# ruotianluo/ImageCaptioning.pytorch

Hardware: NVIDIA H100
Metric: captions/sec at beam=5 seq_len=20 (higher is better)
Workload: dtype f32 (fp32-grade: split-fp16 x3 tensor-core passes, fp32 accumulate)

## Files before the change

imagecaptioning.pytorch_b200/csrc/beam.cu:

```cuda
#include "../../include/capb200.h"
#include "common.cuh"
#include "kernels.cuh"
#include "vocab_row.cuh"

namespace capb200 {

namespace {

constexpr int MAXB = 16;

__device__ __forceinline__ double apply_penalty(int kind, float alpha, int length, double p) {
    if (kind == 1) return p / (pow(5.0 + length, (double)alpha) / pow(6.0, (double)alpha));
    if (kind == 2) return p / (double)length;
    return p;
}

template <int U = 8>
__device__ __forceinline__ void select_step(const BeamState& s, int img, int t, int live, int kl, int row0, int hist0, const float* top_val,
                                            const int* top_idx, const int* pen, int n_pen, float lambda, int penalty_kind,
                                            float penalty_alpha, double* __restrict__ done_p) {
    const int lane = threadIdx.x;
    const int b = s.beam, T = s.T;
    const int ncand = live * kl;
    float cv[U];
// ... 33 lines not shown
#pragma unroll
        for (int o = 16; o > 0; o >>= 1) {
            const float ov = __shfl_xor_sync(0xffffffffu, wv, o);
            const int of = __shfl_xor_sync(0xffffffffu, wf, o);
            if (ov > wv || (ov == wv && of < wf)) { wv = ov; wf = of; }
        }
        if (bu >= 0 && bf == wf && bv == wv) {
#pragma unroll
            for (int u = 0; u < U; ++u) if (u == bu) { cv[u] = -INFINITY; cf[u] = 0x7fffffff; }
        }
        if (lane == j) { my_v = wv; my_f = wf; }
    }
    __shared__ int sh_parent[MAXB], sh_word[MAXB], sh_slot[MAXB];
    const bool has = lane < b;
    const int parent = has ? my_f / s.V1 : 0;
    const int word = has ? my_f % s.V1 : 0;
    const bool ended = has && ((word == 0) || (t == T - 1));
    const unsigned em = __ballot_sync(0xffffffffu, ended);
    const int cnt0 = s.done_cnt[img];
    const int slot = cnt0 + __popc(em & ((1u << lane) - 1u));
    if (has) { sh_parent[lane] = parent; sh_word[lane] = word; sh_slot[lane] = ended ? slot : -1; }
    __syncwarp();
#pragma unroll 1
    for (int idx = lane; idx < b * t; idx += 32) {
        const int j = idx / t, q = idx - j * t;
        const long dst = ((long)img * b + j) * T, src = ((long)img * b + sh_parent[j]) * T;
        seq_new[dst + q] = seq_old[src + q];
        hist_new[dst + q] = hist_old[src + q];
    }
    if (em != 0u) {
#pragma unroll 1
        for (int idx = lane; idx < b * (t + 1); idx += 32) {
            const int j = idx / (t + 1), q = idx - j * (t + 1);
            if (sh_slot[j] < 0) continue;
            const long rec = ((long)img * b * T + sh_slot[j]) * T, src = ((long)img * b + sh_parent[j]) * T;
            s.done_seq[rec + q] = (q < t) ? seq_old[src + q] : sh_word[j];
            s.done_hist[rec + q] = (q < t) ? hist_old[src + q] : hist0 + sh_parent[j];
        }
    }
    if (has) {
        const long dst = ((long)img * b + lane) * T;
        seq_new[dst + t] = word;
        hist_new[dst + t] = hist0 + parent;
        float new_sum = my_v;
        if (ended) {
            const long rec = (long)img * b * T + slot;
            s.done_len[rec] = t + 1;
            s.done_raw[rec] = new_sum;
            done_p[rec] = apply_penalty(penalty_kind, penalty_alpha, t + 1, (double)new_sum);
            new_sum -= 1000.0f;
        }
        s.sums[(long)img * b + lane] = new_sum;
        s.tokens[(long)img * b + lane] = word;
        s.src_row[(long)img * b + lane] = row0 + parent;
    }
    if (lane == 0 && em != 0u) s.done_cnt[img] = cnt0 + __popc(em);
}

__global__ void __launch_bounds__(32) beam_step_kernel(BeamState s, int t, int live, const float* __restrict__ top_val,
                                                       const int* __restrict__ top_idx, int penalty_kind, float penalty_alpha,
                                                       double* __restrict__ done_p) {
    const int img = blockIdx.x;
    const long row0 = (long)img * live;
    select_step(s, img, t, live, s.beam, (int)row0, (int)row0, top_val + row0 * s.beam, top_idx + row0 * s.beam, nullptr, 0, 0.f, penalty_kind,
                penalty_alpha, done_p);
}

constexpr int kStepGroups = 8;
template <int U>
__global__ void __maxnreg__(U <= 2 ? 48 : 64) beam_search_step_kernel(BeamState s, const VocabStepArgs a, int t, int live, int penalty_kind, float penalty_alpha,
                                                        double* __restrict__ done_p, NextStateGather next) {
    __shared__ float s_red[kStepGroups][VT2 / 32];
    __shared__ int s_ridx[kStepGroups][VT2 / 32];
    __shared__ float s_val[MAXB * MAXB];
    __shared__ int s_idx[MAXB * MAXB];
    const int img = blockIdx.x, g = threadIdx.x / VT2, ng = blockDim.x / VT2;
    const int b = s.beam, row0 = img * live;
    for (int j = g; j < live; j += ng)
        stats_online128_row(a, row0 + j, threadIdx.x % VT2, GroupBarrier{1 + g}, s_red[g], s_ridx[g], s_val + j * b, s_idx + j * b);
    __syncthreads();
    if (threadIdx.x < 32) select_step<U>(s, img, t, live, b, row0, row0, s_val, s_idx, nullptr, 0, 0.f, penalty_kind, penalty_alpha, done_p);
    if (t == s.T - 1) return;
    __syncthreads();
    const int n4 = next.H >> 2;
    for (int i = threadIdx.x; i < b * n4; i += blockDim.x) {
        const int j = i / n4, c4 = i - j * n4;
        const long r = (long)img * b + j;
        copy_states4(r, s.src_row[r], c4, 2, next.s0, next.s1);
    }
}

__global__ void __launch_bounds__(32) diverse_beam_step_kernel(BeamState s, int G, int t, int k, const float* __restrict__ top_val,
                                                               const int* __restrict__ top_idx, float lambda, int rows_total, int penalty_kind,
                                                               float penalty_alpha, double* __restrict__ done_p) {
    const int i = blockIdx.x, lane = threadIdx.x;
    const int b = s.beam, T = s.T;
    __shared__ int sh_pen[MAXB];
    for (int g = 0; g < G && g <= t; ++g) {
        const int lt = t - g;
        if (lt >= T) continue;
        const int n_pen = g * b;
        __syncwarp();
        if (lane < n_pen) {
            const int pg = lane / b, j = lane - pg * b;
            const int last = min(t - pg, T - 1);
            const int* seq_pg = (last & 1) ? s.seq_a : s.seq_b;
            sh_pen[lane] = seq_pg[((long)(i * G + pg) * b + j) * T + lt];
        }
        __syncwarp();
        const int vimg = i * G + g;
        select_step(s, vimg, lt, lt == 0 ? 1 : b, k, vimg * b, g * rows_total + vimg * b, top_val + (long)vimg * b * k, top_idx + (long)vimg * b * k,
                    sh_pen, n_pen, lambda, penalty_kind, penalty_alpha, done_p);
    }
}

__global__ void __launch_bounds__(32) beam_finalize_kernel(BeamState s, int keep, const double* __restrict__ done_p, long long* __restrict__ out_seq,
                                                           int* __restrict__ out_len, float* __restrict__ out_p, float* __restrict__ out_raw,
                                                           int* __restrict__ out_hist) {
    const int img = blockIdx.x, lane = threadIdx.x;
    const int b = s.beam, T = s.T;
    const int cnt = s.done_cnt[img];
    const long base = (long)img * b * T;
    extern __shared__ unsigned char taken[];
    for (int i = lane; i < cnt; i += 32) taken[i] = 0;
    __syncwarp();
    for (int k = 0; k < keep; ++k) {
        double bv = -INFINITY;
        int bi = 0x7fffffff;
        for (int i = lane; i < cnt; i += 32) {
            if (!taken[i]) {
                const double v = done_p[base + i];
                if (v > bv || (v == bv && i < bi)) { bv = v; bi = i; }
            }
        }
#pragma unroll
        for (int o = 16; o > 0; o >>= 1) {
            const double ov = __shfl_xor_sync(0xffffffffu, bv, o);
            const int oi = __shfl_xor_sync(0xffffffffu, bi, o);
            if (ov > bv || (ov == bv && oi < bi)) { bv = ov; bi = oi; }
        }
        const long o = (long)img * keep + k;
        if (bi == 0x7fffffff) {
            if (lane == 0) { out_len[o] = 0; out_p[o] = -INFINITY; out_raw[o] = -INFINITY; }
            for (int q = lane; q < T; q += 32) { out_seq[o * T + q] = 0; out_hist[o * T + q] = -1; }
            continue;
        }
        if (lane == 0) {
            taken[bi] = 1;
            out_len[o] = s.done_len[base + bi];
            out_p[o] = (float)bv;
            out_raw[o] = s.done_raw[base + bi];
        }
        const int len = s.done_len[base + bi];
        for (int q = lane; q < T; q += 32) {
            out_seq[o * T + q] = (q < len) ? (long long)s.done_seq[(base + bi) * T + q] : 0;
            out_hist[o * T + q] = (q < len) ? s.done_hist[(base + bi) * T + q] : -1;
        }
        __syncwarp();
    }
}

__global__ void beam_edit_kernel(int rows, int k_in, int beam, int t, DecodeEdits ed, const int* __restrict__ prev_tokens,
                                 const float* __restrict__ val_in, const int* __restrict__ idx_in, float* __restrict__ val_out, int* __restrict__ idx_out,
                                 int first_beam, int first_group_rows, int first_group) {
    const int r = blockIdx.x * blockDim.x + threadIdx.x;
    if (r >= rows) return;
    if (first_beam > 0 && (r % first_beam) / first_group_rows == first_group) t = 0;
    float v[MAXB];
    int ix[MAXB];
    const int prev = (t > 0 && prev_tokens != nullptr) ? prev_tokens[r] : -1;
    bool prev_bad = false;
// ... 40 lines not shown
        return;
    }
    auto apply_edits = [&]() {
        if (seqs == nullptr || !ed.any()) return;
        __syncthreads();
        if (threadIdx.x == 0) {
            const int prev = sidx > 0 ? (int)seqs[item - 1] : -1;
            if (ed.unk_col >= 0 && ed.unk_col < V1) d[ed.unk_col] -= 1000.0f;
            if (ed.constraint && prev >= 0 && prev < V1) d[prev] = -INFINITY;
            bool prev_bad = false;
            for (int i = 0; i < ed.n_bad; ++i) prev_bad |= (sidx > 0 && ed.bad[i] == prev);
            if (prev_bad) d[0] = -INFINITY;
        }
    };
    const float* src = slab + (long)sidx * step_stride + (long)row * ld_slab;
    if (stats != nullptr) {
        const float2 st = stats[(long)sidx * stats_stride + row];
        const float mx = st.x, lsum = st.y;
        const float m2 = (mx - mx) - lsum, l2 = lsum;
        const bool twice = sidx > 0;
        const bool vec4 = ((V1 & 3) == 0) && ((ld_slab & 3) == 0) && ((step_stride & 3) == 0) && ((reinterpret_cast<uintptr_t>(slab) & 15) == 0) &&
                          ((reinterpret_cast<uintptr_t>(dst) & 15) == 0);
        if (vec4) {
            const float4* s4 = reinterpret_cast<const float4*>(src);
            float4* d4 = reinterpret_cast<float4*>(d);
            for (int v = threadIdx.x; v < V1 / 4; v += blockDim.x) {
                const float4 x = __ldg(s4 + v);
                float4 o;
                o.x = (x.x - mx) - lsum; o.y = (x.y - mx) - lsum; o.z = (x.z - mx) - lsum; o.w = (x.w - mx) - lsum;
                if (twice) { o.x = (o.x - m2) - l2; o.y = (o.y - m2) - l2; o.z = (o.z - m2) - l2; o.w = (o.w - m2) - l2; }
                d4[v] = o;
            }
        } else {
            for (int v = threadIdx.x; v < V1; v += blockDim.x) {
                const float lp = (src[v] - mx) - lsum;
                d[v] = twice ? (lp - m2) - l2 : lp;
            }
        }
        apply_edits();
        return;
    }
    const bool vec = ((V1 & 3) == 0) && ((ld_slab & 3) == 0) && ((step_stride & 3) == 0) && ((reinterpret_cast<uintptr_t>(slab) & 15) == 0) &&
                     ((reinterpret_cast<uintptr_t>(dst) & 15) == 0);
    if (vec) {
        const float4* s4 = reinterpret_cast<const float4*>(src);
        float4* d4 = reinterpret_cast<float4*>(d);
        for (int v = threadIdx.x; v < V1 / 4; v += blockDim.x) d4[v] = __ldg(s4 + v);
    } else {
        for (int v = threadIdx.x; v < V1; v += blockDim.x) d[v] = src[v];
    }
    apply_edits();
}

}

int beam_edit_launch(int rows, int k_in, int beam, int t, const DecodeEdits& ed, const int* prev_tokens, const float* val_in, const int* idx_in,
                     float* val_out, int* idx_out, cudaStream_t stream, int first_beam, int first_group_rows, int first_group) {
    CAPB_REQUIRE(k_in >= beam && k_in <= MAXB, "beam_size + number of active decode edits must be <= 16");
    if (rows <= 0) return 0;
    beam_edit_kernel<<<cdiv(rows, 128), 128, 0, stream>>>(rows, k_in, beam, t, ed, prev_tokens, val_in, idx_in, val_out, idx_out, first_beam,
                                                          first_group_rows, first_group);
    CAPB_CHECK_CUDA(cudaGetLastError());
    return 0;
}

int scale_rows_launch(float* x, long ld, int rows, int cols, float factor, cudaStream_t stream, int skip_beam, int skip_group_rows, int skip_group) {
    if (rows <= 0 || cols <= 0) return 0;
    long blocks = ((long)rows * cols + 255) / 256;
    if (blocks > sm_count() * 16) blocks = sm_count() * 16;
    scale_rows_kernel<<<(int)blocks, 256, 0, stream>>>(x, ld, rows, cols, factor, skip_beam, skip_group_rows, skip_group);
    CAPB_CHECK_CUDA(cudaGetLastError());
    return 0;
}

int beam_step_launch(const BeamState& s, int t, int live, const float* top_val, const int* top_idx, int penalty_kind, float penalty_alpha,
                     cudaStream_t stream) {
    CAPB_REQUIRE(s.beam >= 1 && s.beam <= MAXB, "beam size 1..16");
    CAPB_REQUIRE(s.beam * s.T <= MAXB * CAPB200_MAX_SEQ_LENGTH, "beam*T record capacity (16 x CAPB200_MAX_SEQ_LENGTH)");
    beam_step_kernel<<<s.B, 32, 0, stream>>>(s, t, live, top_val, top_idx, penalty_kind, penalty_alpha, s.done_p);
    CAPB_CHECK_CUDA(cudaGetLastError());
    return 0;
}

bool beam_search_step_applies(const VocabStepArgs& a, const NextStateGather& next) {
    auto al16 = [](const void* p) { return (reinterpret_cast<uintptr_t>(p) & 15) == 0; };
    auto al8 = [](const void* p) { return (reinterpret_cast<uintptr_t>(p) & 7) == 0; };
    auto state_ok = [&](const StateCopy& c) {
        return c.src != nullptr && c.dst.f != nullptr && (c.ld_src & 3) == 0 && (c.dst.ld & 3) == 0 && al16(c.src) && al16(c.dst.f) &&
               ((c.dst.hi == nullptr) == (c.dst.lo == nullptr)) && (c.dst.hi == nullptr || (al8(c.dst.hi) && al8(c.dst.lo)));
    };
    return (a.V1 & 3) == 0 && (a.ld & 3) == 0 && al16(a.logits) && next.H > 0 && (next.H & 3) == 0 && state_ok(next.s0) && state_ok(next.s1);
}

int beam_search_step_launch(const BeamState& s, const VocabStepArgs& a, int t, int live, int penalty_kind, float penalty_alpha,
                            const NextStateGather& next, cudaStream_t stream) {
    CAPB_REQUIRE(s.beam >= 1 && s.beam <= MAXB, "beam size 1..16");
    CAPB_REQUIRE(s.beam * s.T <= MAXB * CAPB200_MAX_SEQ_LENGTH, "beam*T record capacity (16 x CAPB200_MAX_SEQ_LENGTH)");
    CAPB_REQUIRE(a.topk == s.beam && a.stats != nullptr && a.rows == s.B * live && live >= 1 && live <= s.beam, "fused beam step arguments");
    CAPB_REQUIRE(beam_search_step_applies(a, next), "the fused beam step needs 16-byte aligned logit and state rows (V + 1 and H multiples of 4)");
    const int threads = min(live, kStepGroups) * VT2;
    if (s.beam <= 8) beam_search_step_kernel<2><<<s.B, threads, 0, stream>>>(s, a, t, live, penalty_kind, penalty_alpha, s.done_p, next);
    else beam_search_step_kernel<8><<<s.B, threads, 0, stream>>>(s, a, t, live, penalty_kind, penalty_alpha, s.done_p, next);
    CAPB_CHECK_CUDA(cudaGetLastError());
    return 0;
}

int diverse_beam_step_launch(const BeamState& s, int G, int t, int k, const float* top_val, const int* top_idx, float lambda, int rows_total,
                             int penalty_kind, float penalty_alpha, cudaStream_t stream) {
    CAPB_REQUIRE(G >= 2 && s.beam >= 1 && G * s.beam <= MAXB, "group_size * beams per group must be in 2..16");
    CAPB_REQUIRE(k >= s.beam && k <= MAXB && s.beam * k <= 256, "candidate list width");
    CAPB_REQUIRE(s.beam * s.T <= MAXB * CAPB200_MAX_SEQ_LENGTH, "beam*T record capacity (16 x CAPB200_MAX_SEQ_LENGTH)");
    CAPB_REQUIRE(lambda >= 0.f, "diversity_lambda must be >= 0 (the candidate lists rely on the penalty only lowering values)");
    diverse_beam_step_kernel<<<s.B / G, 32, 0, stream>>>(s, G, t, k, top_val, top_idx, lambda, rows_total, penalty_kind, penalty_alpha, s.done_p);
    CAPB_CHECK_CUDA(cudaGetLastError());
    return 0;
}

int beam_finalize_launch(const BeamState& s, int keep, long long* out_seq, int* out_len, float* out_p, float* out_raw, int* out_hist,
                         cudaStream_t stream) {
    CAPB_REQUIRE(keep >= 1 && keep <= s.beam, "keep must be in 1..beam");
    beam_finalize_kernel<<<s.B, 32, (size_t)s.beam * s.T, stream>>>(s, keep, s.done_p, out_seq, out_len, out_p, out_raw, out_hist);
    CAPB_CHECK_CUDA(cudaGetLastError());
    return 0;
}

int gather_logprob_rows_launch(const float* slab, long step_stride, long ld_slab, const int* hist, int nseq, int T, int V1, float* dst,
                               const float2* stats, long stats_stride, cudaStream_t stream, const long long* seqs, const DecodeEdits* ed) {
    if (nseq <= 0) return 0;
    gather_rows_kernel<<<nseq * T, 256, 0, stream>>>(slab, step_stride, ld_slab, hist, T, V1, dst, stats, stats_stride, seqs, ed ? *ed : DecodeEdits());
    CAPB_CHECK_CUDA(cudaGetLastError());
    return 0;
}

}
```

imagecaptioning.pytorch_b200/csrc/common.cuh:

```cuda
#pragma once
#include <atomic>
#include <cstdint>
#include <cstdio>
#include <cstring>
#include <string>
#include <cuda.h>
#include <cuda_fp16.h>
#include <cuda_runtime.h>

namespace capb200 {

void set_error(const std::string& msg);
#define CAPB_CHECK_CUDA(expr)                                                                          \
    do {                                                                                               \
        cudaError_t _e = (expr);                                                                       \
        if (_e != cudaSuccess) {                                                                       \
            capb200::set_error(std::string(#expr) + " failed: " + cudaGetErrorString(_e) + " at " +    \
                               __FILE__ + ":" + std::to_string(__LINE__));                            \
            return 1;                                                                                  \
        }                                                                                              \
    } while (0)
#define CAPB_REQUIRE(cond, msg)                                                                        \
    do {                                                                                               \
        if (!(cond)) {                                                                                 \
            capb200::set_error(std::string("requirement failed: ") + #cond + " -- " + (msg));          \
            return 1;                                                                                  \
        }                                                                                              \
    } while (0)

inline int cdiv(int a, int b) { return (a + b - 1) / b; }
inline long round_up(long a, long b) { return (a + b - 1) / b * b; }

inline bool first_use_on_device(std::atomic<unsigned long long>& mask) {
    int dev = 0;
    if (cudaGetDevice(&dev) != cudaSuccess || dev < 0 || dev > 63) return true;
    const unsigned long long bit = 1ull << dev;
    return (mask.fetch_or(bit) & bit) == 0;
}

inline int sm_count() {
    static std::atomic<int> cache[64];
    int dev = 0;
    if (cudaGetDevice(&dev) != cudaSuccess || dev < 0 || dev > 63) dev = 0;
    int n = cache[dev].load();
    if (n == 0) {
        if (cudaDeviceGetAttribute(&n, cudaDevAttrMultiProcessorCount, dev) != cudaSuccess || n < 1) n = 132;
        cache[dev].store(n);
    }
    return n;
}

__device__ __forceinline__ void split_f32(float x, __half& hi, __half& lo) {
    hi = __float2half_rn(x);
    lo = __float2half_rn(x - __half2float(hi));
}

constexpr int kMaxSeg = 3;
struct GemmSeg {
    const float* A = nullptr;
    long lda = 0;
    const float* W = nullptr;
    long ldw = 0;
    const __half* A_hi = nullptr;
    const __half* A_lo = nullptr;
    long lda_h = 0;
    const __half* W_hi = nullptr;
    const __half* W_lo = nullptr;
    long ldw_h = 0;
    int K = 0;
};
struct GemmEpilogue {
    const float* bias = nullptr;
    const float* row_bias = nullptr;
    long ld_row_bias = 0;
    int rows_per_group = 1;
    const float* residual = nullptr;
    long ld_res = 0;
    int relu = 0;
    float* C = nullptr;
    long ldc = 0;
    __half* C_hi = nullptr;
    __half* C_lo = nullptr;
    long ldcs = 0;
    int lstm = 0;
    int H = 0;
    const float* c_prev = nullptr;
    long ld_cprev = 0;
    const int* src_row = nullptr;
    float* c_out = nullptr;
    long ld_cout = 0;
    const float* gather_bias = nullptr;
    long ld_gb = 0;
    const int* gather_idx = nullptr;
    float* h_f = nullptr;
    __half* h_hi = nullptr;
    __half* h_lo = nullptr;
    long ld_h = 0;
    unsigned long long* trace = nullptr;
};

__device__ __forceinline__ float fast_sigmoid(float x) { return __fdividef(1.0f, 1.0f + __expf(-x)); }
__device__ __forceinline__ float fast_tanh(float x) {
    const float e = __expf(2.0f * x);
    return 1.0f - __fdividef(2.0f, 1.0f + e);
}
__device__ __forceinline__ void fast_tanh4(const float (&x)[4], float (&t)[4]) {
    float y[4];
#pragma unroll
    for (int i = 0; i < 4; ++i) y[i] = 1.0f + __expf(fminf(2.0f * x[i], 20.0f));
    const float p01 = y[0] * y[1], p23 = y[2] * y[3];
    const float r = __fdividef(1.0f, p01 * p23);
    const float r01 = r * p23, r23 = r * p01;
    t[0] = fmaf(-2.0f, r01 * y[1], 1.0f);
    t[1] = fmaf(-2.0f, r01 * y[0], 1.0f);
    t[2] = fmaf(-2.0f, r23 * y[3], 1.0f);
    t[3] = fmaf(-2.0f, r23 * y[2], 1.0f);
}
struct GemmProblem {
    int M = 0, N = 0, nseg = 0;
    GemmSeg seg[kMaxSeg];
    GemmEpilogue epi;
};

enum NumericMode : int {
    kModeSimtFp32 = 0,
    kModeTcF16x3 = 1,
    kModeTcF16x1 = 2,
};

int gemm_simt_launch(const GemmProblem& p, cudaStream_t stream);

struct GemmTcPlan;
GemmTcPlan* gemm_tc_plan_create(const GemmProblem& p, int passes);
int gemm_tc_tile_n(int M, int N);
int gemm_tc_tile_m(int M, int N, int bn);
void gemm_tc_plan_destroy(GemmTcPlan* plan);
int gemm_tc_plan_launch(GemmTcPlan* plan, const GemmEpilogue* epi_override, int M_override, cudaStream_t stream);
bool gemm_tc_supported(const GemmProblem& p, std::string* why);

int split_planes_launch(const float* x, long ldx, int rows, int cols, __half* hi, __half* lo, long ldh, cudaStream_t stream);
int* range_flag_ptr();
int range_flag_read(int reset);
#define CAPB_CHECK_RANGE()                                                                                              \
    do {                                                                                                                \
        if (capb200::range_flag_read(0)) {                                                                              \
            capb200::set_error("a value with |x| >= 65504 (or inf/nan) reached a split-fp16 conversion in an earlier call: results of the "   \
                               "tensor-core modes are invalid for such inputs/weights (DESIGN.md section 3); capb200_range_status(1) clears the flag"); \
            return 1;                                                                                                   \
        }                                                                                                               \
    } while (0)
int split_planes_interleave_launch(const float* x, long ldx, int H, int cols, __half* hi, __half* lo, long ldh, cudaStream_t stream);

}
```

imagecaptioning.pytorch_b200/csrc/engine.cu:

```cuda
#include <map>
#include <mutex>
#include <vector>

#include "../../include/capb200.h"
#include "common.cuh"
#include "kernels.cuh"
#include "engine_common.cuh"
#include "train_common.cuh"

namespace capb200 {

static thread_local std::string g_last_error;
void set_error(const std::string& msg) { g_last_error = msg; }
const char* last_error_cstr() { return g_last_error.c_str(); }

__global__ void capb_fill_int_kernel(int* p, int n, int v) {
    const int i = blockIdx.x * blockDim.x + threadIdx.x;
    if (i < n) p[i] = v;
}
__global__ void capb_load_token_column_kernel(const long long* src, long ld, int col, int n, int* dst) {
    const int i = blockIdx.x * blockDim.x + threadIdx.x;
    if (i < n) dst[i] = (int)src[(long)i * ld + col];
}
__global__ void capb_store_token_column_kernel(const int* src, int n, long long* dst, long ld, int col) {
    const int i = blockIdx.x * blockDim.x + threadIdx.x;
    if (i < n) dst[(long)i * ld + col] = src[i];
}
int store_token_column_launch(const int* src, int n, long long* dst, long ld, int col, cudaStream_t st) {
    if (n <= 0) return 0;
    capb_store_token_column_kernel<<<cdiv(n, 256), 256, 0, st>>>(src, n, dst, ld, col);
    CAPB_CHECK_CUDA(cudaGetLastError());
    return 0;
}
int fill_int_launch(int* p, int n, int v, cudaStream_t st) {
    if (n <= 0) return 0;
    capb_fill_int_kernel<<<cdiv(n, 256), 256, 0, st>>>(p, n, v);
    CAPB_CHECK_CUDA(cudaGetLastError());
    return 0;
}
int load_token_column_launch(const long long* src, long ld, int col, int n, int* dst, cudaStream_t st) {
    if (n <= 0) return 0;
    capb_load_token_column_kernel<<<cdiv(n, 256), 256, 0, st>>>(src, ld, col, n, dst);
    CAPB_CHECK_CUDA(cudaGetLastError());
    return 0;
}

namespace {

__global__ void add_vec_kernel(const float* a, const float* b, float* o, int n) {
    const int i = blockIdx.x * blockDim.x + threadIdx.x;
    if (i < n) o[i] = a[i] + b[i];
}
__global__ void interleave_gates_kernel(const float* src, float* dst, int H) {
    const int i = blockIdx.x * blockDim.x + threadIdx.x;
    if (i < 4 * H) dst[i] = src[(i & 3) * H + (i >> 2)];
}

__global__ void iota_div_kernel(int* p, int n, int div) {
    const int i = blockIdx.x * blockDim.x + threadIdx.x;
    if (i < n) p[i] = i / div;
}


enum GemmId { G_FC = 0, G_ATT, G_CTX, G_GFC, G_LSTM1, G_H2ATT, G_LSTM2, G_LOGIT, G_CORE, G_A2C, G_COUNT };
constexpr int G_REPORTED = 9;

}
}

using namespace capb200;


struct capb200_engine : EngineBase {
    capb200_model_cfg cfg{};
    capb200_weights w{};
    int E = 0, H = 0, A = 0;

    float *bsum_att = nullptr, *bsum_lang = nullptr, *bsum_core = nullptr;
    float *bsum_att_il = nullptr, *bsum_lang_il = nullptr;
    float* xgate = nullptr;
    long ld_xgate = 0;
    bool use_xgate = true;
    Planes p_fc, p_attw, p_ctx, p_logit, p_a_ih_h, p_a_ih_fc, p_a_ih_x, p_a_hh, p_l_ih_a, p_l_ih_h, p_l_hh, p_h2att, p_i2h, p_h2h, p_a2c;

    Planes in_fc, in_att;
    Act fc_e, att_e, p_att, g_fc, xt, h0_in, h1_in, h0_out, h1_out, att_res, att_h, gates;
    float *c0[2] = {nullptr, nullptr}, *c1[2] = {nullptr, nullptr};
    long ld_c = 0;
    int* img_of_row = nullptr;
    float* att_score = nullptr;
    int core_cur = 0;

    bool profiling = false;
    std::vector<cudaEvent_t> ev_pool;
    std::vector<int> ev_ids;
    std::vector<double> ev_flops;
    size_t ev_used = 0;
    double prof_ms[G_COUNT] = {0};
    double prof_flops[G_COUNT] = {0};
    long prof_calls[G_COUNT] = {0};

    ~capb200_engine() override { for (cudaEvent_t ev : ev_pool) cudaEventDestroy(ev); }
    int decode_workspace(int B, int rows, int R, int beam, int rows_per_image, cudaStream_t st) override;
    int decode_prepare(const float* fc, const float* att, const DecodeCtx& c, cudaStream_t st) override;
    int decode_core(int rows, int rpi, const int* tokens, const int* src_row, int t, float* logits, long ld, const DecodeCtx& c, cudaStream_t st) override;
    bool next_state(NextStateGather* next) override;
    bool loop_graph_ok() const override { return !profiling; }
};

namespace {

void layout_weights(capb200_engine* e, Arena& a) {
    const int H = e->H, E = e->E, A = e->A, V1 = e->V1;
    const bool updown = e->cfg.family == CAPB200_FAMILY_UPDOWN;
    e->bsum_att = a.take<float>(4 * H);
    e->bsum_lang = a.take<float>(4 * H);
    e->bsum_core = a.take<float>(5 * H);
    e->bsum_att_il = a.take<float>(4 * H);
    e->bsum_lang_il = a.take<float>(4 * H);
    if (updown) { e->ld_xgate = round_up(4 * H, 8); e->xgate = a.take<float>((long)V1 * e->ld_xgate); }
    if (!e->tc) return;
    e->p_logit = carve_planes(a, V1, H);
    if (updown) {
        e->p_fc = carve_planes(a, H, e->cfg.fc_feat_size);
        e->p_attw = carve_planes(a, H, e->cfg.att_feat_size);
        e->p_ctx = carve_planes(a, A, H);
        e->p_a_ih_h = carve_planes(a, 4 * H, H);
        e->p_a_ih_fc = carve_planes(a, 4 * H, H);
        e->p_a_ih_x = carve_planes(a, 4 * H, E);
        e->p_a_hh = carve_planes(a, 4 * H, H);
        e->p_l_ih_a = carve_planes(a, 4 * H, H);
        e->p_l_ih_h = carve_planes(a, 4 * H, H);
        e->p_l_hh = carve_planes(a, 4 * H, H);
        e->p_h2att = carve_planes(a, A, H);
    } else if (e->cfg.family == CAPB200_FAMILY_ATT2IN2) {
        e->p_attw = carve_planes(a, H, e->cfg.att_feat_size);
        e->p_ctx = carve_planes(a, A, H);
        e->p_h2att = carve_planes(a, A, H);
        e->p_i2h = carve_planes(a, 5 * H, E);
        e->p_h2h = carve_planes(a, 5 * H, H);
        e->p_a2c = carve_planes(a, 2 * H, H);
    } else {
        e->p_fc = carve_planes(a, E, e->cfg.fc_feat_size);
        e->p_i2h = carve_planes(a, 5 * H, E);
        e->p_h2h = carve_planes(a, 5 * H, H);
    }
}

void layout_workspace(capb200_engine* e, Arena& a, int B, int rows, int R, int beam) {
    const int H = e->H, E = e->E, A = e->A, T = e->T;
    const bool updown = e->cfg.family == CAPB200_FAMILY_UPDOWN;
    const bool attn = e->reads_att;
    const bool tc = e->tc;
    if (tc) {
        e->in_fc = carve_planes(a, B, e->cfg.fc_feat_size);
        if (attn) e->in_att = carve_planes(a, (long)B * R, e->cfg.att_feat_size);
    }
    e->fc_e.carve(a, B, updown ? H : E, tc);
    if (attn) {
        e->att_e.carve(a, (long)B * R, H, tc);
        e->p_att.carve(a, (long)B * R, A, false);
        e->att_res.carve(a, rows, H, tc);
        e->att_h.carve(a, rows, A, false);
    }
    if (updown) {
        e->g_fc.carve(a, B, 4 * H, false);
        e->h1_in.carve(a, rows, H, tc);
        e->h1_out.carve(a, rows, H, tc);
    }
    e->xt.carve(a, rows, E, tc);
    e->h0_in.carve(a, rows, H, tc);
    e->h0_out.carve(a, rows, H, tc);
    e->gates.carve(a, rows, 5 * H, false);
    e->ld_c = round_up(H, 8);
    for (int i = 0; i < 2; ++i) {
        e->c0[i] = a.take<float>((long)rows * e->ld_c);
        e->c1[i] = a.take<float>((long)rows * e->ld_c);
    }
    e->carve_head(a, rows);
    e->img_of_row = a.take<int>(rows);
    e->att_score = a.take<float>((long)rows * (R > 0 ? R : 1));
    e->d.carve(a, B, rows, beam, T);
}

int ensure_workspace(capb200_engine* e, int B, int rows, int R, int beam, cudaStream_t st) {
    return e->grow(B, rows, R, beam, st, [&](Arena& a, int nB, int nRows, int nR, int nBeam) { layout_workspace(e, a, nB, nRows, nR, nBeam); });
}

int run_gemm(capb200_engine* e, int id, GemmProblem& g, int plan_rows, cudaStream_t st) {
    if (!e->profiling) return e->gemm(id, g, plan_rows, st);
    if (e->ev_used + 2 > e->ev_pool.size()) {
        for (int i = 0; i < 64; ++i) {
            cudaEvent_t ev;
            CAPB_CHECK_CUDA(cudaEventCreate(&ev));
            e->ev_pool.push_back(ev);
        }
    }
    double k_total = 0;
    for (int s = 0; s < g.nseg; ++s) k_total += g.seg[s].K;
    CAPB_CHECK_CUDA(cudaEventRecord(e->ev_pool[e->ev_used], st));
    const int rc = e->gemm(id, g, plan_rows, st);
    CAPB_CHECK_CUDA(cudaEventRecord(e->ev_pool[e->ev_used + 1], st));
    e->ev_used += 2;
    e->ev_ids.push_back(id);
    e->ev_flops.push_back(2.0 * g.M * g.N * k_total);
    return rc;
}

int prepare(capb200_engine* e, const float* fc, const float* att, const float* mask, int B, int R, cudaStream_t st) {
    CAPB_NVTX("capb200 prepare_feature (fc_embed, att_embed, ctx2att)");
    const int H = e->H, E = e->E, A = e->A;
    const bool updown = e->cfg.family == CAPB200_FAMILY_UPDOWN;
    const capb200_weights& w = e->w;
    ActView fc_in;  fc_in.f = const_cast<float*>(fc);  fc_in.ld = e->cfg.fc_feat_size;
    if (e->tc && e->cfg.family != CAPB200_FAMILY_ATT2IN2) {
        e->launches++;
        if (split_planes_launch(fc, e->cfg.fc_feat_size, B, e->cfg.fc_feat_size, e->in_fc.hi, e->in_fc.lo, e->in_fc.ld, st)) return 1;
    }
    if (e->cfg.family != CAPB200_FAMILY_ATT2IN2) {
        GemmProblem g;
        g.M = B; g.N = updown ? H : E; g.nseg = 1;
        g.seg[0] = seg_of(fc_in, w.fc_embed_w, e->cfg.fc_feat_size, e->p_fc, e->cfg.fc_feat_size);
        g.seg[0].A_hi = e->in_fc.hi; g.seg[0].A_lo = e->in_fc.lo; g.seg[0].lda_h = e->in_fc.ld;
        g.epi.bias = w.fc_embed_b; g.epi.relu = updown ? 1 : 0;
        g.epi.C = e->fc_e.v.f; g.epi.ldc = e->fc_e.v.ld; g.epi.C_hi = e->fc_e.v.hi; g.epi.C_lo = e->fc_e.v.lo; g.epi.ldcs = e->fc_e.v.ld;
        if (run_gemm(e, G_FC, g, e->capB, st)) return 1;
    }
    if (!e->reads_att) return 0;
    ActView att_in; att_in.f = const_cast<float*>(att); att_in.ld = e->cfg.att_feat_size;
    if (e->tc) {
        e->launches++;
        if (split_planes_launch(att, e->cfg.att_feat_size, B * R, e->cfg.att_feat_size, e->in_att.hi, e->in_att.lo, e->in_att.ld, st)) return 1;
    }
    {
        GemmProblem g;
        g.M = B * R; g.N = H; g.nseg = 1;
        g.seg[0] = seg_of(att_in, w.att_embed_w, e->cfg.att_feat_size, e->p_attw, e->cfg.att_feat_size);
        g.seg[0].A_hi = e->in_att.hi; g.seg[0].A_lo = e->in_att.lo; g.seg[0].lda_h = e->in_att.ld;
        g.epi.bias = w.att_embed_b; g.epi.relu = 1;
        g.epi.C = e->att_e.v.f; g.epi.ldc = e->att_e.v.ld; g.epi.C_hi = e->att_e.v.hi; g.epi.C_lo = e->att_e.v.lo; g.epi.ldcs = e->att_e.v.ld;
        if (run_gemm(e, G_ATT, g, e->capB * e->capR, st)) return 1;
    }
    if (mask != nullptr) {
        e->launches++;
        if (mask_rows_launch(e->att_e.v, B, R, H, mask, R, st)) return 1;
    }
    {
        GemmProblem g;
        g.M = B * R; g.N = A; g.nseg = 1;
        g.seg[0] = seg_of(e->att_e.v, w.ctx2att_w, H, e->p_ctx, H);
        g.epi.bias = w.ctx2att_b;
        g.epi.C = e->p_att.v.f; g.epi.ldc = e->p_att.v.ld;
        if (run_gemm(e, G_CTX, g, e->capB * e->capR, st)) return 1;
    }
    if (!updown) return 0;
    {
        GemmProblem g;
        g.M = B; g.N = 4 * H; g.nseg = 1;
        g.seg[0] = seg_of(e->fc_e.v, w.att_lstm_w_ih + H, E + 2 * H, e->p_a_ih_fc, H);
        g.epi.bias = e->tc ? e->bsum_att_il : e->bsum_att;
        g.epi.C = e->g_fc.v.f; g.epi.ldc = e->g_fc.v.ld;
        if (run_gemm(e, G_GFC, g, e->capB, st)) return 1;
    }
    return 0;
}

int logit_gemm(capb200_engine* e, const ActView& h, int rows, float* logits, long ld_logits, cudaStream_t st) {
    ActView x;
    if (e->run_logit_head(h, rows, &x, st)) return 1;
    GemmProblem g;
    g.M = rows; g.N = e->V1; g.nseg = 1;
    g.seg[0] = seg_of(x, e->w.logit_w, e->H, e->p_logit, e->H);
    g.epi.bias = e->w.logit_b;
    g.epi.C = logits; g.epi.ldc = ld_logits;
    return run_gemm(e, G_LOGIT, g, e->capRows, st);
}

int core_step(capb200_engine* e, int rows, int rpi, const int* tokens, const int* src_row, float* logits, long ld_logits, int n_images, int R,
              const float* mask, cudaStream_t st, bool states_gathered = false) {
    const int H = e->H, E = e->E, A = e->A;
    const capb200_weights& w = e->w;
    if (e->cfg.family == CAPB200_FAMILY_UPDOWN) {
        StateCopy s0, s1;
        s0.src = e->h0_out.v.f; s0.ld_src = e->h0_out.v.ld; s0.dst = e->h0_in.v;
        s1.src = e->h1_out.v.f; s1.ld_src = e->h1_out.v.ld; s1.dst = e->h1_in.v;
        const bool xg = e->use_xgate;
        CAPB_REQUIRE(!states_gathered || xg, "the fused beam step gathers the states only; the word embedding needs the separate gather");
        if (!states_gathered) {
            e->launches++;
            if (state_gather_embed_launch(rows, tokens, src_row, w.embed, E, xg ? 0 : E, 1, e->xt.v, H, 2, s0, s1, st)) return 1;
        }
        const int cur = e->core_cur, nxt = cur ^ 1;
        {
            GemmProblem g;
            g.M = rows; g.N = 4 * H;
            g.seg[0] = seg_of(e->h1_in.v, w.att_lstm_w_ih, E + 2 * H, e->p_a_ih_h, H);
            g.seg[1] = seg_of(e->h0_in.v, w.att_lstm_w_hh, H, e->p_a_hh, H);
            g.nseg = 2;
            if (!xg) { g.seg[2] = seg_of(e->xt.v, w.att_lstm_w_ih + 2 * H, E + 2 * H, e->p_a_ih_x, E); g.nseg = 3; }
            g.epi.row_bias = e->g_fc.v.f; g.epi.ld_row_bias = e->g_fc.v.ld; g.epi.rows_per_group = rpi;
            if (e->tc) {
                g.epi.lstm = 1; g.epi.H = H;
                g.epi.c_prev = e->c0[cur]; g.epi.ld_cprev = e->ld_c; g.epi.src_row = src_row;
                g.epi.c_out = e->c0[nxt]; g.epi.ld_cout = e->ld_c;
                g.epi.gather_bias = xg ? e->xgate : nullptr; g.epi.ld_gb = e->ld_xgate; g.epi.gather_idx = tokens;
                g.epi.h_f = e->h0_out.v.f; g.epi.h_hi = e->h0_out.v.hi; g.epi.h_lo = e->h0_out.v.lo; g.epi.ld_h = e->h0_out.v.ld;
            } else {
                g.epi.C = e->gates.v.f; g.epi.ldc = e->gates.v.ld;
            }
            if (run_gemm(e, G_LSTM1, g, e->capRows, st)) return 1;
        }
        if (!e->tc) {
            e->launches++;
            if (lstm_pointwise_launch(rows, H, e->gates.v.f, e->gates.v.ld, src_row, e->c0[cur], e->ld_c, e->c0[nxt], e->ld_c, e->h0_out.v,
                                      xg ? e->xgate : nullptr, e->ld_xgate, tokens, st)) return 1;
        }
        {
            GemmProblem g;
            g.M = rows; g.N = A; g.nseg = 1;
            g.seg[0] = seg_of(e->h0_out.v, w.h2att_w, H, e->p_h2att, H);
            g.epi.bias = w.h2att_b;
            g.epi.C = e->att_h.v.f; g.epi.ldc = e->att_h.v.ld;
            if (run_gemm(e, G_H2ATT, g, e->capRows, st)) return 1;
        }
        e->launches += 2;
        if (additive_attention_launch(n_images, rpi, R, A, H, e->att_h.v.f, e->att_h.v.ld, e->p_att.v.f, e->p_att.v.ld, e->att_e.v.f, e->att_e.v.ld,
                                      mask, R, w.alpha_w, w.alpha_b, e->att_score, e->att_res.v, st)) return 1;
        {
            GemmProblem g;
            g.M = rows; g.N = 4 * H; g.nseg = 3;
            g.seg[0] = seg_of(e->att_res.v, w.lang_lstm_w_ih, 2 * H, e->p_l_ih_a, H);
            g.seg[1] = seg_of(e->h0_out.v, w.lang_lstm_w_ih + H, 2 * H, e->p_l_ih_h, H);
            g.seg[2] = seg_of(e->h1_in.v, w.lang_lstm_w_hh, H, e->p_l_hh, H);
            if (e->tc) {
                g.epi.bias = e->bsum_lang_il;
                g.epi.lstm = 1; g.epi.H = H;
                g.epi.c_prev = e->c1[cur]; g.epi.ld_cprev = e->ld_c; g.epi.src_row = src_row;
                g.epi.c_out = e->c1[nxt]; g.epi.ld_cout = e->ld_c;
                g.epi.h_f = e->h1_out.v.f; g.epi.h_hi = e->h1_out.v.hi; g.epi.h_lo = e->h1_out.v.lo; g.epi.ld_h = e->h1_out.v.ld;
            } else {
                g.epi.bias = e->bsum_lang;
                g.epi.C = e->gates.v.f; g.epi.ldc = e->gates.v.ld;
            }
            if (run_gemm(e, G_LSTM2, g, e->capRows, st)) return 1;
        }
        if (!e->tc) {
            e->launches++;
            if (lstm_pointwise_launch(rows, H, e->gates.v.f, e->gates.v.ld, src_row, e->c1[cur], e->ld_c, e->c1[nxt], e->ld_c, e->h1_out.v,
                                      nullptr, 0, nullptr, st)) return 1;
        }
        e->core_cur = nxt;
        return logit_gemm(e, e->h1_out.v, rows, logits, ld_logits, st);
    }
    if (e->cfg.family == CAPB200_FAMILY_ATT2IN2) {
        StateCopy s0, s1;
        s0.src = e->h0_out.v.f; s0.ld_src = e->h0_out.v.ld; s0.dst = e->h0_in.v;
        e->launches++;
        if (state_gather_embed_launch(rows, tokens, src_row, w.embed, E, E, 1, e->xt.v, H, 1, s0, s1, st)) return 1;
        const int cur = e->core_cur, nxt = cur ^ 1;
        {
            GemmProblem g;
            g.M = rows; g.N = A; g.nseg = 1;
            g.seg[0] = seg_of(e->h0_in.v, w.h2att_w, H, e->p_h2att, H);
            g.epi.bias = w.h2att_b;
            g.epi.C = e->att_h.v.f; g.epi.ldc = e->att_h.v.ld;
            if (run_gemm(e, G_H2ATT, g, e->capRows, st)) return 1;
        }
        e->launches += 2;
        if (additive_attention_launch(n_images, rpi, R, A, H, e->att_h.v.f, e->att_h.v.ld, e->p_att.v.f, e->p_att.v.ld, e->att_e.v.f, e->att_e.v.ld,
                                      mask, R, w.alpha_w, w.alpha_b, e->att_score, e->att_res.v, st)) return 1;
        {
            GemmProblem g;
            g.M = rows; g.N = 5 * H; g.nseg = 2;
            g.seg[0] = seg_of(e->xt.v, w.i2h_w, E, e->p_i2h, E);
            g.seg[1] = seg_of(e->h0_in.v, w.h2h_w, H, e->p_h2h, H);
            g.epi.bias = e->bsum_core;
            g.epi.C = e->gates.v.f; g.epi.ldc = e->gates.v.ld;
            if (run_gemm(e, G_CORE, g, e->capRows, st)) return 1;
        }
        {
            GemmProblem g;
            g.M = rows; g.N = 2 * H; g.nseg = 1;
            g.seg[0] = seg_of(e->att_res.v, w.a2c_w, H, e->p_a2c, H);
            g.epi.residual = e->gates.v.f + 3 * H; g.epi.ld_res = e->gates.v.ld;
            g.epi.C = e->gates.v.f + 3 * H; g.epi.ldc = e->gates.v.ld;
            if (run_gemm(e, G_A2C, g, e->capRows, st)) return 1;
        }
        e->launches++;
        if (maxout_pointwise_launch(rows, H, e->gates.v.f, e->gates.v.ld, src_row, e->c0[cur], e->ld_c, e->c0[nxt], e->ld_c, e->h0_out.v, st)) return 1;
        e->core_cur = nxt;
        return logit_gemm(e, e->h0_out.v, rows, logits, ld_logits, st);
    }
    const bool fresh = (src_row == e->d.neg1);
    for (int pass = fresh ? 0 : 1; pass < 2; ++pass) {
        StateCopy s0, s1;
        s0.src = e->h0_out.v.f; s0.ld_src = e->h0_out.v.ld; s0.dst = e->h0_in.v;
        const int* srcs = (pass == 0) ? e->d.neg1 : (fresh ? nullptr : src_row);
        e->launches++;
        if (pass == 0) {
            if (state_gather_embed_launch(rows, e->img_of_row, srcs, e->fc_e.v.f, e->fc_e.v.ld, E, 0, e->xt.v, H, 1, s0, s1, st)) return 1;
        } else {
            if (state_gather_embed_launch(rows, tokens, srcs, w.embed, E, E, 0, e->xt.v, H, 1, s0, s1, st)) return 1;
        }
        const int cur = e->core_cur, nxt = cur ^ 1;
        GemmProblem g;
        g.M = rows; g.N = 5 * H; g.nseg = 2;
        g.seg[0] = seg_of(e->xt.v, w.i2h_w, E, e->p_i2h, E);
        g.seg[1] = seg_of(e->h0_in.v, w.h2h_w, H, e->p_h2h, H);
        g.epi.bias = e->bsum_core;
        g.epi.C = e->gates.v.f; g.epi.ldc = e->gates.v.ld;
        if (run_gemm(e, G_CORE, g, e->capRows, st)) return 1;
        e->launches++;
        if (maxout_pointwise_launch(rows, H, e->gates.v.f, e->gates.v.ld, srcs, e->c0[cur], e->ld_c, e->c0[nxt], e->ld_c, e->h0_out.v, st)) return 1;
        e->core_cur = nxt;
    }
    return logit_gemm(e, e->h0_out.v, rows, logits, ld_logits, st);
}

}

namespace capb200 {

int add_vec_launch(const float* a, const float* b, float* o, int n, cudaStream_t st) {
    add_vec_kernel<<<cdiv(n, 256), 256, 0, st>>>(a, b, o, n);
    CAPB_CHECK_CUDA(cudaGetLastError());
    return 0;
}

int interleave_gates_launch(const float* src, float* dst, int H, cudaStream_t st) {
    interleave_gates_kernel<<<cdiv(4 * H, 256), 256, 0, st>>>(src, dst, H);
    CAPB_CHECK_CUDA(cudaGetLastError());
    return 0;
}

int build_gate_table(EngineBase& e, const float* embed, int E, int H, const float* w_x, long ld_w, const Planes& p_x, float* xgate, long ld_xgate,
                     cudaStream_t st) {
    const int V1 = e.V1;
    const long ldE = round_up(E, 8);
    char* tmp = nullptr;
    const size_t tmp_bytes = (size_t)V1 * ldE * (sizeof(float) + (e.tc ? 2 * sizeof(__half) : 0)) + 1024;
    CAPB_CHECK_CUDA(cudaMallocAsync(&tmp, tmp_bytes, st));
    CAPB_CHECK_CUDA(cudaMemsetAsync(tmp, 0, tmp_bytes, st));
    ActView ev;
    ev.ld = ldE;
    ev.f = reinterpret_cast<float*>(tmp);
    if (e.tc) {
        ev.hi = reinterpret_cast<__half*>(tmp + (size_t)V1 * ldE * sizeof(float));
        ev.lo = ev.hi + (size_t)V1 * ldE;
    }
    int rc = 0;
    if (ldE == E) {
        rc = relu_copy_launch(embed, (long)V1 * E, ev, st);
    } else {
        for (int v = 0; v < V1 && !rc; ++v) {
            ActView rv = ev;
            rv.f += (long)v * ldE; if (rv.hi) { rv.hi += (long)v * ldE; rv.lo += (long)v * ldE; }
            rc = relu_copy_launch(embed + (long)v * E, E, rv, st);
        }
    }
    GemmProblem g;
    g.M = V1; g.N = 4 * H; g.nseg = 1;
    g.seg[0] = seg_of(ev, w_x, ld_w, p_x, E);
    g.epi.C = xgate; g.epi.ldc = ld_xgate;
    if (!rc) {
        if (!e.tc) {
            rc = gemm_simt_launch(g, st);
        } else {
            GemmTcPlan* plan = gemm_tc_plan_create(g, e.mode == CAPB200_MODE_TC_F16X3 ? 3 : 1);
            rc = plan ? gemm_tc_plan_launch(plan, nullptr, 0, st) : 1;
            if (plan) gemm_tc_plan_destroy(plan);
        }
    }
    e.launches += 2;
    cudaFreeAsync(tmp, st);
    return rc;
}

EngineBase* engine_base(capb200_engine* e) { return e; }

}

int capb200_engine::decode_workspace(int B, int rows, int R, int beam, int rows_per_image, cudaStream_t st) {
    if (ensure_workspace(this, B, rows, R, beam, st)) return 1;
    if (!reads_att) { iota_div_kernel<<<cdiv(rows, 256), 256, 0, st>>>(img_of_row, rows, rows_per_image); launches++; }
    return 0;
}

int capb200_engine::decode_prepare(const float* fc, const float* att, const DecodeCtx& c, cudaStream_t st) {
    if (prepare(this, fc, att, c.mask, c.B, c.R, st)) return 1;
    core_cur = 0;
    return 0;
}

int capb200_engine::decode_core(int rows, int rpi, const int* tokens, const int* src_row, int , float* logits, long ld, const DecodeCtx& c,
                                cudaStream_t st) {
    return core_step(this, rows, rpi, tokens, src_row, logits, ld, c.B, c.R, c.mask, st, d.states_gathered);
}

bool capb200_engine::next_state(NextStateGather* next) {
    if (cfg.family != CAPB200_FAMILY_UPDOWN || !use_xgate) return false;
    next->s0.src = h0_out.v.f; next->s0.ld_src = h0_out.v.ld; next->s0.dst = h0_in.v;
    next->s1.src = h1_out.v.f; next->s1.ld_src = h1_out.v.ld; next->s1.dst = h1_in.v;
    next->H = H;
    return true;
}

extern "C" {

const char* capb200_last_error(void) { return g_last_error.c_str(); }
int capb200_abi_version(void) { return CAPB200_ABI_VERSION; }
int capb200_range_status(int reset) { return range_flag_read(reset); }

capb200_engine* capb200_engine_create(const capb200_model_cfg* cfg) {
    if (cfg == nullptr) { set_error("null cfg"); return nullptr; }
    if (cfg->family != CAPB200_FAMILY_UPDOWN && cfg->family != CAPB200_FAMILY_NEWFC && cfg->family != CAPB200_FAMILY_ATT2IN2) {
        set_error("unknown model family");
        return nullptr;
    }
    capb200_engine* e = create_engine<capb200_engine>(cfg->vocab_size, cfg->seq_length, cfg->numeric_mode, G_COUNT);
    if (e == nullptr) return nullptr;
    e->cfg = *cfg;
    e->E = cfg->input_encoding_size;
    e->H = cfg->rnn_size;
    e->A = cfg->att_hid_size;
    e->bind_name = "capb200_engine_bind_weights";
    e->family = e->graph_family = cfg->family;
    e->reads_fc = cfg->family != CAPB200_FAMILY_ATT2IN2;
    e->reads_att = cfg->family != CAPB200_FAMILY_NEWFC;
    return e;
}

void capb200_engine_destroy(capb200_engine* e) { delete e; }

long capb200_engine_launch_count(const capb200_engine* e) { return e ? e->launches : 0; }

int capb200_engine_set_profiling(capb200_engine* e, int enable) {
    CAPB_REQUIRE(e != nullptr, "null engine");
    e->profiling = enable != 0;
    return 0;
}

int capb200_engine_read_profile(capb200_engine* e, int reset, double* ms, double* flops, long* calls, int n) {
    CAPB_REQUIRE(e != nullptr && n >= G_REPORTED, "need room for 9 GEMM ids");
    CAPB_CHECK_CUDA(cudaDeviceSynchronize());
    for (size_t i = 0; i < e->ev_ids.size(); ++i) {
        float t = 0.f;
        CAPB_CHECK_CUDA(cudaEventElapsedTime(&t, e->ev_pool[2 * i], e->ev_pool[2 * i + 1]));
        e->prof_ms[e->ev_ids[i]] += t;
        e->prof_flops[e->ev_ids[i]] += e->ev_flops[i];
        e->prof_calls[e->ev_ids[i]] += 1;
    }
    e->ev_ids.clear();
    e->ev_flops.clear();
    e->ev_used = 0;
    e->prof_ms[G_CORE] += e->prof_ms[G_A2C]; e->prof_flops[G_CORE] += e->prof_flops[G_A2C]; e->prof_calls[G_CORE] += e->prof_calls[G_A2C];
    e->prof_ms[G_A2C] = 0; e->prof_flops[G_A2C] = 0; e->prof_calls[G_A2C] = 0;
    for (int i = 0; i < G_REPORTED; ++i) {
        if (ms) ms[i] = e->prof_ms[i];
        if (flops) flops[i] = e->prof_flops[i];
        if (calls) calls[i] = e->prof_calls[i];
        if (reset) { e->prof_ms[i] = 0; e->prof_flops[i] = 0; e->prof_calls[i] = 0; }
    }
    return 0;
}

int capb200_engine_bind_weights(capb200_engine* e, const capb200_weights* w, void* stream) {
    CAPB_REQUIRE(e != nullptr && w != nullptr, "null argument");
    cudaStream_t st = static_cast<cudaStream_t>(stream);
    const bool updown = e->cfg.family == CAPB200_FAMILY_UPDOWN;
    const bool att2in2 = e->cfg.family == CAPB200_FAMILY_ATT2IN2;
    CAPB_REQUIRE(w->embed && (att2in2 || (w->fc_embed_w && w->fc_embed_b)) && w->logit_w && w->logit_b, "missing shared weights");
    if (att2in2) {
        CAPB_REQUIRE(w->att_embed_w && w->att_embed_b && w->ctx2att_w && w->ctx2att_b && w->h2att_w && w->h2att_b && w->alpha_w && w->alpha_b &&
                         w->i2h_w && w->i2h_b && w->h2h_w && w->h2h_b && w->a2c_w && w->a2c_b, "missing Att2in2 weights");
    } else if (updown) {
        CAPB_REQUIRE(w->att_embed_w && w->att_embed_b && w->ctx2att_w && w->ctx2att_b && w->att_lstm_w_ih && w->att_lstm_w_hh && w->att_lstm_b_ih &&
                         w->att_lstm_b_hh && w->lang_lstm_w_ih && w->lang_lstm_w_hh && w->lang_lstm_b_ih && w->lang_lstm_b_hh && w->h2att_w &&
                         w->h2att_b && w->alpha_w && w->alpha_b, "missing UpDown weights");
    } else {
        CAPB_REQUIRE(w->i2h_w && w->i2h_b && w->h2h_w && w->h2h_b, "missing NewFC weights");
    }
    e->w = *w;
    const int H = e->H, E = e->E, A = e->A, V1 = e->V1;
    if (e->alloc_wblock(st, [&](Arena& a) { layout_weights(e, a); })) return 1;
    int rc = 0;
    if (updown) {
        rc |= add_vec_launch(w->att_lstm_b_ih, w->att_lstm_b_hh, e->bsum_att, 4 * H, st);
        rc |= add_vec_launch(w->lang_lstm_b_ih, w->lang_lstm_b_hh, e->bsum_lang, 4 * H, st);
        rc |= interleave_gates_launch(e->bsum_att, e->bsum_att_il, H, st);
        rc |= interleave_gates_launch(e->bsum_lang, e->bsum_lang_il, H, st);
        e->launches += 4;
    } else {
        rc |= add_vec_launch(w->i2h_b, w->h2h_b, e->bsum_core, 5 * H, st);
        e->launches += 1;
        if (att2in2) {
            rc |= add_vec_launch(e->bsum_core + 3 * H, w->a2c_b, e->bsum_core + 3 * H, 2 * H, st);
            e->launches += 1;
        }
    }
    if (rc) return 1;
    if (e->tc) {
        rc = e->pack(w->logit_w, H, V1, H, e->p_logit, st);
        if (updown) {
            rc |= e->pack(w->fc_embed_w, e->cfg.fc_feat_size, H, e->cfg.fc_feat_size, e->p_fc, st);
            rc |= e->pack(w->att_embed_w, e->cfg.att_feat_size, H, e->cfg.att_feat_size, e->p_attw, st);
            rc |= e->pack(w->ctx2att_w, H, A, H, e->p_ctx, st);
            rc |= e->pack_gates(w->att_lstm_w_ih, E + 2 * H, H, H, e->p_a_ih_h, st);
            rc |= e->pack_gates(w->att_lstm_w_ih + H, E + 2 * H, H, H, e->p_a_ih_fc, st);
            rc |= e->pack_gates(w->att_lstm_w_ih + 2 * H, E + 2 * H, H, E, e->p_a_ih_x, st);
            rc |= e->pack_gates(w->att_lstm_w_hh, H, H, H, e->p_a_hh, st);
            rc |= e->pack_gates(w->lang_lstm_w_ih, 2 * H, H, H, e->p_l_ih_a, st);
            rc |= e->pack_gates(w->lang_lstm_w_ih + H, 2 * H, H, H, e->p_l_ih_h, st);
            rc |= e->pack_gates(w->lang_lstm_w_hh, H, H, H, e->p_l_hh, st);
            rc |= e->pack(w->h2att_w, H, A, H, e->p_h2att, st);
        } else if (att2in2) {
            rc |= e->pack(w->att_embed_w, e->cfg.att_feat_size, H, e->cfg.att_feat_size, e->p_attw, st);
            rc |= e->pack(w->ctx2att_w, H, A, H, e->p_ctx, st);
            rc |= e->pack(w->h2att_w, H, A, H, e->p_h2att, st);
            rc |= e->pack(w->i2h_w, E, 5 * H, E, e->p_i2h, st);
            rc |= e->pack(w->h2h_w, H, 5 * H, H, e->p_h2h, st);
            rc |= e->pack(w->a2c_w, H, 2 * H, H, e->p_a2c, st);
        } else {
            rc |= e->pack(w->fc_embed_w, e->cfg.fc_feat_size, E, e->cfg.fc_feat_size, e->p_fc, st);
            rc |= e->pack(w->i2h_w, E, 5 * H, E, e->p_i2h, st);
            rc |= e->pack(w->h2h_w, H, 5 * H, H, e->p_h2h, st);
        }
// ... 1025 lines not shown
```

imagecaptioning.pytorch_b200/csrc/engine_common.cuh:

```cuda
#pragma once
#include <cstdio>
#include <cstdlib>
#include <cstring>
#include <string>
#include <vector>

#include "../../include/capb200.h"
#include "common.cuh"
#include "kernels.cuh"
#include "nvtx.cuh"

struct capb200_cider_table {
    capb200::CiderTable* t = nullptr;
};

namespace capb200 {

struct Planes {
    __half* hi = nullptr;
    __half* lo = nullptr;
    long ld = 0;
};

struct Arena {
// ... 10 lines not shown

struct Act {
    ActView v;
    void carve(Arena& a, long rows, long cols, bool planes) {
        v.ld = round_up(cols, 64);
        v.f = a.take<float>(rows * v.ld);
        if (planes) {
            v.hi = a.take<__half>(rows * v.ld);
            v.lo = a.take<__half>(rows * v.ld);
        } else {
            v.hi = v.lo = nullptr;
        }
    }
};

inline DecodeEdits to_edits(const capb200_decode_edits& c) {
    DecodeEdits e;
    e.constraint = c.decoding_constraint;
    e.unk_col = c.unk_col;
    e.n_bad = (c.bad_endings != nullptr && c.n_bad_endings > 0) ? c.n_bad_endings : 0;
    e.bad = c.bad_endings;
    e.trigrams = c.block_trigrams;
    e.trigram_rows = c.trigram_rows;
    return e;
}

inline Planes carve_planes(Arena& a, long rows, long cols) {
    Planes p;
    p.ld = round_up(cols, 64);
    p.hi = a.take<__half>(rows * p.ld);
    p.lo = a.take<__half>(rows * p.ld);
    return p;
}


inline GemmSeg seg_of(const ActView& a, const float* w, long ldw, const Planes& wp, int K) {
    GemmSeg s;
    s.A = a.f; s.lda = a.ld; s.W = w; s.ldw = ldw;
    s.A_hi = a.hi; s.A_lo = a.lo; s.lda_h = a.ld;
    s.W_hi = wp.hi; s.W_lo = wp.lo; s.ldw_h = wp.ld;
    s.K = K;
    return s;
}


inline int run_gemm_mode(int mode, GemmTcPlan** plan, GemmProblem& g, int plan_rows, cudaStream_t st) {
    if (mode == 0) return gemm_simt_launch(g, st);
    if (*plan == nullptr) {
        GemmProblem planned = g;
        planned.M = plan_rows;
        *plan = gemm_tc_plan_create(planned, mode == 1 ? 3 : 1);
        if (*plan == nullptr) return 1;
    }
    return gemm_tc_plan_launch(*plan, &g.epi, g.M, st);
}


struct DecodeBuffers {
    int *tokens = nullptr, *src_row = nullptr, *neg1 = nullptr, *unfinished = nullptr, *forced = nullptr;
    float* top_val = nullptr;
    int* top_idx = nullptr;
    float* top_val_e = nullptr;
    int* top_idx_e = nullptr;
    float2* slab_stats = nullptr;
    BeamState bs;
    long long* rec_seq = nullptr;
    int *rec_len = nullptr, *rec_hist = nullptr, *out_hist = nullptr, *tmp_len = nullptr;
    float *rec_p = nullptr, *rec_raw = nullptr, *tmp_p = nullptr, *tmp_raw = nullptr;
    float* slab = nullptr;
    size_t slab_bytes = 0;
    float2* dbs_stats = nullptr;
    size_t dbs_stats_bytes = 0;
    int* dbs_done_cnt = nullptr;
    size_t dbs_done_bytes = 0;
    const float2* last_stats = nullptr;
    long slab_step_stride = 0;
    int last_B = 0, last_beam = 0;
    DecodeEdits last_edits;
    cudaGraphExec_t loop_exec = nullptr;
    unsigned long long loop_key[8] = {0, 0, 0, 0, 0, 0, 0, 0}, seen_key[8] = {0, 0, 0, 0, 0, 0, 0, 0};
    long loop_launches = 0;
    bool graph_broken = false;
    bool states_gathered = false;

    void release() {
        if (loop_exec) cudaGraphExecDestroy(loop_exec);
        loop_exec = nullptr;
        cudaFree(slab);
        cudaFree(dbs_stats);
        cudaFree(dbs_done_cnt);
        slab = nullptr; dbs_stats = nullptr; dbs_done_cnt = nullptr;
    }

    void carve(Arena& a, int B, int rows, int beam, int T) {
        tokens = a.take<int>(rows);
        src_row = a.take<int>(rows);
        neg1 = a.take<int>(rows);
        unfinished = a.take<int>(rows);
        forced = a.take<int>(rows);
        top_val = a.take<float>((long)rows * 16);
        top_idx = a.take<int>((long)rows * 16);
        top_val_e = a.take<float>((long)rows * 16);
        top_idx_e = a.take<int>((long)rows * 16);
        slab_stats = a.take<float2>((long)rows * T);
        const long rec = (long)B * beam * T;
        bs.sums = a.take<float>((long)B * beam);
        bs.seq_a = a.take<int>(rec);
        bs.seq_b = a.take<int>(rec);
        bs.hist_a = a.take<int>(rec);
        bs.hist_b = a.take<int>(rec);
        bs.done_cnt = a.take<int>(B);
        bs.done_seq = a.take<int>(rec * T);
        bs.done_hist = a.take<int>(rec * T);
        bs.done_len = a.take<int>(rec);
        bs.done_p = a.take<double>(rec);
        bs.done_raw = a.take<float>(rec);
        bs.tokens = tokens;
        bs.src_row = src_row;
        rec_seq = a.take<long long>(rec);
        rec_hist = a.take<int>(rec);
        out_hist = a.take<int>(rec);
        rec_len = a.take<int>((long)B * beam);
        rec_p = a.take<float>((long)B * beam);
        rec_raw = a.take<float>((long)B * beam);
        tmp_len = a.take<int>((long)B * beam);
        tmp_p = a.take<float>((long)B * beam);
        tmp_raw = a.take<float>((long)B * beam);
    }
};

__global__ void capb_fill_int_kernel(int* p, int n, int v);
__global__ void capb_load_token_column_kernel(const long long* src, long ld, int col, int n, int* dst);
int fill_int_launch(int* p, int n, int v, cudaStream_t st);
int load_token_column_launch(const long long* src, long ld, int col, int n, int* dst, cudaStream_t st);
int store_token_column_launch(const int* src, int n, long long* dst, long ld, int col, cudaStream_t st);

inline const int* beam_ancestors(const BeamState& s, int t) { return ((t - 1) & 1) ? s.hist_a : s.hist_b; }

inline unsigned long long loop_graph_key(const void* ws, const void* wblock, const void* mask, int R, int family) {
    unsigned long long h = 1469598103934665603ull;
    auto mix = [&](unsigned long long v) { h ^= v; h *= 1099511628211ull; };
    mix(reinterpret_cast<uintptr_t>(ws)); mix(reinterpret_cast<uintptr_t>(wblock)); mix(reinterpret_cast<uintptr_t>(mask));
    mix((unsigned long long)R); mix((unsigned long long)family + 17);
    return h | 1ull;
}

inline int grow_buffer(void** p, size_t* bytes, size_t need, cudaStream_t st) {
    if (need <= *bytes) return 0;
    CAPB_CHECK_CUDA(cudaStreamSynchronize(st));
    if (*p) CAPB_CHECK_CUDA(cudaFree(*p));
    *p = nullptr;
    *bytes = 0;
    const cudaError_t e = cudaMalloc(p, need);
    if (e != cudaSuccess) {
        (void)cudaGetLastError();
        *p = nullptr;
        set_error("cannot allocate " + std::to_string(need >> 20) + " MB of device workspace (" + cudaGetErrorString(e) +
                  "); its size grows with batch, length and V + 1: DESIGN.md, 'Vocabularies above 51 199 words'");
        return 1;
    }
    *bytes = need;
    return 0;
}

template <class Loop>
int run_beam_loop(DecodeBuffers& d, const unsigned long long (&key)[8], bool use_graph, long* launches, cudaStream_t st, Loop run_loop) {
    static const bool graphs_off = getenv("CAPB200_NO_GRAPH") != nullptr;
    const bool debug = getenv("CAPB200_GRAPH_DEBUG") != nullptr;
    const bool try_graph = use_graph && !graphs_off && !d.graph_broken;
    if (try_graph && d.loop_exec != nullptr && memcmp(key, d.loop_key, sizeof(key)) == 0) {
        CAPB_CHECK_CUDA(cudaGraphLaunch(d.loop_exec, st));
        *launches += d.loop_launches;
        if (debug) fprintf(stderr, "capb200: beam loop replayed from its CUDA graph\n");
    } else if (try_graph && memcmp(key, d.seen_key, sizeof(key)) == 0) {
        if (d.loop_exec != nullptr) { cudaGraphExecDestroy(d.loop_exec); d.loop_exec = nullptr; }
        const long l0 = *launches;
        cudaGraph_t graph = nullptr;
        bool ok = cudaStreamBeginCapture(st, cudaStreamCaptureModeThreadLocal) == cudaSuccess;
        const int rc = ok ? run_loop() : 1;
        if (ok) ok = cudaStreamEndCapture(st, &graph) == cudaSuccess && graph != nullptr && rc == 0;
        if (ok) ok = cudaGraphInstantiate(&d.loop_exec, graph, 0) == cudaSuccess;
        if (graph != nullptr) cudaGraphDestroy(graph);
        if (!ok) {
            (void)cudaGetLastError();
            d.loop_exec = nullptr;
            d.graph_broken = true;
            *launches = l0;
            if (run_loop()) return 1;
        } else {
            d.loop_launches = *launches - l0;
            memcpy(d.loop_key, key, sizeof(key));
            CAPB_CHECK_CUDA(cudaGraphLaunch(d.loop_exec, st));
            if (debug) fprintf(stderr, "capb200: beam loop captured into a CUDA graph (%ld launches)\n", d.loop_launches);
        }
    } else {
        memcpy(d.seen_key, key, sizeof(key));
        if (run_loop()) return 1;
    }
    return 0;
}

template <class CoreFn>
int beam_decode_driver(DecodeBuffers& d, int V1, int T, int B, int beam, int keep, int penalty_kind, float penalty_alpha, long long* seq,
                       float* seq_logprobs, long long* done_seq, int* done_len, float* done_p, float* done_raw, CoreFn core, long* launches,
                       cudaStream_t st, unsigned long long graph_key = 0, const DecodeEdits& ed = DecodeEdits(), float temperature = 1.0f,
                       const NextStateGather* next = nullptr, int form = 0) {
    const int rows = B * beam;
    const bool edits = ed.any();
    const int k_in = beam + ed.kinds();
    CAPB_REQUIRE(!ed.trigrams, "block_trigrams applies to _sample only (AttModel.py:306)");
    CAPB_REQUIRE(k_in <= 16, "beam_size + number of active decode edits (decoding_constraint, remove_bad_endings, UNK suppression) must be <= 16");
    CAPB_REQUIRE(form >= 0 && form <= 2, "beam step form must be 0 (automatic), 1 (separate kernels) or 2 (fused)");
    if (temperature == 0.f) temperature = 1.0f;
    CAPB_REQUIRE(temperature > 0.f, "temperature must be positive");
    if (grow_buffer(reinterpret_cast<void**>(&d.slab), &d.slab_bytes, (size_t)T * rows * V1 * sizeof(float), st)) return 1;
    d.slab_step_stride = (long)rows * V1;
    d.last_B = B;
    d.last_beam = beam;
    BeamState s = d.bs;
    s.B = B; s.beam = beam; s.T = T; s.V1 = V1;
    bool fused = false;
    if (form != 1 && next != nullptr && !edits && temperature == 1.0f) {
        VocabStepArgs probe;
        probe.V1 = V1; probe.ld = V1; probe.logits = d.slab;
        fused = beam_search_step_applies(probe, *next);
    }
    CAPB_REQUIRE(form != 2 || fused, "the fused beam step needs the engine's state descriptor, no decode edits, temperature 1 and 16-byte aligned "
                                     "logit and state rows (V + 1 and H multiples of 4)");
    auto run_loop = [&]() -> int {
        CAPB_NVTX("capb200 beam loop (T steps: core, vocab stats, beam step)");
        CAPB_CHECK_CUDA(cudaMemsetAsync(s.sums, 0, sizeof(float) * B * beam, st));
        CAPB_CHECK_CUDA(cudaMemsetAsync(s.done_cnt, 0, sizeof(int) * B, st));
        CAPB_CHECK_CUDA(cudaMemsetAsync(d.tokens, 0, sizeof(int) * rows, st));
        for (int t = 0; t < T; ++t) {
            const int live = (t == 0) ? 1 : beam;
            const int nrows = B * live;
            float* logits = d.slab + (long)t * d.slab_step_stride;
            d.states_gathered = fused && t > 0;
            const int rc = core(nrows, live, d.tokens, t == 0 ? d.neg1 : d.src_row, t, logits, (long)V1);
            d.states_gathered = false;
            if (rc) return 1;
            if (t > 0 && temperature != 1.0f) {
                if (scale_rows_launch(logits, V1, nrows, V1, 1.0f / temperature, st)) return 1;
                *launches += 1;
            }
            VocabStepArgs va;
            va.rows = nrows; va.V1 = V1; va.logits = logits; va.ld = V1;
            va.twice = (t > 0) ? 1 : 0;
            va.topk = edits ? k_in : beam; va.top_val = d.top_val; va.top_idx = d.top_idx;
            va.stats = d.slab_stats + (long)t * rows;
            if (fused) {
                if (beam_search_step_launch(s, va, t, live, penalty_kind, penalty_alpha, *next, st)) return 1;
                *launches += 1;
                continue;
            }
            if (vocab_step_launch(va, st)) return 1;
            const float* tv = d.top_val;
            const int* ti = d.top_idx;
            if (edits) {
                if (beam_edit_launch(nrows, k_in, beam, t, ed, d.tokens, d.top_val, d.top_idx, d.top_val_e, d.top_idx_e, st)) return 1;
                tv = d.top_val_e; ti = d.top_idx_e;
                *launches += 1;
            }
            if (beam_step_launch(s, t, live, tv, ti, penalty_kind, penalty_alpha, st)) return 1;
            *launches += 2;
        }
        return 0;
    };
    unsigned long long key[8] = {graph_key, (unsigned long long)B, (unsigned long long)beam, (unsigned long long)T, (unsigned long long)V1,
                                 (unsigned long long)penalty_kind, 0ull, (unsigned long long)reinterpret_cast<uintptr_t>(d.slab)};
    memcpy(&key[6], &penalty_alpha, sizeof(float));
    memcpy(reinterpret_cast<char*>(&key[6]) + 4, &temperature, sizeof(float));
    key[5] ^= ((unsigned long long)(ed.constraint & 1) << 8) ^ ((unsigned long long)(unsigned)(ed.unk_col + 1) << 16) ^ ((unsigned long long)ed.n_bad << 48);
    key[5] ^= (unsigned long long)fused << 9;
    key[0] ^= (unsigned long long)reinterpret_cast<uintptr_t>(ed.bad) * 0x9E3779B97F4A7C15ull;
    d.last_edits = ed;
    d.last_stats = d.slab_stats;
    if (run_beam_loop(d, key, graph_key != 0, launches, st, run_loop)) return 1;
    CAPB_NVTX("capb200 beam finalize + log-prob rows");
    if (beam_finalize_launch(s, beam, d.rec_seq, d.rec_len, d.rec_p, d.rec_raw, d.rec_hist, st)) return 1;
    *launches += 1;
    if (keep == beam) {
        CAPB_CHECK_CUDA(cudaMemcpyAsync(seq, d.rec_seq, sizeof(long long) * B * beam * T, cudaMemcpyDeviceToDevice, st));
        if (seq_logprobs) {
            *launches += 1;
            if (gather_logprob_rows_launch(d.slab, d.slab_step_stride, V1, d.rec_hist, B * beam, T, V1, seq_logprobs, d.slab_stats, rows, st, d.rec_seq, &ed)) return 1;
        }
    } else {
        *launches += 1;
        if (beam_finalize_launch(s, 1, seq, d.tmp_len, d.tmp_p, d.tmp_raw, d.out_hist, st)) return 1;
        if (seq_logprobs) {
            *launches += 1;
            if (gather_logprob_rows_launch(d.slab, d.slab_step_stride, V1, d.out_hist, B, T, V1, seq_logprobs, d.slab_stats, rows, st, seq, &ed)) return 1;
        }
    }
    if (done_seq) CAPB_CHECK_CUDA(cudaMemcpyAsync(done_seq, d.rec_seq, sizeof(long long) * B * beam * T, cudaMemcpyDeviceToDevice, st));
    if (done_len) CAPB_CHECK_CUDA(cudaMemcpyAsync(done_len, d.rec_len, sizeof(int) * B * beam, cudaMemcpyDeviceToDevice, st));
    if (done_p) CAPB_CHECK_CUDA(cudaMemcpyAsync(done_p, d.rec_p, sizeof(float) * B * beam, cudaMemcpyDeviceToDevice, st));
    if (done_raw) CAPB_CHECK_CUDA(cudaMemcpyAsync(done_raw, d.rec_raw, sizeof(float) * B * beam, cudaMemcpyDeviceToDevice, st));
    return 0;
}

template <class CoreFn>
int diverse_beam_decode_driver(DecodeBuffers& d, int V1, int T, int B, int beam, int G, float lambda, int keep, int penalty_kind, float penalty_alpha,
                               long long* seq, float* seq_logprobs, long long* done_seq, int* done_len, float* done_p, float* done_raw, CoreFn core,
                               long* launches, cudaStream_t st, unsigned long long graph_key, const DecodeEdits& ed, float temperature) {
    CAPB_REQUIRE(G >= 2 && beam % G == 0, "diverse beam search needs group_size >= 2 dividing beam_size");
    CAPB_REQUIRE(lambda >= 0.f, "diversity_lambda must be >= 0");
    const int bdash = beam / G, rows = B * beam, steps = T + G - 1;
    CAPB_REQUIRE(keep == 1 || keep == bdash, "sample_n must be 1 or beam_size / group_size (AttModel.py:223)");
    const bool edits = ed.any();
    const int k_in = beam + ed.kinds();
    CAPB_REQUIRE(!ed.trigrams, "block_trigrams applies to _sample only (AttModel.py:306)");
    CAPB_REQUIRE(k_in <= 16, "beam_size + number of active decode edits (decoding_constraint, remove_bad_endings, UNK suppression) must be <= 16");
    if (temperature == 0.f) temperature = 1.0f;
    CAPB_REQUIRE(temperature > 0.f, "temperature must be positive");
    if (grow_buffer(reinterpret_cast<void**>(&d.slab), &d.slab_bytes, (size_t)steps * rows * V1 * sizeof(float), st)) return 1;
    if (grow_buffer(reinterpret_cast<void**>(&d.dbs_stats), &d.dbs_stats_bytes, (size_t)steps * rows * sizeof(float2), st)) return 1;
    if (grow_buffer(reinterpret_cast<void**>(&d.dbs_done_cnt), &d.dbs_done_bytes, (size_t)B * G * sizeof(int), st)) return 1;
    d.slab_step_stride = (long)rows * V1;
    d.last_B = B;
    d.last_beam = beam;
    d.last_edits = ed;
    d.last_stats = d.dbs_stats;
    BeamState s = d.bs;
    s.B = B * G; s.beam = bdash; s.T = T; s.V1 = V1;
    s.done_cnt = d.dbs_done_cnt;
    auto run_loop = [&]() -> int {
        CAPB_NVTX("capb200 diverse beam loop (T+G-1 steps: core, vocab stats, group steps)");
        CAPB_CHECK_CUDA(cudaMemsetAsync(s.sums, 0, sizeof(float) * rows, st));
        CAPB_CHECK_CUDA(cudaMemsetAsync(s.done_cnt, 0, sizeof(int) * B * G, st));
        CAPB_CHECK_CUDA(cudaMemsetAsync(d.tokens, 0, sizeof(int) * rows, st));
        CAPB_CHECK_CUDA(cudaMemsetAsync(d.src_row, 0xff, sizeof(int) * rows, st));
        for (int t = 0; t < steps; ++t) {
            float* logits = d.slab + (long)t * d.slab_step_stride;
            if (core(rows, beam, d.tokens, d.src_row, t, logits, (long)V1)) return 1;
            if (t > 0 && temperature != 1.0f) {
                if (scale_rows_launch(logits, V1, rows, V1, 1.0f / temperature, st, beam, bdash, t)) return 1;
                *launches += 1;
            }
            VocabStepArgs va;
            va.rows = rows; va.V1 = V1; va.logits = logits; va.ld = V1;
            va.twice = (t > 0) ? 1 : 0;
            va.first_beam = beam; va.first_group_rows = bdash; va.first_group = t;
            va.topk = edits ? k_in : beam; va.top_val = d.top_val; va.top_idx = d.top_idx;
            va.stats = d.dbs_stats + (long)t * rows;
            if (vocab_step_launch(va, st)) return 1;
            const float* tv = d.top_val;
            const int* ti = d.top_idx;
            if (edits) {
                if (beam_edit_launch(rows, k_in, beam, t, ed, d.tokens, d.top_val, d.top_idx, d.top_val_e, d.top_idx_e, st, beam, bdash, t)) return 1;
                tv = d.top_val_e; ti = d.top_idx_e;
                *launches += 1;
            }
            if (diverse_beam_step_launch(s, G, t, beam, tv, ti, lambda, rows, penalty_kind, penalty_alpha, st)) return 1;
            *launches += 2;
        }
// ... 573 lines not shown
```

imagecaptioning.pytorch_b200/csrc/gemm_tc.cu:

```cuda
#include <cstdlib>
#include <cstring>

#include "common.cuh"
#include "ptx.cuh"

namespace capb200 {

namespace {

constexpr int BM = 128;
constexpr int BK = 64;
constexpr int kConsumers = 2;
constexpr int kThreads = 128 * (1 + kConsumers);

struct TcParams {
    CUtensorMap a_hi[kMaxSeg];
    CUtensorMap a_lo[kMaxSeg];
    CUtensorMap w_hi[kMaxSeg];
    CUtensorMap w_lo[kMaxSeg];
    int kblocks[kMaxSeg];
    int nseg;
    int M, N;
    float* C;
    long ldc;
    __half* C_hi;
    __half* C_lo;
    long ldcs;
    const float* bias;
    const float* row_bias;
    long ld_row_bias;
    int rows_per_group;
    int relu;
    const float* residual;
    long ld_res;
    int tiles_m, tiles_n;
    int lstm, H;
    const float* c_prev;
    long ld_cprev;
    const int* src_row;
    float* c_out;
    long ld_cout;
    const float* gather_bias;
    long ld_gb;
    const int* gather_idx;
    float* h_f;
    __half* h_hi;
    __half* h_lo;
    long ld_h;
    unsigned long long* trace;
};

__device__ __forceinline__ unsigned long long gtimer() {
    unsigned long long t;
    asm volatile("mov.u64 %0, %%globaltimer;" : "=l"(t));
    return t;
}
#define CAPB_TRACE(slot) do { if (TRACE && p.trace != nullptr) p.trace[(long)blockIdx.x * 16 + (slot)] = gtimer(); } while (0)

template <int BN, int PASSES, int TM = BM>
struct TcCfg {
    static constexpr int kTileM = TM;
    static constexpr int kPasses = PASSES;
    static constexpr int kPlanes = (PASSES == 3) ? 2 : 1;
    static constexpr uint32_t kABytes = TM * BK * 2;
    static constexpr uint32_t kWBytes = BN * BK * 2;
    static constexpr uint32_t kStageBytes = kPlanes * (kABytes + kWBytes);
    static constexpr uint32_t kRingBudget = 227 * 1024 - 1024  - 256 ;
    static constexpr int kStages = kRingBudget / kStageBytes >= 8 ? 8 : kRingBudget / kStageBytes;
    static constexpr uint32_t kSmemBytes = kStages * kStageBytes + 1024  + 256 ;
    static_assert(BN == 64 || BN == 128 || BN == 160, "wgmma wrappers exist for N = 64, 128 and 160");
    static_assert(TM == BM || TM == 2 * BM, "one or two 128-row A boxes per plane");
    static_assert(kWBytes % 1024 == 0, "operand tiles must keep the 1024-byte swizzle-atom alignment");
    static_assert(kStages >= 2, "need at least a double buffer");
    static_assert(kSmemBytes <= 227 * 1024, "shared memory of one H100 block");
};

template <int BN>
__device__ __forceinline__ void wgmma_f16(float* acc, uint64_t da, uint64_t db, int scale_d) {
    if (BN == 160) ptx::wgmma_f16_n160(acc, da, db, scale_d);
    else if (BN == 128) ptx::wgmma_f16_n128(acc, da, db, scale_d);
    else ptx::wgmma_f16_n64(acc, da, db, scale_d);
}

enum EpiKind : int {
    kEpiStore = 0,
    kEpiPlanes = 1,
    kEpiLstm = 2,
};

template <int BN>
__device__ __forceinline__ void epi_adds(const TcParams& p, float* acc, int r0, int c0) {
    const int ncol = p.N - c0;
    const int lim[2] = {r0 < p.M ? ncol : 0, r0 + 8 < p.M ? ncol : 0};
    if (p.bias != nullptr) {
        const float* b = p.bias + c0;
#pragma unroll
        for (int j = 0; j < BN / 8; ++j) {
#pragma unroll
            for (int e = 0; e < 2; ++e) {
                if (8 * j + e < ncol) {
                    const float x = __ldg(b + 8 * j + e);
                    acc[4 * j + e] += x;
                    acc[4 * j + 2 + e] += x;
                }
            }
        }
    }
    const float* tab[3][2];
#pragma unroll
    for (int h = 0; h < 2; ++h) {
        const int row = lim[h] > 0 ? r0 + 8 * h : 0;
        tab[0][h] = p.row_bias != nullptr ? p.row_bias + (long)(row / p.rows_per_group) * p.ld_row_bias + c0 : nullptr;
        tab[1][h] = p.gather_bias != nullptr ? p.gather_bias + (long)(lim[h] > 0 ? p.gather_idx[row] : 0) * p.ld_gb + c0 : nullptr;
        tab[2][h] = p.residual != nullptr ? p.residual + (long)row * p.ld_res + c0 : nullptr;
    }
#pragma unroll 1
    for (int t = 0; t < 3; ++t) {
        const float* const t0 = t == 0 ? tab[0][0] : t == 1 ? tab[1][0] : tab[2][0];
        const float* const t1 = t == 0 ? tab[0][1] : t == 1 ? tab[1][1] : tab[2][1];
        if (t0 == nullptr) continue;
#pragma unroll
        for (int j = 0; j < BN / 8; ++j) {
#pragma unroll
            for (int e = 0; e < 4; ++e) {
                const int k = 8 * j + (e & 1);
                if (k < lim[e >> 1]) acc[4 * j + e] += (e >> 1 ? t1 : t0)[k];
            }
        }
    }
    if (p.relu) {
#pragma unroll
        for (int i = 0; i < BN / 2; ++i) acc[i] = fmaxf(acc[i], 0.0f);
    }
}

template <int BN, bool TRACE>
__device__ __forceinline__ void epi_lstm(const TcParams& p, float* acc, int r0, int c0, int lane, int slot) {
    constexpr int kRuns = BN / 32;
    const bool odd = lane & 1;
    const bool upper = lane & 2;
    const int row = r0 + (odd ? 8 : 0);
    const int u0 = ((c0 - 2 * (lane & 3)) >> 2) + (upper ? 4 : 0);
    const bool row_ok = row < p.M;
    const bool full = u0 + 8 * (kRuns - 1) + 4 <= p.H;
    int src = row;
    if (p.src_row != nullptr && row_ok) src = p.src_row[row];
    const float* cprev = (row_ok && src >= 0 && p.c_prev != nullptr) ? p.c_prev + (long)src * p.ld_cprev + u0 : nullptr;
    float cp[BN / 8];
    if (cprev != nullptr && full && (reinterpret_cast<uintptr_t>(cprev) & 15) == 0) {
#pragma unroll
        for (int k = 0; k < kRuns; ++k) {
            const float4 v = *reinterpret_cast<const float4*>(cprev + 8 * k);
            cp[4 * k] = v.x; cp[4 * k + 1] = v.y; cp[4 * k + 2] = v.z; cp[4 * k + 3] = v.w;
        }
    } else {
#pragma unroll
        for (int i = 0; i < BN / 8; ++i) {
            const int du = 8 * (i / 4) + i % 4;
            cp[i] = (cprev != nullptr && u0 + du < p.H) ? cprev[du] : 0.0f;
        }
    }
    if (TRACE && slot >= 0) {
        float s = 0.0f;
#pragma unroll
        for (int i = 0; i < BN / 8; ++i) s += cp[i];
        asm volatile("" ::"f"(s));
        CAPB_TRACE(slot);
    }
    __syncwarp();
#pragma unroll
    for (int j = 0; j < BN / 8; ++j) {
        float* v = acc + 4 * j;
        const float s0 = __shfl_xor_sync(0xffffffffu, odd ? v[0] : v[2], 1);
        const float s1 = __shfl_xor_sync(0xffffffffu, odd ? v[1] : v[3], 1);
        const float gi = odd ? s0 : v[0], gf = odd ? s1 : v[1], gg = odd ? v[2] : s0, go = odd ? v[3] : s1;
        v[0] = gi; v[1] = gf; v[2] = gg; v[3] = go;
    }
#pragma unroll
    for (int k = 0; k < kRuns; ++k) {
#pragma unroll
        for (int t = 0; t < 2; ++t) {
            float* x = acc + 4 * (4 * k + t);
            float* y = acc + 4 * (4 * k + 2 + t);
#pragma unroll
            for (int g = 0; g < 4; ++g) {
                const float keep = upper ? y[g] : x[g];
                const float recv = __shfl_xor_sync(0xffffffffu, upper ? x[g] : y[g], 2);
                x[g] = upper ? recv : keep;
                y[g] = upper ? keep : recv;
            }
        }
    }
    float cn[BN / 8], hn[BN / 8];
#pragma unroll
    for (int i = 0; i < BN / 8; ++i) {
        const int k = i / 4, o = i % 4;
        const float* g = acc + 4 * (4 * k + (o >> 1) + 2 * (o & 1));
        cn[i] = fast_sigmoid(g[1]) * cp[i] + fast_sigmoid(g[0]) * fast_tanh(g[2]);
        hn[i] = fast_sigmoid(g[3]) * fast_tanh(cn[i]);
    }
    if (TRACE && slot >= 0) {
        float s = 0.0f;
#pragma unroll
        for (int i = 0; i < BN / 8; ++i) s += hn[i];
        asm volatile("" ::"f"(s));
        CAPB_TRACE(slot + 1);
    }
    if (row_ok) {
        float* const c_out = p.c_out + (long)row * p.ld_cout + u0;
        float* const h_f = p.h_f + (long)row * p.ld_h + u0;
        __half* const h_hi = p.h_hi + (long)row * p.ld_h + u0;
        __half* const h_lo = p.h_lo + (long)row * p.ld_h + u0;
        const bool planes = p.h_hi != nullptr;
        const uintptr_t a16 = reinterpret_cast<uintptr_t>(c_out) | reinterpret_cast<uintptr_t>(h_f);
        const uintptr_t a8 = planes ? reinterpret_cast<uintptr_t>(h_hi) | reinterpret_cast<uintptr_t>(h_lo) : 0;
        if (full && (a16 & 15) == 0 && (a8 & 7) == 0) {
#pragma unroll
            for (int k = 0; k < kRuns; ++k) {
                const float* c = cn + 4 * k;
                const float* h = hn + 4 * k;
                *reinterpret_cast<float4*>(c_out + 8 * k) = make_float4(c[0], c[1], c[2], c[3]);
                *reinterpret_cast<float4*>(h_f + 8 * k) = make_float4(h[0], h[1], h[2], h[3]);
                if (planes) {
                    __half hh[4], hl[4];
#pragma unroll
                    for (int o = 0; o < 4; ++o) split_f32(h[o], hh[o], hl[o]);
                    const __half2 hi01 = __halves2half2(hh[0], hh[1]), hi23 = __halves2half2(hh[2], hh[3]);
                    const __half2 lo01 = __halves2half2(hl[0], hl[1]), lo23 = __halves2half2(hl[2], hl[3]);
                    *reinterpret_cast<uint2*>(h_hi + 8 * k) = make_uint2(*reinterpret_cast<const uint32_t*>(&hi01), *reinterpret_cast<const uint32_t*>(&hi23));
                    *reinterpret_cast<uint2*>(h_lo + 8 * k) = make_uint2(*reinterpret_cast<const uint32_t*>(&lo01), *reinterpret_cast<const uint32_t*>(&lo23));
                }
            }
        } else {
#pragma unroll
            for (int i = 0; i < BN / 8; ++i) {
                const int du = 8 * (i / 4) + i % 4;
                if (u0 + du < p.H) {
                    c_out[du] = cn[i];
                    h_f[du] = hn[i];
                    if (planes) {
                        __half hh, hl;
                        split_f32(hn[i], hh, hl);
                        h_hi[du] = hh;
                        h_lo[du] = hl;
                    }
                }
            }
        }
    }
    if (TRACE && slot >= 0) CAPB_TRACE(slot + 2);
}

template <int BN, bool PLANES>
__device__ __forceinline__ void epi_store(const TcParams& p, const float* acc, int r0, int c0) {
    const int ncol = p.N - c0;
#pragma unroll
    for (int h = 0; h < 2; ++h) {
        const int row = r0 + 8 * h;
        if (row >= p.M) continue;
        if (p.C != nullptr) {
            float* const dst = p.C + (long)row * p.ldc + c0;
            if (ncol >= BN && (reinterpret_cast<uintptr_t>(dst) & 7) == 0) {
#pragma unroll
                for (int j = 0; j < BN / 8; ++j) *reinterpret_cast<float2*>(dst + 8 * j) = make_float2(acc[4 * j + 2 * h], acc[4 * j + 2 * h + 1]);
            } else {
#pragma unroll
                for (int j = 0; j < BN / 8; ++j) {
                    if (8 * j < ncol) dst[8 * j] = acc[4 * j + 2 * h];
                    if (8 * j + 1 < ncol) dst[8 * j + 1] = acc[4 * j + 2 * h + 1];
                }
            }
        }
        if (PLANES) {
            __half* const dh = p.C_hi + (long)row * p.ldcs + c0;
            __half* const dl = p.C_lo + (long)row * p.ldcs + c0;
            if (ncol >= BN && ((reinterpret_cast<uintptr_t>(dh) | reinterpret_cast<uintptr_t>(dl)) & 3) == 0) {
#pragma unroll
                for (int j = 0; j < BN / 8; ++j) {
                    __half h0, l0, h1, l1;
                    split_f32(acc[4 * j + 2 * h], h0, l0);
                    split_f32(acc[4 * j + 2 * h + 1], h1, l1);
                    *reinterpret_cast<__half2*>(dh + 8 * j) = __halves2half2(h0, h1);
                    *reinterpret_cast<__half2*>(dl + 8 * j) = __halves2half2(l0, l1);
                }
            } else {
#pragma unroll
                for (int j = 0; j < BN / 8; ++j) {
#pragma unroll
                    for (int e = 0; e < 2; ++e) {
                        __half hi, lo;
                        split_f32(acc[4 * j + 2 * h + e], hi, lo);
                        if (8 * j + e < ncol) { dh[8 * j + e] = hi; dl[8 * j + e] = lo; }
                    }
                }
            }
        }
    }
}

template <int BN, int EPI, bool TRACE>
__device__ __forceinline__ void epilogue_tile(const TcParams& p, float* acc, int m0, int n0, int tid, int slot) {
    const int warp = tid >> 5, lane = tid & 31;
    const int r0 = m0 + warp * 16 + (lane >> 2);
    const int c0 = n0 + 2 * (lane & 3);
    epi_adds<BN>(p, acc, r0, c0);
    if (EPI == kEpiLstm) epi_lstm<BN, TRACE>(p, acc, r0, c0, lane, slot);
    else epi_store<BN, EPI == kEpiPlanes>(p, acc, r0, c0);
}

template <int BN, int EPI, bool TRACE>
__device__ __forceinline__ void epilogue_rows128(const TcParams& p, float* acc0, const float* acc1, int m0, int n0, int tid, int slot) {
#pragma unroll 1
    for (int h = 0; h < 2; ++h) {
        epilogue_tile<BN, EPI, TRACE>(p, acc0, m0 + 64 * h, n0, tid, h == 0 ? slot : -1);
#pragma unroll
        for (int i = 0; i < BN / 2; ++i) acc0[i] = acc1[i];
    }
}

template <int PASSES>
__device__ __forceinline__ void init_ring(const TcParams& p, uint64_t* full_bar, uint64_t* empty_bar, int stages, int readers) {
    for (int s = 0; s < p.nseg; ++s) {
        ptx::prefetch_tmap(&p.a_hi[s]);
        ptx::prefetch_tmap(&p.w_hi[s]);
        if (PASSES == 3) {
            ptx::prefetch_tmap(&p.a_lo[s]);
            ptx::prefetch_tmap(&p.w_lo[s]);
        }
    }
    for (int i = 0; i < stages; ++i) {
        ptx::mbar_init(&full_bar[i], 1);
        ptx::mbar_init(&empty_bar[i], readers);
    }
}

template <typename Cfg>
__device__ __forceinline__ void fill_stage(const TcParams& p, uint8_t* st, uint64_t* bar, int s, int kb, int m0, int n0) {
    uint8_t* a_hi = st;
    uint8_t* a_lo = st + Cfg::kABytes;
    uint8_t* w_hi = st + Cfg::kABytes * Cfg::kPlanes;
    uint8_t* w_lo = w_hi + Cfg::kWBytes;
    ptx::mbar_arrive_expect_tx(bar, Cfg::kStageBytes);
#pragma unroll
    for (int r = 0; r < Cfg::kTileM; r += BM) ptx::tma_load_2d(a_hi + r * BK * 2, &p.a_hi[s], bar, kb * BK, m0 + r);
    ptx::tma_load_2d(w_hi, &p.w_hi[s], bar, kb * BK, n0);
    if (Cfg::kPasses == 3) {
#pragma unroll
        for (int r = 0; r < Cfg::kTileM; r += BM) ptx::tma_load_2d(a_lo + r * BK * 2, &p.a_lo[s], bar, kb * BK, m0 + r);
        ptx::tma_load_2d(w_lo, &p.w_lo[s], bar, kb * BK, n0);
    }
}

template <int BN, int PASSES>
__device__ __forceinline__ void mma_kblock(float* acc0, float* acc1, uint32_t a_hi, uint32_t a_lo, uint32_t w_hi, uint32_t w_lo) {
    constexpr uint32_t kHalf = 64 * 128;
#pragma unroll
    for (int i = 0; i < BN / 2; ++i) { ptx::reg_fence(acc0[i]); ptx::reg_fence(acc1[i]); }
    ptx::wgmma_fence();
#pragma unroll
    for (int k = 0; k < BK / 16; ++k) {
        const uint32_t koff = k * 32;
        const uint64_t dwh = ptx::make_smem_desc_sw128(w_hi + koff);
        if (PASSES == 3) {
            const uint64_t dwl = ptx::make_smem_desc_sw128(w_lo + koff);
            wgmma_f16<BN>(acc0, ptx::make_smem_desc_sw128(a_hi + koff), dwl, 1);
            wgmma_f16<BN>(acc1, ptx::make_smem_desc_sw128(a_hi + kHalf + koff), dwl, 1);
            wgmma_f16<BN>(acc0, ptx::make_smem_desc_sw128(a_lo + koff), dwh, 1);
            wgmma_f16<BN>(acc1, ptx::make_smem_desc_sw128(a_lo + kHalf + koff), dwh, 1);
            wgmma_f16<BN>(acc0, ptx::make_smem_desc_sw128(a_hi + koff), dwh, 1);
            wgmma_f16<BN>(acc1, ptx::make_smem_desc_sw128(a_hi + kHalf + koff), dwh, 1);
        } else {
            wgmma_f16<BN>(acc0, ptx::make_smem_desc_sw128(a_hi + koff), dwh, 1);
            wgmma_f16<BN>(acc1, ptx::make_smem_desc_sw128(a_hi + kHalf + koff), dwh, 1);
        }
    }
    ptx::wgmma_commit();
    ptx::wgmma_wait<0>();
#pragma unroll
    for (int i = 0; i < BN / 2; ++i) { ptx::reg_fence(acc0[i]); ptx::reg_fence(acc1[i]); }
}

template <int BN, int PASSES, int EPI, bool TRACE = false>
__global__ void __launch_bounds__(kThreads, 1) gemm_tc_kernel(const __grid_constant__ TcParams p) {
    using Cfg = TcCfg<BN, PASSES>;
    extern __shared__ uint8_t smem_raw[];
    uint8_t* smem = reinterpret_cast<uint8_t*>((reinterpret_cast<uintptr_t>(smem_raw) + 1023) & ~uintptr_t(1023));
    uint64_t* full_bar = reinterpret_cast<uint64_t*>(smem + Cfg::kStages * Cfg::kStageBytes);
    uint64_t* empty_bar = full_bar + Cfg::kStages;
    uint64_t* turn_bar = empty_bar + Cfg::kStages;

    const int wg = threadIdx.x >> 7;
    const int n_tiles = p.tiles_m * p.tiles_n;

    if (threadIdx.x == 0) {
        init_ring<PASSES>(p, full_bar, empty_bar, Cfg::kStages, 1);
        for (int c = 0; c < kConsumers; ++c) ptx::mbar_init(&turn_bar[c], 1);
        ptx::fence_mbar_init();
    }
    __syncthreads();
    if (threadIdx.x == 0) CAPB_TRACE(0);

    if (wg == 0) {
        ptx::setmaxnreg_dec<40>();
        if (threadIdx.x == 0) {
            int stage = 0;
            uint32_t phase = 0;
            for (int t = blockIdx.x; t < n_tiles; t += gridDim.x) {
                const int m0 = (t % p.tiles_m) * BM;
                const int n0 = (t / p.tiles_m) * BN;
                for (int s = 0; s < p.nseg; ++s) {
                    for (int kb = 0; kb < p.kblocks[s]; ++kb) {
                        ptx::mbar_wait(&empty_bar[stage], phase ^ 1);
                        fill_stage<Cfg>(p, smem + stage * Cfg::kStageBytes, &full_bar[stage], s, kb, m0, n0);
                        if (++stage == Cfg::kStages) { stage = 0; phase ^= 1; }
                    }
                }
            }
        }
    } else {
        ptx::setmaxnreg_inc<232>();
        const int cw = wg - 1;
        const int tid = threadIdx.x & 127;
        int kb_tile = 0;
        for (int s = 0; s < p.nseg; ++s) kb_tile += p.kblocks[s];
        int mine = 0;
        for (int it = cw, t = blockIdx.x + cw * gridDim.x; t < n_tiles; it += 2, t += 2 * gridDim.x, ++mine) {
            const int m0 = (t % p.tiles_m) * BM;
            const int n0 = (t / p.tiles_m) * BN;
            if (it > 0) ptx::mbar_wait(&turn_bar[cw], (cw == 1 ? mine : mine - 1) & 1);
            if (TRACE && it == 1 && tid == 0) CAPB_TRACE(4);
            const long g0 = (long)it * kb_tile;
            int stage = (int)(g0 % Cfg::kStages);
            uint32_t phase = (uint32_t)(g0 / Cfg::kStages) & 1;
            float acc0[BN / 2], acc1[BN / 2];
#pragma unroll
            for (int i = 0; i < BN / 2; ++i) { acc0[i] = 0.0f; acc1[i] = 0.0f; }
            for (int s = 0; s < p.nseg; ++s) {
                for (int kb = 0; kb < p.kblocks[s]; ++kb) {
                    ptx::mbar_wait(&full_bar[stage], phase);
                    if (TRACE && it == 0 && s == 0 && kb == 0 && tid == 0) CAPB_TRACE(1);
                    const uint32_t st = ptx::smem_u32(smem + stage * Cfg::kStageBytes);
                    const uint32_t w_hi = st + Cfg::kABytes * Cfg::kPlanes;
                    mma_kblock<BN, PASSES>(acc0, acc1, st, st + Cfg::kABytes, w_hi, w_hi + Cfg::kWBytes);
                    if (tid == 0) ptx::mbar_arrive(&empty_bar[stage]);
                    if (++stage == Cfg::kStages) { stage = 0; phase ^= 1; }
                }
            }
            if (tid == 0) ptx::mbar_arrive(&turn_bar[cw ^ 1]);
            if (TRACE && it < 2 && tid == 0) CAPB_TRACE(2 + it);
            epilogue_rows128<BN, EPI, TRACE>(p, acc0, acc1, m0, n0, tid, (TRACE && it < 2 && tid == 0) ? 9 + 3 * it : -1);
            if (TRACE && it < 2 && tid == 0) CAPB_TRACE(6 + it);
        }
    }
    __syncthreads();
    if (threadIdx.x == 0) CAPB_TRACE(8);
}

template <int BN, int PASSES, int EPI, bool TRACE = false>
__global__ void __launch_bounds__(kThreads, 1) gemm_tc256_kernel(const __grid_constant__ TcParams p) {
    using Cfg = TcCfg<BN, PASSES, 2 * BM>;
    extern __shared__ uint8_t smem_raw[];
    uint8_t* smem = reinterpret_cast<uint8_t*>((reinterpret_cast<uintptr_t>(smem_raw) + 1023) & ~uintptr_t(1023));
    uint64_t* full_bar = reinterpret_cast<uint64_t*>(smem + Cfg::kStages * Cfg::kStageBytes);
    uint64_t* empty_bar = full_bar + Cfg::kStages;

    const int wg = threadIdx.x >> 7;
    const int n_tiles = p.tiles_m * p.tiles_n;

    if (threadIdx.x == 0) {
        init_ring<PASSES>(p, full_bar, empty_bar, Cfg::kStages, kConsumers);
        ptx::fence_mbar_init();
    }
    __syncthreads();
    if (threadIdx.x == 0) CAPB_TRACE(0);

    if (wg == 0) {
        ptx::setmaxnreg_dec<40>();
        if (threadIdx.x == 0) {
            int stage = 0;
            uint32_t phase = 0;
            for (int t = blockIdx.x; t < n_tiles; t += gridDim.x) {
                const int m0 = (t % p.tiles_m) * Cfg::kTileM;
                const int n0 = (t / p.tiles_m) * BN;
                for (int s = 0; s < p.nseg; ++s) {
                    for (int kb = 0; kb < p.kblocks[s]; ++kb) {
                        ptx::mbar_wait(&empty_bar[stage], phase ^ 1);
                        fill_stage<Cfg>(p, smem + stage * Cfg::kStageBytes, &full_bar[stage], s, kb, m0, n0);
                        if (++stage == Cfg::kStages) { stage = 0; phase ^= 1; }
                    }
                }
                if (TRACE && t == (int)blockIdx.x) CAPB_TRACE(5);
            }
        }
    } else {
        ptx::setmaxnreg_inc<232>();
        const int cw = wg - 1;
        const int tid = threadIdx.x & 127;
        const uint32_t a_rows = cw * BM * BK * 2;
        int stage = 0;
        uint32_t phase = 0;
        for (int it = 0, t = blockIdx.x; t < n_tiles; ++it, t += gridDim.x) {
            const int m0 = (t % p.tiles_m) * Cfg::kTileM + BM * cw;
            const int n0 = (t / p.tiles_m) * BN;
            float acc0[BN / 2], acc1[BN / 2];
#pragma unroll
            for (int i = 0; i < BN / 2; ++i) { acc0[i] = 0.0f; acc1[i] = 0.0f; }
            for (int s = 0; s < p.nseg; ++s) {
                for (int kb = 0; kb < p.kblocks[s]; ++kb) {
                    ptx::mbar_wait(&full_bar[stage], phase);
                    if (TRACE && it == 0 && s == 0 && kb == 0 && cw == 0 && tid == 0) CAPB_TRACE(1);
                    const uint32_t st = ptx::smem_u32(smem + stage * Cfg::kStageBytes);
                    const uint32_t w_hi = st + Cfg::kABytes * Cfg::kPlanes;
                    mma_kblock<BN, PASSES>(acc0, acc1, st + a_rows, st + Cfg::kABytes + a_rows, w_hi, w_hi + Cfg::kWBytes);
                    if (tid == 0) ptx::mbar_arrive(&empty_bar[stage]);
                    if (++stage == Cfg::kStages) { stage = 0; phase ^= 1; }
                }
            }
            if (TRACE && it == 0 && tid == 0) CAPB_TRACE(2 + cw);
            epilogue_rows128<BN, EPI, TRACE>(p, acc0, acc1, m0, n0, tid, (TRACE && it == 0 && tid == 0) ? 9 + 3 * cw : -1);
            if (TRACE && it == 0 && tid == 0) CAPB_TRACE(6 + cw);
        }
    }
    __syncthreads();
    if (threadIdx.x == 0) CAPB_TRACE(8);
}

typedef CUresult (*EncodeTiledFn)(CUtensorMap*, CUtensorMapDataType, cuuint32_t, void*, const cuuint64_t*, const cuuint64_t*,
                                  const cuuint32_t*, const cuuint32_t*, CUtensorMapInterleave, CUtensorMapSwizzle,
                                  CUtensorMapL2promotion, CUtensorMapFloatOOBfill);

EncodeTiledFn get_encode_fn() {
    static EncodeTiledFn fn = nullptr;
    if (fn == nullptr) {
        void* sym = nullptr;
        cudaDriverEntryPointQueryResult qres;
        if (cudaGetDriverEntryPoint("cuTensorMapEncodeTiled", &sym, cudaEnableDefault, &qres) != cudaSuccess || sym == nullptr) {
            return nullptr;
        }
        fn = reinterpret_cast<EncodeTiledFn>(sym);
    }
    return fn;
}

bool encode_plane(CUtensorMap* map, const __half* base, long rows, long K, long pitch, int box_rows, std::string* err) {
    EncodeTiledFn fn = get_encode_fn();
    if (fn == nullptr) { *err = "cuTensorMapEncodeTiled entry point not available"; return false; }
    cuuint64_t gdim[2] = {static_cast<cuuint64_t>(K), static_cast<cuuint64_t>(rows)};
    cuuint64_t gstride[1] = {static_cast<cuuint64_t>(pitch) * 2};
    cuuint32_t box[2] = {static_cast<cuuint32_t>(BK), static_cast<cuuint32_t>(box_rows)};
    cuuint32_t estr[2] = {1, 1};
    CUresult r = fn(map, CU_TENSOR_MAP_DATA_TYPE_FLOAT16, 2, const_cast<__half*>(base), gdim, gstride, box, estr,
                    CU_TENSOR_MAP_INTERLEAVE_NONE, CU_TENSOR_MAP_SWIZZLE_128B, CU_TENSOR_MAP_L2_PROMOTION_L2_256B,
                    CU_TENSOR_MAP_FLOAT_OOB_FILL_NONE);
    if (r != CUDA_SUCCESS) { *err = "cuTensorMapEncodeTiled failed with CUresult " + std::to_string((int)r); return false; }
    return true;
}

template <int BN, int PASSES, int EPI, bool TRACE, int TM>
int launch_cfg(const TcParams& prm, cudaStream_t stream) {
    using Cfg = TcCfg<BN, PASSES, TM>;
    void (*kernel)(TcParams);
    if constexpr (TM == BM) kernel = gemm_tc_kernel<BN, PASSES, EPI, TRACE>;
    else kernel = gemm_tc256_kernel<BN, PASSES, EPI, TRACE>;
    static std::atomic<unsigned long long> attr_set{0};
    if (first_use_on_device(attr_set)) {
        CAPB_CHECK_CUDA(cudaFuncSetAttribute(kernel, cudaFuncAttributeMaxDynamicSharedMemorySize, Cfg::kSmemBytes));
    }
    TcParams prm2 = prm;
    prm2.tiles_n = cdiv(prm.N, BN);
    prm2.tiles_m = cdiv(prm.M, TM);
    const int n_tiles = prm2.tiles_n * prm2.tiles_m;
    const int sms = sm_count();
    kernel<<<n_tiles < sms ? n_tiles : sms, kThreads, Cfg::kSmemBytes, stream>>>(prm2);
    CAPB_CHECK_CUDA(cudaGetLastError());
    return 0;
}

template <int EPI, int TM>
int launch_width(int bn, int passes, const TcParams& prm, cudaStream_t stream) {
    if (prm.trace != nullptr) {
        if (bn == 160) return launch_cfg<160, 3, EPI, true, TM>(prm, stream);
        if constexpr (TM == BM) if (bn == 64) return launch_cfg<64, 3, EPI, true, TM>(prm, stream);
        return launch_cfg<128, 3, EPI, true, TM>(prm, stream);
    }
    if (bn == 160) return passes == 3 ? launch_cfg<160, 3, EPI, false, TM>(prm, stream) : launch_cfg<160, 1, EPI, false, TM>(prm, stream);
    if constexpr (TM == BM) {
        if (bn == 64) return passes == 3 ? launch_cfg<64, 3, EPI, false, TM>(prm, stream) : launch_cfg<64, 1, EPI, false, TM>(prm, stream);
    }
    return passes == 3 ? launch_cfg<128, 3, EPI, false, TM>(prm, stream) : launch_cfg<128, 1, EPI, false, TM>(prm, stream);
}

template <int EPI>
int launch_kind(int bm, int bn, int passes, const TcParams& prm, cudaStream_t stream) {
    return bm == 2 * BM ? launch_width<EPI, 2 * BM>(bn, passes, prm, stream) : launch_width<EPI, BM>(bn, passes, prm, stream);
}

}

struct GemmTcPlan {
    TcParams prm;
    int passes;
    int bn;
};

static void fill_epilogue(TcParams& t, const GemmEpilogue& e) {
    t.C = e.C; t.ldc = e.ldc;
    t.C_hi = e.C_hi; t.C_lo = e.C_lo; t.ldcs = e.ldcs;
    t.bias = e.bias; t.row_bias = e.row_bias; t.ld_row_bias = e.ld_row_bias;
    t.rows_per_group = e.rows_per_group < 1 ? 1 : e.rows_per_group;
    t.relu = e.relu;
    t.residual = e.residual; t.ld_res = e.ld_res;
    t.lstm = e.lstm; t.H = e.H;
    t.c_prev = e.c_prev; t.ld_cprev = e.ld_cprev; t.src_row = e.src_row;
    t.c_out = e.c_out; t.ld_cout = e.ld_cout;
    t.gather_bias = e.gather_bias; t.ld_gb = e.ld_gb; t.gather_idx = e.gather_idx;
    t.h_f = e.h_f; t.h_hi = e.h_hi; t.h_lo = e.h_lo; t.ld_h = e.ld_h;
    t.trace = e.trace;
}

bool gemm_tc_supported(const GemmProblem& p, std::string* why) {
    auto bad = [&](const char* m) { if (why) *why = m; return false; };
    if (p.nseg < 1 || p.nseg > kMaxSeg) return bad("1..3 K-segments");
    for (int s = 0; s < p.nseg; ++s) {
        const GemmSeg& g = p.seg[s];
        if (g.A_hi == nullptr || g.W_hi == nullptr) return bad("split planes missing");
        if ((g.lda_h & 7) || (g.ldw_h & 7)) return bad("plane pitch must be a multiple of 8 elements (16 bytes)");
        if ((reinterpret_cast<uintptr_t>(g.A_hi) & 15) || (reinterpret_cast<uintptr_t>(g.W_hi) & 15)) return bad("plane base must be 16-byte aligned");
        if (g.K < 1) return bad("empty K-segment");
    }
    return true;
}

int gemm_tc_tile_n(int M, int N) {
    const int sms = sm_count();
    const int tiles_m = cdiv(M, BM);
    if (tiles_m * cdiv(N, 128) < sms / 2 && N > 64) return 64;
    const long cost128 = (long)cdiv(tiles_m * cdiv(N, 128), sms) * 128;
    const long cost160 = (long)cdiv(tiles_m * cdiv(N, 160), sms) * 160;
    return cost160 < cost128 ? 160 : 128;
}

int gemm_tc_tile_m(int M, int N, int bn) {
    if (bn == 64) return BM;
    const char* force = getenv("CAPB200_GEMM_BM");
    if (force != nullptr && strcmp(force, "128") == 0) return BM;
    if (force != nullptr && strcmp(force, "256") == 0) return 2 * BM;
    const int sms = sm_count();
    const int tiles_n = cdiv(N, bn);
    return cdiv(M, 2 * BM) * tiles_n <= sms && cdiv(M, BM) * tiles_n > sms ? 2 * BM : BM;
}

GemmTcPlan* gemm_tc_plan_create(const GemmProblem& p, int passes) {
    std::string why;
    if (!gemm_tc_supported(p, &why)) { set_error("gemm_tc: unsupported problem: " + why); return nullptr; }
    if (passes != 1 && passes != 3) { set_error("gemm_tc: passes must be 1 or 3"); return nullptr; }
    GemmTcPlan* plan = new GemmTcPlan();
    memset(&plan->prm, 0, sizeof(TcParams));
    plan->passes = passes;
    plan->bn = gemm_tc_tile_n(p.M, p.N);
    TcParams& t = plan->prm;
    t.nseg = p.nseg;
    t.M = p.M;
    t.N = p.N;
    std::string err;
    for (int s = 0; s < p.nseg; ++s) {
        const GemmSeg& g = p.seg[s];
        t.kblocks[s] = cdiv(g.K, BK);
        bool ok = encode_plane(&t.a_hi[s], g.A_hi, p.M, g.K, g.lda_h, BM, &err) &&
                  encode_plane(&t.w_hi[s], g.W_hi, p.N, g.K, g.ldw_h, plan->bn, &err);
        if (ok && passes == 3) {
            if (g.A_lo == nullptr || g.W_lo == nullptr) { err = "lo planes missing for 3-pass mode"; ok = false; }
            ok = ok && encode_plane(&t.a_lo[s], g.A_lo, p.M, g.K, g.lda_h, BM, &err) &&
                 encode_plane(&t.w_lo[s], g.W_lo, p.N, g.K, g.ldw_h, plan->bn, &err);
        }
        if (!ok) { set_error("gemm_tc: " + err); delete plan; return nullptr; }
    }
    fill_epilogue(t, p.epi);
    return plan;
}

void gemm_tc_plan_destroy(GemmTcPlan* plan) { delete plan; }

int gemm_tc_plan_launch(GemmTcPlan* plan, const GemmEpilogue* epi_override, int M_override, cudaStream_t stream) {
    if (M_override > plan->prm.M) { set_error("gemm_tc: M override exceeds the planned row count"); return 1; }
    const int M = M_override > 0 ? M_override : plan->prm.M;
    TcParams prm = plan->prm;
    if (epi_override != nullptr) fill_epilogue(prm, *epi_override);
    prm.M = M;
    if (prm.lstm && (prm.N != 4 * prm.H || prm.c_out == nullptr || prm.h_f == nullptr)) {
        set_error("gemm_tc: fused LSTM epilogue needs N == 4H, c_out and h_f");
        return 1;
    }
    if (prm.M <= 0 || prm.N <= 0) return 0;
    const int kind = prm.lstm ? kEpiLstm : prm.C_hi != nullptr ? kEpiPlanes : kEpiStore;
    if (prm.trace != nullptr && plan->passes != 3) { set_error("gemm_tc: the traced kernel is the 3-pass one"); return 1; }
    const int bm = gemm_tc_tile_m(prm.M, prm.N, plan->bn);
    if (kind == kEpiLstm) return launch_kind<kEpiLstm>(bm, plan->bn, plan->passes, prm, stream);
    if (kind == kEpiPlanes) return launch_kind<kEpiPlanes>(bm, plan->bn, plan->passes, prm, stream);
    return launch_kind<kEpiStore>(bm, plan->bn, plan->passes, prm, stream);
}

}
```

imagecaptioning.pytorch_b200/csrc/kernels.cuh:

```cuda
#pragma once
#include "common.cuh"

namespace capb200 {

struct ActView {
    float* f = nullptr;
    __half* hi = nullptr;
    __half* lo = nullptr;
    long ld = 0;
};

struct StateCopy {
    const float* src = nullptr;
    long ld_src = 0;
    ActView dst;
};

__device__ __forceinline__ void copy_states4(long r, int src, int c4, int nstate, const StateCopy& sc0, const StateCopy& sc1) {
    float4 v0 = make_float4(0.f, 0.f, 0.f, 0.f), v1 = v0;
    if (src >= 0) {
        v0 = *reinterpret_cast<const float4*>(sc0.src + (long)src * sc0.ld_src + 4 * c4);
        if (nstate > 1) v1 = *reinterpret_cast<const float4*>(sc1.src + (long)src * sc1.ld_src + 4 * c4);
    }
    for (int s = 0; s < nstate; ++s) {
// ... 13 lines not shown
int state_gather_embed_launch(int rows, const int* tokens, const int* src_row, const float* emb, long ld_emb, int E, int relu,
                              ActView xt, int H, int nstate, StateCopy sc0, StateCopy sc1, cudaStream_t stream);
int lstm_pointwise_launch(int rows, int H, const float* gates, long ld_g, const int* src_row, const float* c_prev, long ld_cp,
                          float* c_out, long ld_co, ActView h_out, const float* gather_bias, long ld_gb, const int* gather_idx,
                          cudaStream_t stream);
int relu_copy_launch(const float* x, long n, ActView out_flat, cudaStream_t stream);
int lstm_ln_launch(int rows, int H, const float* gates, long ld_g, const float* c_prev, long ld_cp, float* c_out, long ld_co, float* h_out, long ld_h,
                   const float* ln_a, const float* ln_b, float eps, float* ln_out, long ld_ln, cudaStream_t stream);
int maxout_pointwise_launch(int rows, int H, const float* sums, long ld_s, const int* src_row, const float* c_prev, long ld_cp,
                            float* c_out, long ld_co, ActView h_out, cudaStream_t stream);
int additive_attention_launch(int n_images, int rpi, int R, int A, int H, const float* att_h, long ld_ah, const float* p_att, long ld_pa,
                              const float* att, long ld_at, const float* mask, long ld_mask, const float* alpha_w, const float* alpha_b,
                              float* score_scratch , ActView out, cudaStream_t stream, float* alpha_out = nullptr );
int mask_rows_launch(ActView x, int n_images, int R, int cols, const float* mask, long ld_mask, cudaStream_t stream);
int ss_select_launch(int rows, int V1, const float* prev_logp, long ld, const long long* labels, long ld_labels, int col, unsigned long long seed, float prob,
                     int* tok_out, cudaStream_t stream);

struct DecodeEdits {
    int constraint = 0;
    int unk_col = -1;
    int n_bad = 0;
    const int* bad = nullptr;
    int trigrams = 0;
    int trigram_rows = 0;
    __host__ __device__ bool any() const { return constraint != 0 || unk_col >= 0 || n_bad > 0 || trigrams != 0; }
    __host__ __device__ int kinds() const { return (constraint ? 1 : 0) + (unk_col >= 0 ? 1 : 0) + (n_bad > 0 ? 1 : 0); }
};

struct VocabStepArgs {
    int rows = 0;
    int V1 = 0;
    float* logits = nullptr;
    long ld = 0;
    int twice = 0;
    float2* stats = nullptr;
    int topk = 0;
    float* top_val = nullptr;
    int* top_idx = nullptr;
    int select = 0;
    float top = 0.f;
    DecodeEdits edits;
    const int* prev_tokens = nullptr;
    float temperature = 1.0f;
    unsigned long long seed = 0;
    unsigned long long step = 0;
    const int* forced = nullptr;
    int* unfinished = nullptr;
    int first_step = 0;
    int* tokens_out = nullptr;
    long long* seq_out = nullptr;
    long ld_seq = 0;
    int t = 0;
    float* picked_lp = nullptr;
    long ld_picked = 1;
    int first_beam = 0, first_group_rows = 1, first_group = -1;
    __host__ __device__ int row_twice(int r) const {
        return twice && !(first_beam > 0 && (r % first_beam) / first_group_rows == first_group);
    }
};
int vocab_step_launch(const VocabStepArgs& a, cudaStream_t stream);
int beam_edit_launch(int rows, int k_in, int beam, int t, const DecodeEdits& ed, const int* prev_tokens, const float* val_in, const int* idx_in,
                     float* val_out, int* idx_out, cudaStream_t stream, int first_beam = 0, int first_group_rows = 1, int first_group = -1);
int scale_rows_launch(float* x, long ld, int rows, int cols, float factor, cudaStream_t stream, int skip_beam = 0, int skip_group_rows = 1,
                      int skip_group = -1);

struct BeamState {
    int B = 0, beam = 0, T = 0, V1 = 0;
    float* sums = nullptr;
    int* seq_a = nullptr;
    int* seq_b = nullptr;
    int* hist_a = nullptr;
    int* hist_b = nullptr;
    int* done_cnt = nullptr;
    int* done_seq = nullptr;
    int* done_hist = nullptr;
    int* done_len = nullptr;
    double* done_p = nullptr;
    float* done_raw = nullptr;
    int* tokens = nullptr;
    int* src_row = nullptr;
};
int beam_step_launch(const BeamState& s, int t, int live, const float* top_val, const int* top_idx, int penalty_kind, float penalty_alpha,
                     cudaStream_t stream);
struct NextStateGather {
    StateCopy s0, s1;
    int H = 0;
};
bool beam_search_step_applies(const VocabStepArgs& a, const NextStateGather& next);
int beam_search_step_launch(const BeamState& s, const VocabStepArgs& a, int t, int live, int penalty_kind, float penalty_alpha,
                            const NextStateGather& next, cudaStream_t stream);
int diverse_beam_step_launch(const BeamState& s, int G, int t, int k, const float* top_val, const int* top_idx, float lambda, int rows_total,
                             int penalty_kind, float penalty_alpha, cudaStream_t stream);
int beam_finalize_launch(const BeamState& s, int keep, long long* out_seq, int* out_len, float* out_p, float* out_raw, int* out_hist,
                         cudaStream_t stream);
int gather_logprob_rows_launch(const float* slab, long step_stride, long ld_slab, const int* hist, int nseq, int T, int V1, float* dst,
                               const float2* stats, long stats_stride, cudaStream_t stream, const long long* seqs = nullptr,
                               const DecodeEdits* ed = nullptr);

int layer_norm_launch(int rows, int D, const float* x, long ld_x, const float* a, const float* b, float eps, ActView out, cudaStream_t st);
int embed_pe_launch(int rows, int D, const int* tokens, const float* lut, const float* pe_row, float scale, ActView out, cudaStream_t st);
int enc_self_attention_launch(int B, int R, int heads, int dk, const float* q, const float* k, const float* v, long ld, const float* mask,
                              long ld_mask, ActView out, cudaStream_t st, int form = 0);
int dec_self_attention_launch(int rows, int heads, int dk, int t, const float* qkv, long ld_qkv, float* kcache, float* vcache, long step_stride,
                              long ld_c, const int* anc, long ld_anc, const long long* labels, long ld_lab, ActView out, cudaStream_t st, int form = 0);
int cross_attention_launch(int rows, int rpi, int heads, int dk, int R, const float* q, long ld_q, const float* kk, const float* vv, long ld_kv,
                           const float* mask, long ld_mask, ActView out, cudaStream_t st);

int glu_launch(int rows, int H, const float* t, long ld_t, const float* residual, long ld_res, ActView out, cudaStream_t st);
int masked_mean_launch(int B, int R, int H, const float* x, long ld_x, const float* mask, long ld_mask, ActView out, cudaStream_t st);

int gemm_generic_launch(int ta, int tb, int M, int N, int K, const float* A, long lda, const float* B, long ldb, float* C, long ldc, int accumulate,
                        const float* bias, cudaStream_t st);
int gemm_skinny_launch(int M, int N, int nseg, const float* const* A, const long* lda, const float* const* B, const long* ldb, const int* K, const int* tb,
                       float* C, long ldc, const float* bias, const float* row_bias, long ld_rb, int rpg, int accumulate, float* scratch,
                       size_t scratch_floats, int mode, cudaStream_t st);
int gemm_wgrad_launch(int M, int N, int K, const float* dY, long ld_dy, const float* X, long ld_x, float* G, long ld_g, int accumulate, int mode,
                      cudaStream_t st);
int colsum_launch(int rows, int cols, const float* x, long ld, float* out, int accumulate, cudaStream_t st);
struct Tf32Context;
Tf32Context* tf32_context_create();
void tf32_context_destroy(Tf32Context* c);
void tf32_context_new_step(Tf32Context* c);
long tf32_context_launches(const Tf32Context* c);
bool gemm_tf32_supported(int nseg, const float* const* X, const long* ldx, const float* const* W, const long* ldw, const int* K);
int gemm_tf32_launch(Tf32Context* ctx, int M, int N, int nseg, const float* const* X, const long* ldx, const float* const* W, const long* ldw, const int* K,
                     float* C, long ldc, const float* bias, const float* row_bias, long ld_rb, int rpg, int accumulate, cudaStream_t st);
const float* tf32_transposed(Tf32Context* ctx, const float* src, long ld_src, int rows, int cols, bool per_step, long* ld_dst, cudaStream_t st);
int dropout_apply_launch(float* x, int rows, int cols, long ld, unsigned long long seed, unsigned site, unsigned step, float p, cudaStream_t st);
int relu_dropout_apply_launch(float* x, int rows, int cols, long ld, unsigned long long seed, unsigned site, unsigned step, float p, cudaStream_t st);
int dropout_mask_launch(float* m, long n, unsigned long long seed, unsigned site, unsigned step, float p, cudaStream_t st);
int dropout_copy_launch(const float* x, long ld_x, float* y, long ld_y, int rows, int cols, unsigned long long seed, unsigned site, unsigned step, float p,
                        cudaStream_t st);
int embed_relu_dropout_launch(int rows, int E, const int* tokens, const float* emb, float* xt, unsigned long long seed, unsigned step, float p,
                              cudaStream_t st);
int scst_dlogits_launch(const float* logp, long ld_row, const long long* seq, const float* reward, const float* mask_sum, float upstream, int N, int T, int V1,
                        float* dl, cudaStream_t st, const float* row_coef = nullptr);
int scst_drop_worst_launch(const long long* seq, const float* row_loss, int N, int T, int keep, float upstream, float* row_msum, float* row_coef, float* loss,
                           cudaStream_t st);
int xe_loss_backward_launch(const float* logp, long ld_row, const long long* labels, long ld_l, const float* masks, long ld_m, int N, int steps, int Ls, int V1,
                            float smoothing, float upstream, float* mask_sum, float* item_loss, float* dl, float* loss, cudaStream_t st, int keep = 0,
                            float* row_loss = nullptr, float* row_msum = nullptr, float* row_coef = nullptr);
struct PpoScratch {
    float* terms;
    float* row_msum;
    float* row_coef;
    float* mask_sum;
};
int ppo_shift_launch(const long long* seq, int N, int T, long long* tokens_in, cudaStream_t st);
int ppo_loss_backward_launch(const float* lp, long ld_lp, const float* lo, const long long* seq, const float* adv, const double* scores, int N, int T, int V1,
                             float cliprange, float kl_coef, float upstream, int keep, const PpoScratch& s, float* dl, float* scores_out, float* loss,
                             float* row_loss, float* pg_loss, float* kl_loss, float* clipfrac, cudaStream_t st);
int logsoftmax_vjp_launch(const float* logp, const float* g, long ld_row, const long long* seq, int N, int T, int V1, float* dl, cudaStream_t st);
int lstm_cell_backward_launch(int rows, int H, const float* gates, const float* c_prev, const float* c_new, const float* dh, const float* dh_extra,
                              long ld_extra, unsigned drop_site, unsigned drop_step, unsigned long long seed, float p, float* dc_carry, float* dgates,
                              cudaStream_t st);
int maxout_cell_backward_launch(int rows, int H, const float* sums, const float* c_prev, const float* c_new, const float* dh, const float* dh_extra,
                                long ld_extra, unsigned drop_site, unsigned drop_step, unsigned long long seed, float p, float* dc_carry, float* dsums,
                                cudaStream_t st);
int attention_backward_launch(int n_images, int rpi, int R, int A, int H, const float* d_out, const float* alpha, const float* att_h, const float* p_att,
                              const float* att, const float* w, float* d_att_h, float* d_att, float* d_p_att, float* d_w, float* d_b, float* d_alpha_scratch,
                              cudaStream_t st);
int relu_dropout_backward_launch(long n, const float* x, const float* dy, float* dx, float scale, cudaStream_t st);
int embed_backward_launch(int rows, int E, const int* tokens, const float* xt, const float* dxt, long ld_dxt, float scale, float* d_emb, cudaStream_t st);
int embed_scatter_launch(int rows, int E, const int* tokens, const float* dxt, long ld_dxt, float* d_emb, cudaStream_t st);
int per_image_sum_launch(int steps, int rows, int rpi, int cols, const float* x, float* out, cudaStream_t st);
int add_strided_launch(float* a, const float* b, long ld_b, int rows, int cols, cudaStream_t st);

int ln_backward_launch(int rows, int D, const float* x, long ld_x, const float* a, const float* dy, long ld_dy, float eps, float* dx, long ld_dx, int accumulate,
                       float* stats, float* da, float* db, int accumulate_params, cudaStream_t st, const float* add1 = nullptr, long ld_a1 = 0,
// ... 84 lines not shown
```

imagecaptioning.pytorch_b200/csrc/pointwise.cu:

```cuda
#include "common.cuh"
#include "kernels.cuh"

namespace capb200 {

static int pw_blocks(long total) {
    long b = (total + 255) / 256;
    return (int)(b > sm_count() * 8 ? sm_count() * 8 : b);
}

namespace {

__device__ __forceinline__ float sigmoidf_(float x) { return fast_sigmoid(x); }

__device__ __forceinline__ void store_act(const ActView& o, long row, int col, float v) {
    o.f[row * o.ld + col] = v;
    if (o.hi != nullptr) {
        __half h, l;
        split_f32(v, h, l);
        o.hi[row * o.ld + col] = h;
        o.lo[row * o.ld + col] = l;
    }
}

__global__ void state_gather_embed_kernel(int rows, const int* __restrict__ tokens, const int* __restrict__ src_row,
                                          const float* __restrict__ emb, long ld_emb, int E, int relu, ActView xt,
                                          int H, int nstate, StateCopy sc0, StateCopy sc1) {
    const int r = blockIdx.x;
    if (r >= rows) return;
    const int tok = tokens[r];
    const float* e = emb + (long)tok * ld_emb;
    for (int c = threadIdx.x; c < E; c += blockDim.x) {
        float v = __ldg(e + c);
        if (relu) v = fmaxf(v, 0.f);
        store_act(xt, r, c, v);
    }
    const int src = src_row ? src_row[r] : r;
    const bool vec = (H & 3) == 0 && (sc0.ld_src & 3) == 0 && (sc0.dst.ld & 3) == 0 && (nstate < 2 || ((sc1.ld_src & 3) == 0 && (sc1.dst.ld & 3) == 0));
    if (vec) {
        for (int c4 = threadIdx.x; c4 < (H >> 2); c4 += blockDim.x) copy_states4(r, src, c4, nstate, sc0, sc1);
        return;
    }
    for (int s = 0; s < nstate; ++s) {
        const StateCopy& sc = (s == 0) ? sc0 : sc1;
        for (int c = threadIdx.x; c < H; c += blockDim.x) {
            const float v = (src < 0) ? 0.f : sc.src[(long)src * sc.ld_src + c];
            store_act(sc.dst, r, c, v);
        }
    }
}

__global__ void lstm_pointwise_kernel(int rows, int H, const float* __restrict__ gates, long ld_g, const int* __restrict__ src_row,
                                      const float* __restrict__ c_prev, long ld_cp, float* __restrict__ c_out, long ld_co, ActView h_out,
                                      const float* __restrict__ gather_bias, long ld_gb, const int* __restrict__ gather_idx) {
    const long total = (long)rows * H;
    for (long i = blockIdx.x * (long)blockDim.x + threadIdx.x; i < total; i += (long)gridDim.x * blockDim.x) {
        const int r = (int)(i / H), c = (int)(i % H);
        const float* g = gates + (long)r * ld_g;
        float gi = g[c], gf = g[H + c], gg = g[2 * H + c], go = g[3 * H + c];
        if (gather_bias != nullptr) {
            const float* gb = gather_bias + (long)gather_idx[r] * ld_gb;
            gi += __ldg(gb + c); gf += __ldg(gb + H + c); gg += __ldg(gb + 2 * H + c); go += __ldg(gb + 3 * H + c);
        }
        const int src = src_row ? src_row[r] : r;
        const float cp = (src < 0 || c_prev == nullptr) ? 0.f : c_prev[(long)src * ld_cp + c];
        const float cn = sigmoidf_(gf) * cp + sigmoidf_(gi) * fast_tanh(gg);
        const float hn = sigmoidf_(go) * fast_tanh(cn);
        c_out[(long)r * ld_co + c] = cn;
        store_act(h_out, r, c, hn);
    }
}

__global__ void __launch_bounds__(256) lstm_ln_kernel(int H, const float* __restrict__ gates, long ld_g, const float* __restrict__ c_prev, long ld_cp,
                                                      float* __restrict__ c_out, long ld_co, float* __restrict__ h_out, long ld_h, const float* __restrict__ ln_a,
                                                      const float* __restrict__ ln_b, float eps, float* __restrict__ ln_out, long ld_ln) {
    __shared__ float sh[8];
    const int r = blockIdx.x;
    const float* g = gates + (long)r * ld_g;
    float hv[8];
    float s = 0.f;
#pragma unroll
    for (int u = 0; u < 8; ++u) {
        const int c = threadIdx.x + 256 * u;
        hv[u] = 0.f;
        if (c < H) {
            const float gi = g[c], gf = g[H + c], gg = g[2 * H + c], go = g[3 * H + c];
            const float cp = c_prev == nullptr ? 0.f : c_prev[(long)r * ld_cp + c];
            const float cn = sigmoidf_(gf) * cp + sigmoidf_(gi) * fast_tanh(gg);
            const float hn = sigmoidf_(go) * fast_tanh(cn);
            c_out[(long)r * ld_co + c] = cn;
            h_out[(long)r * ld_h + c] = hn;
            hv[u] = hn;
            s += hn;
        }
    }
    auto bsum = [&](float v) {
#pragma unroll
        for (int o = 16; o > 0; o >>= 1) v += __shfl_xor_sync(0xffffffffu, v, o);
        __syncthreads();
        if ((threadIdx.x & 31) == 0) sh[threadIdx.x >> 5] = v;
        __syncthreads();
        return ((sh[0] + sh[1]) + (sh[2] + sh[3])) + ((sh[4] + sh[5]) + (sh[6] + sh[7]));
    };
    const float mean = bsum(s) / (float)H;
    float q = 0.f;
// ... 108 lines not shown
}

constexpr int ATT_CT = 256;
__global__ void __launch_bounds__(ATT_CT) att_combine_kernel(int rpi, int R, int H, const float* __restrict__ score, const float* __restrict__ att,
                                                             long ld_at, const float* __restrict__ mask, long ld_mask, ActView out,
                                                             float* __restrict__ alpha_out) {
    extern __shared__ float s_w[];
    const int img = blockIdx.x;
    const int c = blockIdx.y * ATT_CT + threadIdx.x;
    const int warp = threadIdx.x >> 5, lane = threadIdx.x & 31;
    for (int j0 = 0; j0 < rpi; j0 += ATT_JB) {
        const int nj = min(ATT_JB, rpi - j0);
        __syncthreads();
        if (warp < nj) {
            const float* sc = score + ((long)img * rpi + j0 + warp) * R;
            float* w = s_w + warp * R;
            float mx = -INFINITY;
            for (int r = lane; r < R; r += 32) mx = fmaxf(mx, sc[r]);
#pragma unroll
            for (int o = 16; o > 0; o >>= 1) mx = fmaxf(mx, __shfl_xor_sync(0xffffffffu, mx, o));
            float sum = 0.f;
            for (int r = lane; r < R; r += 32) { const float e = expf(sc[r] - mx); w[r] = e; sum += e; }
#pragma unroll
            for (int o = 16; o > 0; o >>= 1) sum += __shfl_xor_sync(0xffffffffu, sum, o);
            const float inv = 1.0f / sum;
            float msum = 0.f;
            for (int r = lane; r < R; r += 32) {
                float v = w[r] * inv;
                if (mask != nullptr) { v *= mask[(long)img * ld_mask + r]; msum += v; }
                w[r] = v;
            }
            if (mask != nullptr) {
#pragma unroll
                for (int o = 16; o > 0; o >>= 1) msum += __shfl_xor_sync(0xffffffffu, msum, o);
                for (int r = lane; r < R; r += 32) w[r] = w[r] / msum;
            }
        }
        __syncthreads();
        if (alpha_out != nullptr && blockIdx.y == 0) {
            for (int i = threadIdx.x; i < nj * R; i += ATT_CT) alpha_out[((long)img * rpi + j0) * R + i] = s_w[i];
        }
        if (c < H) {
            float acc[ATT_JB];
#pragma unroll
            for (int j = 0; j < ATT_JB; ++j) acc[j] = 0.f;
            const float* ap = att + (long)img * R * ld_at + c;
            for (int r = 0; r < R; ++r) {
                const float v = __ldg(ap + (long)r * ld_at);
#pragma unroll
                for (int j = 0; j < ATT_JB; ++j)
                    if (j < nj) acc[j] = fmaf(s_w[j * R + r], v, acc[j]);
            }
#pragma unroll
            for (int j = 0; j < ATT_JB; ++j)
                if (j < nj) store_act(out, (long)img * rpi + j0 + j, c, acc[j]);
        }
    }
}

__global__ void relu_copy_kernel(const float* __restrict__ x, long n, ActView out_flat) {
    for (long i = blockIdx.x * (long)blockDim.x + threadIdx.x; i < n; i += (long)gridDim.x * blockDim.x) {
        const float v = fmaxf(__ldg(x + i), 0.f);
        out_flat.f[i] = v;
        if (out_flat.hi) { __half h, l; split_f32(v, h, l); out_flat.hi[i] = h; out_flat.lo[i] = l; }
    }
}

}

int relu_copy_launch(const float* x, long n, ActView out_flat, cudaStream_t stream) {
    relu_copy_kernel<<<pw_blocks(n), 256, 0, stream>>>(x, n, out_flat);
    CAPB_CHECK_CUDA(cudaGetLastError());
    return 0;
}

int state_gather_embed_launch(int rows, const int* tokens, const int* src_row, const float* emb, long ld_emb, int E, int relu,
                              ActView xt, int H, int nstate, StateCopy sc0, StateCopy sc1, cudaStream_t stream) {
    if (rows <= 0) return 0;
    state_gather_embed_kernel<<<rows, 256, 0, stream>>>(rows, tokens, src_row, emb, ld_emb, E, relu, xt, H, nstate, sc0, sc1);
    CAPB_CHECK_CUDA(cudaGetLastError());
    return 0;
}


int lstm_pointwise_launch(int rows, int H, const float* gates, long ld_g, const int* src_row, const float* c_prev, long ld_cp,
                          float* c_out, long ld_co, ActView h_out, const float* gather_bias, long ld_gb, const int* gather_idx,
                          cudaStream_t stream) {
    if (rows <= 0) return 0;
    lstm_pointwise_kernel<<<pw_blocks((long)rows * H), 256, 0, stream>>>(rows, H, gates, ld_g, src_row, c_prev, ld_cp, c_out, ld_co, h_out,
                                                                          gather_bias, ld_gb, gather_idx);
    CAPB_CHECK_CUDA(cudaGetLastError());
    return 0;
}

int lstm_ln_launch(int rows, int H, const float* gates, long ld_g, const float* c_prev, long ld_cp, float* c_out, long ld_co, float* h_out, long ld_h,
                   const float* ln_a, const float* ln_b, float eps, float* ln_out, long ld_ln, cudaStream_t stream) {
    if (rows <= 0) return 0;
    CAPB_REQUIRE(H <= 2048, "lstm_ln: hidden size above 2048");
    lstm_ln_kernel<<<rows, 256, 0, stream>>>(H, gates, ld_g, c_prev, ld_cp, c_out, ld_co, h_out, ld_h, ln_a, ln_b, eps, ln_out, ld_ln);
    CAPB_CHECK_CUDA(cudaGetLastError());
    return 0;
}

int maxout_pointwise_launch(int rows, int H, const float* sums, long ld_s, const int* src_row, const float* c_prev, long ld_cp,
                            float* c_out, long ld_co, ActView h_out, cudaStream_t stream) {
    if (rows <= 0) return 0;
    maxout_pointwise_kernel<<<pw_blocks((long)rows * H), 256, 0, stream>>>(rows, H, sums, ld_s, src_row, c_prev, ld_cp, c_out, ld_co, h_out);
    CAPB_CHECK_CUDA(cudaGetLastError());
    return 0;
}

int additive_attention_launch(int n_images, int rpi, int R, int A, int H, const float* att_h, long ld_ah, const float* p_att, long ld_pa,
                              const float* att, long ld_at, const float* mask, long ld_mask, const float* alpha_w, const float* alpha_b,
                              float* score_scratch, ActView out, cudaStream_t stream, float* alpha_out) {
    if (n_images <= 0 || rpi <= 0) return 0;
    CAPB_REQUIRE(A <= 1024, "attention: att_hid_size above 1024");
    CAPB_REQUIRE(score_scratch != nullptr, "attention: score scratch missing");
    const int na = cdiv(A, 32);
    dim3 sgrid(cdiv(R, ATT_SW), n_images);
#define CAPB_ATT_CASE(NA_)                                                                                                             \
    att_score_kernel<NA_><<<sgrid, ATT_SW * 32, sizeof(float) * (ATT_JB + 1) * NA_ * 32, stream>>>(rpi, R, A, att_h, ld_ah, p_att, ld_pa, alpha_w, \
                                                                                               alpha_b, score_scratch)
    if (na <= 2) CAPB_ATT_CASE(2);
    else if (na <= 4) CAPB_ATT_CASE(4);
    else if (na <= 8) CAPB_ATT_CASE(8);
    else if (na <= 16) CAPB_ATT_CASE(16);
    else CAPB_ATT_CASE(32);
#undef CAPB_ATT_CASE
    CAPB_CHECK_CUDA(cudaGetLastError());
    const size_t smem = sizeof(float) * (size_t)ATT_JB * R;
    CAPB_REQUIRE(smem <= 48 * 1024, "attention: too many regions");
    dim3 grid(n_images, cdiv(H, ATT_CT));
    att_combine_kernel<<<grid, ATT_CT, smem, stream>>>(rpi, R, H, score_scratch, att, ld_at, mask, ld_mask, out, alpha_out);
    CAPB_CHECK_CUDA(cudaGetLastError());
    return 0;
}

}
```

imagecaptioning.pytorch_b200/models.py:

```python
from __future__ import annotations

import ctypes
import threading
from collections.abc import Mapping
from typing import Optional

import torch
import torch.nn as nn

from . import _lib

BAD_ENDINGS = ['a', 'an', 'the', 'in', 'for', 'at', 'of', 'with', 'before', 'after', 'on', 'upon', 'near', 'to', 'is', 'are', 'am', 'the']

_PENALTY = {'': 0, 'wu': 1, 'avg': 2}


class _DoneBeam(Mapping):

    def __init__(self, owner, image, rank, seq, p, raw):
        self._owner, self._image, self._rank = owner, image, rank
        self._seq, self._p, self._raw = seq, p, raw
        self._logps = None

    def _materialise(self):
# ... 227 lines not shown
            for key in path[:-1]:
                dst = getattr(dst, key) if isinstance(key, str) else dst[key]
            setattr(dst, path[-1], t.data_ptr())

    def _grad_table(self, lib, device, slots=None):
        slots = self._grad_slots() if slots is None else slots
        fg = self._flat_grads(device, slots)
        g = self._grads_struct()
        self._fill_struct(g, [(path, fg.by_name[_slot_name(path)]) for path, _ in slots])
        self._bind_head_grads(lib, [fg.by_name[n] for n, _ in self._head_named()], True)
        table, n = fg.event_table() if getattr(self, '_grad_sync_on', False) else (None, 0)
        _lib.check(getattr(lib, 'capb200_%s_set_grad_events' % self._abi)(self._engine, table, n), '%s_set_grad_events' % self._abi)
        return fg, g

    def _bind_key(self, tensors):
        if getattr(self, '_is_replica', False) or any(not t.is_leaf for t in tensors):
            return None
        return tuple((t.data_ptr(), t._version) for t in tensors)

    def _ensure_engine(self, device):
        lib = self._enter_device(device)
        key = (_tls.dev, self.numeric_mode)
        if self._engine is None or self._engine_key != key:
            self._destroy_engine()
            cfg = self._cfg()
            with torch.cuda.device(device):
                eng = getattr(lib, 'capb200_%s_create' % self._abi)(ctypes.byref(cfg))
            if not eng:
                raise RuntimeError('capb200 %s_create failed: %s' % (self._abi, lib.capb200_last_error().decode()))
            self._engine, self._engine_key, self._bound_versions = eng, key, None
            if self._head_named():
                _lib.check(getattr(lib, 'capb200_%s_set_logit_layers' % self._abi)(eng, self.logit_layers), '%s_set_logit_layers' % self._abi)
        slots = self._slots()
        head = self._head_named()
        versions = self._bind_key([t for _, t in slots] + [t for _, t in head])
        if versions is None or versions != self._bound_versions:
            keep = []
            for name, t in [(_slot_name(path), t) for path, t in slots] + head:
                if t.device != device or t.dtype != torch.float32:
                    raise RuntimeError('capb200: parameter %s must be a float32 tensor on %s' % (name, device))
                keep.append(t.detach().contiguous())
            w = self._weights_struct()
            self._fill_struct(w, [(path, t) for (path, _), t in zip(slots, keep)])
            _lib.check(getattr(lib, 'capb200_%s_bind_weights' % self._abi)(self._engine, ctypes.byref(w), _lib.current_stream()),
                       '%s_bind_weights' % self._abi)
            if head:
                hk = keep[len(slots):]
                ws = (ctypes.c_void_p * (len(hk) // 2))(*[t.data_ptr() for t in hk[0::2]])
                bs = (ctypes.c_void_p * (len(hk) // 2))(*[t.data_ptr() for t in hk[1::2]])
                _lib.check(getattr(lib, 'capb200_%s_bind_logit_head' % self._abi)(self._engine, ws, bs, _lib.current_stream()),
                           '%s_bind_logit_head' % self._abi)
            self._keepalive = keep
            self._bound_versions = versions
        return lib

    def _cfg(self):
        return _lib.ModelCfg(self.family, self.vocab_size, self.input_encoding_size, self.rnn_size, self.att_hid_size, self.fc_feat_size,
                             self.att_feat_size, self.seq_length, _lib.MODES[self.numeric_mode])

    def _free_engine(self, handle):
        getattr(_lib.load(), 'capb200_%s_destroy' % self._abi)(handle)

    def _destroy_engine(self):
        if self._engine is not None:
            self._free_engine(self._engine)
            self._engine = None

    def __del__(self):
        try:
            store = self.__dict__.get('_store')
            if store is None or store.owner != id(self):
                return
            for slot in store.slots.values():
                if slot['engine'] is not None:
                    self._free_engine(slot['engine'])
                    slot['engine'] = None
        except Exception:
            pass

    @property
    def launch_count(self) -> int:
        return 0 if self._engine is None else int(getattr(_lib.load(), 'capb200_%s_launch_count' % self._abi)(self._engine))

    GEMM_IDS = ('fc_embed', 'att_embed', 'ctx2att', 'fc_gate_bias', 'att_lstm', 'h2att', 'lang_lstm', 'logit', 'newfc_core')

    def set_profiling(self, enable: bool):
        _lib.check(_lib.load().capb200_engine_set_profiling(self._engine, int(enable)), 'set_profiling')

    def read_profile(self, reset=True):
        import numpy as np
        ms, fl, calls = np.zeros(9), np.zeros(9), np.zeros(9, dtype=np.int64)
        _lib.check(_lib.load().capb200_engine_read_profile(self._engine, int(reset), ms.ctypes.data, fl.ctypes.data, calls.ctypes.data, 9), 'read_profile')
        return {n: (float(ms[i]), float(fl[i]), int(calls[i])) for i, n in enumerate(self.GEMM_IDS)}

    def forward(self, *args, **kwargs):
        mode = kwargs.pop('mode', 'forward')
        return getattr(self, '_' + mode)(*args, **kwargs)

    @staticmethod
    def _f32(t):
        return None if t is None else t.detach().to(torch.float32).contiguous()

    def _clip(self, att_feats, att_masks):
        if att_masks is not None:
            max_len = int(att_masks.detach().long().sum(1).max().item())
            att_feats = att_feats[:, :max_len]
            att_masks = att_masks[:, :max_len]
        return self._f32(att_feats), self._f32(att_masks)

    _no_diverse = None

    def _check_opts(self, opt, beam_size=None, sample_n=None):
        group_size = opt.get('group_size', 1)
        if group_size != 1:
            if beam_size is None or beam_size <= 1:
                raise NotImplementedError('diverse sampling (group_size > 1 with beam_size 1, AttModel._diverse_sample) is out of scope of the engine')
            if self._no_diverse is not None:
                raise NotImplementedError('diverse beam search is not implemented for %s: %s' % (self.family_name, self._no_diverse))
            if group_size < 1 or beam_size % group_size != 0:
                raise NotImplementedError('diverse beam search needs group_size dividing beam_size (got %r, %r)' % (beam_size, group_size))
            if sample_n not in (1, beam_size // group_size):
                raise NotImplementedError('diverse beam search returns sample_n = 1 or beam_size // group_size captions per image (AttModel.py:223)')
            if float(opt.get('diversity_lambda', 0.5)) < 0:
                raise NotImplementedError('diverse beam search needs diversity_lambda >= 0 on the engine (its candidate lists rely on the '
                                          'penalty only lowering log-probs)')
        if opt.get('output_logsoftmax', 1) != 1:
            raise NotImplementedError('output_logsoftmax=0 is out of scope of the engine')

    def _decode_edits(self, opt, device, beam, batch_size=0):
        ed = _lib.DecodeEdits.none()
        keep = None
        ed.decoding_constraint = 1 if opt.get('decoding_constraint', 0) else 0
        if opt.get('remove_bad_endings', 0) and self.bad_endings_ix:
            keep = torch.tensor(sorted(set(self.bad_endings_ix)), dtype=torch.int32, device=device)
            ed.n_bad_endings, ed.bad_endings = keep.numel(), keep.data_ptr()
        if beam:
            if opt.get('suppress_UNK', 0) and self.vocab.get(str(self.vocab_size)) == 'UNK':
                ed.unk_col = self.vocab_size
            elif self.unk_idx is not None:
                ed.unk_col = int(self.unk_idx)
            if opt.get('block_trigrams', 0):
                pass
        elif opt.get('block_trigrams', 0):
            ed.block_trigrams, ed.trigram_rows = 1, int(batch_size)
        return ed, keep

    @_on_device
    def _sample(self, fc_feats, att_feats, att_masks=None, opt={}, forced_tokens=None):
        sample_method = opt.get('sample_method', 'greedy')
        beam_size = opt.get('beam_size', 1)
        temperature = float(opt.get('temperature', 1.0))
        sample_n = int(opt.get('sample_n', 1))
        if self._autograd_active():
            return self._sample_autograd(fc_feats, att_feats, att_masks, opt, forced_tokens)
        if beam_size > 1 and sample_method in ('greedy', 'beam_search'):
            return self._sample_beam(fc_feats, att_feats, att_masks, opt)
        self._check_opts(opt)
        top = 0.0
        if forced_tokens is not None:
            method = _lib.SAMPLE_FORCED
        else:
            method, top, gumbel = sampling_method(sample_method)
            if gumbel:
                temperature = 1.0
        lib = self._ensure_engine(fc_feats.device)
        fc = self._f32(fc_feats)
        att, masks = self._clip(att_feats, att_masks)
        B = fc.shape[0]
        R = att.shape[1] if att is not None and att.dim() == 3 else 1
        N, T, V1 = B * sample_n, self.seq_length, self.vocab_size + 1
        seq = torch.empty(N, T, dtype=torch.long, device=fc.device)
        logprobs = torch.empty(N, T, V1, dtype=torch.float32, device=fc.device)
        draws = method in (_lib.SAMPLE_MULTINOMIAL, _lib.SAMPLE_TOPK, _lib.SAMPLE_TOPP)
        seed = int(torch.randint(0, 2 ** 62, (1,)).item()) if draws else 0
        edits, keep_bad = self._decode_edits(opt, fc.device, beam=False, batch_size=B)
# ... 849 lines not shown
```

Measured before the change: 25070.

## Fuse next-step attention-LSTM gate GEMM into logit GEMM and beam-step cell

During beam search, the part of the next step's attention-LSTM gate GEMM that depends only on the previous states (h1_out and h0_out) is computed in the same grouped tensor-core launch as the logit GEMM. The result goes to a new q_att buffer. The fused beam-step kernel then applies the LSTM cell itself, adding the per-image fc bias and the per-token gate table to the gathered q_att rows. This removes the separate att-LSTM GEMM and pointwise launch from the following step. In exchange it adds a grouped-GEMM plan path with a catch-up tile schedule, more work in the beam-step kernel, and more threads per block.

```diff
diff --git a/imagecaptioning.pytorch_b200/csrc/beam.cu b/imagecaptioning.pytorch_b200/csrc/beam.cu
--- a/imagecaptioning.pytorch_b200/csrc/beam.cu
+++ b/imagecaptioning.pytorch_b200/csrc/beam.cu
@@ -139,11 +139,27 @@
     if (threadIdx.x < 32) select_step<U>(s, img, t, live, b, row0, row0, s_val, s_idx, nullptr, 0, 0.f, penalty_kind, penalty_alpha, done_p);
     if (t == s.T - 1) return;
     __syncthreads();
-    const int n4 = next.H >> 2;
+    const int H = next.H, n4 = H >> 2;
+    const NextCell& nc = next.cell;
+    const bool cell = nc.q != nullptr;
     for (int i = threadIdx.x; i < b * n4; i += blockDim.x) {
         const int j = i / n4, c4 = i - j * n4;
         const long r = (long)img * b + j;
-        copy_states4(r, s.src_row[r], c4, 2, next.s0, next.s1);
+        if (cell) copy_states4(r, s.src_row[r], c4, 1, next.s1, next.s1);
+        else copy_states4(r, s.src_row[r], c4, 2, next.s0, next.s1);
+    }
+    if (!cell) return;
+    const float* const c_prev = nc.c[(t + 1) & 1];
+    float* const c_out = nc.c[t & 1];
+    const int n = b * H, stride = blockDim.x;
+    for (int i = threadIdx.x; i < n; i += 2 * stride) {
+        const int i1 = i + stride < n ? i + stride : i;
+        const int j0 = i / H, u0 = i - j0 * H, j1 = i1 / H, u1 = i1 - j1 * H;
+        const long r0 = (long)img * b + j0, r1 = (long)img * b + j1;
+        const CellOperands o0 = next_cell_load(nc, img, s.src_row[r0], s.tokens[r0], u0, c_prev);
+        const CellOperands o1 = next_cell_load(nc, img, s.src_row[r1], s.tokens[r1], u1, c_prev);
+        next_cell_store(nc, r0, u0, o0, c_out);
+        next_cell_store(nc, r1, u1, o1, c_out);
     }
 }
 
@@ -350,6 +366,12 @@
     return 0;
 }
 
+bool next_cell_applies(const NextCell& c) {
+    auto al16 = [](const void* p) { return (reinterpret_cast<uintptr_t>(p) & 15) == 0; };
+    return c.q != nullptr && al16(c.q) && al16(c.row_bias) && al16(c.gather_bias) && ((c.ld_q | c.ld_rb | c.ld_gb) & 3) == 0 && c.c[0] != nullptr &&
+           c.c[1] != nullptr && c.h_out.f != nullptr && c.h_out.hi != nullptr && c.h_out.lo != nullptr;
+}
+
 bool beam_search_step_applies(const VocabStepArgs& a, const NextStateGather& next) {
     auto al16 = [](const void* p) { return (reinterpret_cast<uintptr_t>(p) & 15) == 0; };
     auto al8 = [](const void* p) { return (reinterpret_cast<uintptr_t>(p) & 7) == 0; };
@@ -357,7 +379,9 @@
         return c.src != nullptr && c.dst.f != nullptr && (c.ld_src & 3) == 0 && (c.dst.ld & 3) == 0 && al16(c.src) && al16(c.dst.f) &&
                ((c.dst.hi == nullptr) == (c.dst.lo == nullptr)) && (c.dst.hi == nullptr || (al8(c.dst.hi) && al8(c.dst.lo)));
     };
-    return (a.V1 & 3) == 0 && (a.ld & 3) == 0 && al16(a.logits) && next.H > 0 && (next.H & 3) == 0 && state_ok(next.s0) && state_ok(next.s1);
+    const bool cell_ok = next.cell.q == nullptr || next_cell_applies(next.cell);
+    return (a.V1 & 3) == 0 && (a.ld & 3) == 0 && al16(a.logits) && next.H > 0 && (next.H & 3) == 0 && state_ok(next.s0) && state_ok(next.s1) &&
+           cell_ok;
 }
 
 int beam_search_step_launch(const BeamState& s, const VocabStepArgs& a, int t, int live, int penalty_kind, float penalty_alpha,
@@ -366,7 +390,7 @@
     CAPB_REQUIRE(s.beam * s.T <= MAXB * CAPB200_MAX_SEQ_LENGTH, "beam*T record capacity (16 x CAPB200_MAX_SEQ_LENGTH)");
     CAPB_REQUIRE(a.topk == s.beam && a.stats != nullptr && a.rows == s.B * live && live >= 1 && live <= s.beam, "fused beam step arguments");
     CAPB_REQUIRE(beam_search_step_applies(a, next), "the fused beam step needs 16-byte aligned logit and state rows (V + 1 and H multiples of 4)");
-    const int threads = min(live, kStepGroups) * VT2;
+    const int threads = min(next.cell.q != nullptr ? s.beam : live, kStepGroups) * VT2;
     if (s.beam <= 8) beam_search_step_kernel<2><<<s.B, threads, 0, stream>>>(s, a, t, live, penalty_kind, penalty_alpha, s.done_p, next);
     else beam_search_step_kernel<8><<<s.B, threads, 0, stream>>>(s, a, t, live, penalty_kind, penalty_alpha, s.done_p, next);
     CAPB_CHECK_CUDA(cudaGetLastError());
diff --git a/imagecaptioning.pytorch_b200/csrc/common.cuh b/imagecaptioning.pytorch_b200/csrc/common.cuh
--- a/imagecaptioning.pytorch_b200/csrc/common.cuh
+++ b/imagecaptioning.pytorch_b200/csrc/common.cuh
@@ -104,6 +104,10 @@
     const float e = __expf(2.0f * x);
     return 1.0f - __fdividef(2.0f, 1.0f + e);
 }
+__device__ __forceinline__ void lstm_cell_unit(float gi, float gf, float gg, float go, float c_prev, float& c, float& h) {
+    c = fast_sigmoid(gf) * c_prev + fast_sigmoid(gi) * fast_tanh(gg);
+    h = fast_sigmoid(go) * fast_tanh(c);
+}
 __device__ __forceinline__ void fast_tanh4(const float (&x)[4], float (&t)[4]) {
     float y[4];
 #pragma unroll
@@ -132,6 +136,7 @@
 
 struct GemmTcPlan;
 GemmTcPlan* gemm_tc_plan_create(const GemmProblem& p, int passes);
+GemmTcPlan* gemm_tc_group_plan_create(const GemmProblem& lead, const GemmProblem& p, int passes);
 int gemm_tc_tile_n(int M, int N);
 int gemm_tc_tile_m(int M, int N, int bn);
 void gemm_tc_plan_destroy(GemmTcPlan* plan);
diff --git a/imagecaptioning.pytorch_b200/csrc/engine.cu b/imagecaptioning.pytorch_b200/csrc/engine.cu
--- a/imagecaptioning.pytorch_b200/csrc/engine.cu
+++ b/imagecaptioning.pytorch_b200/csrc/engine.cu
@@ -62,8 +62,8 @@
 }
 
 
-enum GemmId { G_FC = 0, G_ATT, G_CTX, G_GFC, G_LSTM1, G_H2ATT, G_LSTM2, G_LOGIT, G_CORE, G_A2C, G_COUNT };
-constexpr int G_REPORTED = 9;
+enum GemmId { G_FC = 0, G_ATT, G_CTX, G_GFC, G_LSTM1, G_H2ATT, G_LSTM2, G_LOGIT, G_CORE, G_LOGIT_Q, G_A2C, G_COUNT };
+constexpr int G_REPORTED = 10;
 
 }
 }
@@ -85,6 +85,7 @@
 
     Planes in_fc, in_att;
     Act fc_e, att_e, p_att, g_fc, xt, h0_in, h1_in, h0_out, h1_out, att_res, att_h, gates;
+    Act q_att;
     float *c0[2] = {nullptr, nullptr}, *c1[2] = {nullptr, nullptr};
     long ld_c = 0;
     int* img_of_row = nullptr;
@@ -167,6 +168,7 @@
         e->g_fc.carve(a, B, 4 * H, false);
         e->h1_in.carve(a, rows, H, tc);
         e->h1_out.carve(a, rows, H, tc);
+        if (tc) e->q_att.carve(a, rows, 4 * H, false);
     }
     e->xt.carve(a, rows, E, tc);
     e->h0_in.carve(a, rows, H, tc);
@@ -187,8 +189,22 @@
     return e->grow(B, rows, R, beam, st, [&](Arena& a, int nB, int nRows, int nR, int nBeam) { layout_workspace(e, a, nB, nRows, nR, nBeam); });
 }
 
-int run_gemm(capb200_engine* e, int id, GemmProblem& g, int plan_rows, cudaStream_t st) {
-    if (!e->profiling) return e->gemm(id, g, plan_rows, st);
+int gemm_group(capb200_engine* e, int site, const GemmProblem& lead, GemmProblem& g, int plan_rows, cudaStream_t st) {
+    CAPB_REQUIRE(e->tc, "grouped GEMM launches run on the tensor cores");
+    e->launches++;
+    GemmTcPlan*& plan = e->plans[site];
+    if (plan == nullptr) {
+        GemmProblem pl = lead, pg = g;
+        pl.M = plan_rows; pg.M = plan_rows;
+        plan = gemm_tc_group_plan_create(pl, pg, e->mode == CAPB200_MODE_TC_F16X3 ? 3 : 1);
+        if (plan == nullptr) return 1;
+    }
+    return gemm_tc_plan_launch(plan, &g.epi, g.M, st);
+}
+
+int run_gemm(capb200_engine* e, int id, GemmProblem& g, int plan_rows, cudaStream_t st, const GemmProblem* lead = nullptr) {
+    auto launch = [&]() { return lead != nullptr ? gemm_group(e, id, *lead, g, plan_rows, st) : e->gemm(id, g, plan_rows, st); };
+    if (!e->profiling) return launch();
     if (e->ev_used + 2 > e->ev_pool.size()) {
         for (int i = 0; i < 64; ++i) {
             cudaEvent_t ev;
@@ -196,14 +212,17 @@
             e->ev_pool.push_back(ev);
         }
     }
-    double k_total = 0;
-    for (int s = 0; s < g.nseg; ++s) k_total += g.seg[s].K;
+    auto flops = [](const GemmProblem& p) {
+        double k_total = 0;
+        for (int s = 0; s < p.nseg; ++s) k_total += p.seg[s].K;
+        return 2.0 * p.M * p.N * k_total;
+    };
     CAPB_CHECK_CUDA(cudaEventRecord(e->ev_pool[e->ev_used], st));
-    const int rc = e->gemm(id, g, plan_rows, st);
+    const int rc = launch();
     CAPB_CHECK_CUDA(cudaEventRecord(e->ev_pool[e->ev_used + 1], st));
     e->ev_used += 2;
     e->ev_ids.push_back(id);
-    e->ev_flops.push_back(2.0 * g.M * g.N * k_total);
+    e->ev_flops.push_back(flops(g) + (lead != nullptr ? flops(*lead) : 0.0));
     return rc;
 }
 
@@ -274,6 +293,23 @@
     g.epi.bias = e->w.logit_b;
     g.epi.C = logits; g.epi.ldc = ld_logits;
     return run_gemm(e, G_LOGIT, g, e->capRows, st);
+}
+
+int logit_q_gemm(capb200_engine* e, int rows, float* logits, long ld_logits, cudaStream_t st) {
+    const int H = e->H, E = e->E;
+    ActView x;
+    if (e->run_logit_head(e->h1_out.v, rows, &x, st)) return 1;
+    GemmProblem q;
+    q.M = rows; q.N = 4 * H; q.nseg = 2;
+    q.seg[0] = seg_of(e->h1_out.v, e->w.att_lstm_w_ih, E + 2 * H, e->p_a_ih_h, H);
+    q.seg[1] = seg_of(e->h0_out.v, e->w.att_lstm_w_hh, H, e->p_a_hh, H);
+    q.epi.C = e->q_att.v.f; q.epi.ldc = e->q_att.v.ld;
+    GemmProblem g;
+    g.M = rows; g.N = e->V1; g.nseg = 1;
+    g.seg[0] = seg_of(x, e->w.logit_w, H, e->p_logit, H);
+    g.epi.bias = e->w.logit_b;
+    g.epi.C = logits; g.epi.ldc = ld_logits;
+    return run_gemm(e, G_LOGIT_Q, g, e->capRows, st, &q);
 }
 
 int core_step(capb200_engine* e, int rows, int rpi, const int* tokens, const int* src_row, float* logits, long ld_logits, int n_images, int R,
@@ -286,12 +322,20 @@
         s1.src = e->h1_out.v.f; s1.ld_src = e->h1_out.v.ld; s1.dst = e->h1_in.v;
         const bool xg = e->use_xgate;
         CAPB_REQUIRE(!states_gathered || xg, "the fused beam step gathers the states only; the word embedding needs the separate gather");
+        const int cur = e->core_cur, nxt = cur ^ 1;
+        const bool pregated = e->d.pregated;
+        CAPB_REQUIRE(!pregated || (xg && e->tc && src_row != nullptr), "the attention-LSTM cell of a beam step needs the gate table and the tensor cores");
         if (!states_gathered) {
             e->launches++;
-            if (state_gather_embed_launch(rows, tokens, src_row, w.embed, E, xg ? 0 : E, 1, e->xt.v, H, 2, s0, s1, st)) return 1;
-        }
-        const int cur = e->core_cur, nxt = cur ^ 1;
-        {
+            if (pregated) {
+                NextStateGather ns;
+                e->next_state(&ns);
+                if (state_gather_cell_launch(rows, rpi, tokens, src_row, H, s1, ns.cell, e->c0[cur], e->c0[nxt], st)) return 1;
+            } else if (state_gather_embed_launch(rows, tokens, src_row, w.embed, E, xg ? 0 : E, 1, e->xt.v, H, 2, s0, s1, st)) {
+                return 1;
+            }
+        }
+        if (!pregated) {
             GemmProblem g;
             g.M = rows; g.N = 4 * H;
             g.seg[0] = seg_of(e->h1_in.v, w.att_lstm_w_ih, E + 2 * H, e->p_a_ih_h, H);
@@ -350,6 +394,7 @@
                                       nullptr, 0, nullptr, st)) return 1;
         }
         e->core_cur = nxt;
+        if (e->d.pregate_next) return logit_q_gemm(e, rows, logits, ld_logits, st);
         return logit_gemm(e, e->h1_out.v, rows, logits, ld_logits, st);
     }
     if (e->cfg.family == CAPB200_FAMILY_ATT2IN2) {
@@ -502,6 +547,14 @@
     next->s0.src = h0_out.v.f; next->s0.ld_src = h0_out.v.ld; next->s0.dst = h0_in.v;
     next->s1.src = h1_out.v.f; next->s1.ld_src = h1_out.v.ld; next->s1.dst = h1_in.v;
     next->H = H;
+    if (tc) {
+        NextCell& c = next->cell;
+        c.q = q_att.v.f; c.ld_q = q_att.v.ld;
+        c.row_bias = g_fc.v.f; c.ld_rb = g_fc.v.ld;
+        c.gather_bias = xgate; c.ld_gb = ld_xgate;
+        c.c[0] = c0[0]; c.c[1] = c0[1]; c.ld_c = ld_c;
+        c.h_out = h0_out.v;
+    }
     return true;
 }
 
@@ -541,7 +594,7 @@
 }
 
 int capb200_engine_read_profile(capb200_engine* e, int reset, double* ms, double* flops, long* calls, int n) {
-    CAPB_REQUIRE(e != nullptr && n >= G_REPORTED, "need room for 9 GEMM ids");
+    CAPB_REQUIRE(e != nullptr && n >= G_REPORTED, "need room for 10 GEMM ids");
     CAPB_CHECK_CUDA(cudaDeviceSynchronize());
     for (size_t i = 0; i < e->ev_ids.size(); ++i) {
         float t = 0.f;
diff --git a/imagecaptioning.pytorch_b200/csrc/engine_common.cuh b/imagecaptioning.pytorch_b200/csrc/engine_common.cuh
--- a/imagecaptioning.pytorch_b200/csrc/engine_common.cuh
+++ b/imagecaptioning.pytorch_b200/csrc/engine_common.cuh
@@ -116,6 +116,7 @@
     long loop_launches = 0;
     bool graph_broken = false;
     bool states_gathered = false;
+    bool pregated = false, pregate_next = false;
 
     void release() {
         if (loop_exec) cudaGraphExecDestroy(loop_exec);
@@ -244,7 +245,9 @@
     const int k_in = beam + ed.kinds();
     CAPB_REQUIRE(!ed.trigrams, "block_trigrams applies to _sample only (AttModel.py:306)");
     CAPB_REQUIRE(k_in <= 16, "beam_size + number of active decode edits (decoding_constraint, remove_bad_endings, UNK suppression) must be <= 16");
-    CAPB_REQUIRE(form >= 0 && form <= 2, "beam step form must be 0 (automatic), 1 (separate kernels) or 2 (fused)");
+    CAPB_REQUIRE((form & ~4) >= 0 && (form & ~4) <= 2, "beam step form must be 0 (automatic), 1 (separate kernels) or 2 (fused), plus 4 without the cell");
+    const bool no_cell = form & 4;
+    form &= 3;
     if (temperature == 0.f) temperature = 1.0f;
     CAPB_REQUIRE(temperature > 0.f, "temperature must be positive");
     if (grow_buffer(reinterpret_cast<void**>(&d.slab), &d.slab_bytes, (size_t)T * rows * V1 * sizeof(float), st)) return 1;
@@ -253,14 +256,18 @@
     d.last_beam = beam;
     BeamState s = d.bs;
     s.B = B; s.beam = beam; s.T = T; s.V1 = V1;
-    bool fused = false;
+    bool fused = false, cell = false;
+    NextStateGather gather;
     if (form != 1 && next != nullptr && !edits && temperature == 1.0f) {
         VocabStepArgs probe;
         probe.V1 = V1; probe.ld = V1; probe.logits = d.slab;
-        fused = beam_search_step_applies(probe, *next);
-    }
+        gather = *next;
+        gather.cell = NextCell();
+        fused = beam_search_step_applies(probe, gather);
+    }
+    cell = !no_cell && next != nullptr && next_cell_applies(next->cell);
     CAPB_REQUIRE(form != 2 || fused, "the fused beam step needs the engine's state descriptor, no decode edits, temperature 1 and 16-byte aligned "
-                                     "logit and state rows (V + 1 and H multiples of 4)");
+                                    "logit and state rows (V + 1 and H multiples of 4)");
     auto run_loop = [&]() -> int {
         CAPB_NVTX("capb200 beam loop (T steps: core, vocab stats, beam step)");
         CAPB_CHECK_CUDA(cudaMemsetAsync(s.sums, 0, sizeof(float) * B * beam, st));
@@ -271,8 +278,10 @@
             const int nrows = B * live;
             float* logits = d.slab + (long)t * d.slab_step_stride;
             d.states_gathered = fused && t > 0;
+            d.pregated = cell && t > 0;
+            d.pregate_next = cell && t + 1 < T;
             const int rc = core(nrows, live, d.tokens, t == 0 ? d.neg1 : d.src_row, t, logits, (long)V1);
-            d.states_gathered = false;
+            d.states_gathered = d.pregated = d.pregate_next = false;
             if (rc) return 1;
             if (t > 0 && temperature != 1.0f) {
                 if (scale_rows_launch(logits, V1, nrows, V1, 1.0f / temperature, st)) return 1;
@@ -284,7 +293,7 @@
             va.topk = edits ? k_in : beam; va.top_val = d.top_val; va.top_idx = d.top_idx;
             va.stats = d.slab_stats + (long)t * rows;
             if (fused) {
-                if (beam_search_step_launch(s, va, t, live, penalty_kind, penalty_alpha, *next, st)) return 1;
+                if (beam_search_step_launch(s, va, t, live, penalty_kind, penalty_alpha, cell ? *next : gather, st)) return 1;
                 *launches += 1;
                 continue;
             }
@@ -306,7 +315,7 @@
     memcpy(&key[6], &penalty_alpha, sizeof(float));
     memcpy(reinterpret_cast<char*>(&key[6]) + 4, &temperature, sizeof(float));
     key[5] ^= ((unsigned long long)(ed.constraint & 1) << 8) ^ ((unsigned long long)(unsigned)(ed.unk_col + 1) << 16) ^ ((unsigned long long)ed.n_bad << 48);
-    key[5] ^= (unsigned long long)fused << 9;
+    key[5] ^= ((unsigned long long)fused << 9) ^ ((unsigned long long)cell << 10);
     key[0] ^= (unsigned long long)reinterpret_cast<uintptr_t>(ed.bad) * 0x9E3779B97F4A7C15ull;
     d.last_edits = ed;
     d.last_stats = d.slab_stats;
diff --git a/imagecaptioning.pytorch_b200/csrc/gemm_tc.cu b/imagecaptioning.pytorch_b200/csrc/gemm_tc.cu
--- a/imagecaptioning.pytorch_b200/csrc/gemm_tc.cu
+++ b/imagecaptioning.pytorch_b200/csrc/gemm_tc.cu
@@ -48,6 +48,18 @@
     __half* h_lo;
     long ld_h;
     unsigned long long* trace;
+    int lead_nseg;
+    int lead_M, lead_N, lead_tiles_m, lead_tiles;
+    int catch_up;
+    float* lead_C;
+    long lead_ldc;
+};
+
+struct TileOut {
+    int M, N;
+    float* C;
+    long ldc;
+    const float* bias;
 };
 
 __device__ __forceinline__ unsigned long long gtimer() {
@@ -89,11 +101,11 @@
 };
 
 template <int BN>
-__device__ __forceinline__ void epi_adds(const TcParams& p, float* acc, int r0, int c0) {
-    const int ncol = p.N - c0;
-    const int lim[2] = {r0 < p.M ? ncol : 0, r0 + 8 < p.M ? ncol : 0};
-    if (p.bias != nullptr) {
-        const float* b = p.bias + c0;
+__device__ __forceinline__ void epi_adds(const TcParams& p, const TileOut& o, float* acc, int r0, int c0) {
+    const int ncol = o.N - c0;
+    const int lim[2] = {r0 < o.M ? ncol : 0, r0 + 8 < o.M ? ncol : 0};
+    if (o.bias != nullptr) {
+        const float* b = o.bias + c0;
 #pragma unroll
         for (int j = 0; j < BN / 8; ++j) {
 #pragma unroll
@@ -135,13 +147,13 @@
 }
 
 template <int BN, bool TRACE>
-__device__ __forceinline__ void epi_lstm(const TcParams& p, float* acc, int r0, int c0, int lane, int slot) {
+__device__ __forceinline__ void epi_lstm(const TcParams& p, const TileOut& o, float* acc, int r0, int c0, int lane, int slot) {
     constexpr int kRuns = BN / 32;
     const bool odd = lane & 1;
     const bool upper = lane & 2;
     const int row = r0 + (odd ? 8 : 0);
     const int u0 = ((c0 - 2 * (lane & 3)) >> 2) + (upper ? 4 : 0);
-    const bool row_ok = row < p.M;
+    const bool row_ok = row < o.M;
     const bool full = u0 + 8 * (kRuns - 1) + 4 <= p.H;
     int src = row;
     if (p.src_row != nullptr && row_ok) src = p.src_row[row];
@@ -196,8 +208,7 @@
     for (int i = 0; i < BN / 8; ++i) {
         const int k = i / 4, o = i % 4;
         const float* g = acc + 4 * (4 * k + (o >> 1) + 2 * (o & 1));
-        cn[i] = fast_sigmoid(g[1]) * cp[i] + fast_sigmoid(g[0]) * fast_tanh(g[2]);
-        hn[i] = fast_sigmoid(g[3]) * fast_tanh(cn[i]);
+        lstm_cell_unit(g[0], g[1], g[2], g[3], cp[i], cn[i], hn[i]);
     }
     if (TRACE && slot >= 0) {
         float s = 0.0f;
@@ -252,14 +263,14 @@
 }
 
 template <int BN, bool PLANES>
-__device__ __forceinline__ void epi_store(const TcParams& p, const float* acc, int r0, int c0) {
-    const int ncol = p.N - c0;
+__device__ __forceinline__ void epi_store(const TcParams& p, const TileOut& o, const float* acc, int r0, int c0) {
+    const int ncol = o.N - c0;
 #pragma unroll
     for (int h = 0; h < 2; ++h) {
         const int row = r0 + 8 * h;
-        if (row >= p.M) continue;
-        if (p.C != nullptr) {
-            float* const dst = p.C + (long)row * p.ldc + c0;
+        if (row >= o.M) continue;
+        if (o.C != nullptr) {
+            float* const dst = o.C + (long)row * o.ldc + c0;
             if (ncol >= BN && (reinterpret_cast<uintptr_t>(dst) & 7) == 0) {
 #pragma unroll
                 for (int j = 0; j < BN / 8; ++j) *reinterpret_cast<float2*>(dst + 8 * j) = make_float2(acc[4 * j + 2 * h], acc[4 * j + 2 * h + 1]);
@@ -299,20 +310,21 @@
 }
 
 template <int BN, int EPI, bool TRACE>
-__device__ __forceinline__ void epilogue_tile(const TcParams& p, float* acc, int m0, int n0, int tid, int slot) {
+__device__ __forceinline__ void epilogue_tile(const TcParams& p, const TileOut& o, float* acc, int m0, int n0, int tid, int slot) {
     const int warp = tid >> 5, lane = tid & 31;
     const int r0 = m0 + warp * 16 + (lane >> 2);
     const int c0 = n0 + 2 * (lane & 3);
-    epi_adds<BN>(p, acc, r0, c0);
-    if (EPI == kEpiLstm) epi_lstm<BN, TRACE>(p, acc, r0, c0, lane, slot);
-    else epi_store<BN, EPI == kEpiPlanes>(p, acc, r0, c0);
+    epi_adds<BN>(p, o, acc, r0, c0);
+    if (EPI == kEpiLstm) epi_lstm<BN, TRACE>(p, o, acc, r0, c0, lane, slot);
+    else epi_store<BN, EPI == kEpiPlanes>(p, o, acc, r0, c0);
 }
 
 template <int BN, int EPI, bool TRACE>
-__device__ __forceinline__ void epilogue_rows128(const TcParams& p, float* acc0, const float* acc1, int m0, int n0, int tid, int slot) {
+__device__ __forceinline__ void epilogue_rows128(const TcParams& p, const TileOut& o, float* acc0, const float* acc1, int m0, int n0, int tid,
+                                                 int slot) {
 #pragma unroll 1
     for (int h = 0; h < 2; ++h) {
-        epilogue_tile<BN, EPI, TRACE>(p, acc0, m0 + 64 * h, n0, tid, h == 0 ? slot : -1);
+        epilogue_tile<BN, EPI, TRACE>(p, o, acc0, m0 + 64 * h, n0, tid, h == 0 ? slot : -1);
 #pragma unroll
         for (int i = 0; i < BN / 2; ++i) acc0[i] = acc1[i];
     }
@@ -380,6 +392,44 @@
     for (int i = 0; i < BN / 2; ++i) { ptx::reg_fence(acc0[i]); ptx::reg_fence(acc1[i]); }
 }
 
+struct TileAt {
+    int m0, n0, s0, s1;
+    bool lead;
+};
+template <int BN>
+__device__ __forceinline__ TileAt tile_at(const TcParams& p, int t) {
+    TileAt a;
+    a.lead = t < p.lead_tiles;
+    if (a.lead) {
+        a.m0 = (t % p.lead_tiles_m) * BM; a.n0 = (t / p.lead_tiles_m) * BN; a.s0 = 0; a.s1 = p.lead_nseg;
+    } else {
+        t -= p.lead_tiles;
+        a.m0 = (t % p.tiles_m) * BM; a.n0 = (t / p.tiles_m) * BN; a.s0 = p.lead_nseg; a.s1 = p.nseg;
+    }
+    return a;
+}
+__device__ __forceinline__ int tile_of(const TcParams& p, int b, int it) {
+    const int G = gridDim.x;
+    const int nl = b < p.lead_tiles ? (p.lead_tiles - 1 - b) / G + 1 : 0;
+    if (it < nl) return b + it * G;
+    int k = it - nl;
+    const int r = p.lead_tiles % G;
+    const int light = G - r;
+    const int v = b >= r ? b - r : b + light;
+    int j;
+    if (v < light && k < p.catch_up) {
+        j = v + k * light;
+    } else {
+        if (v < light) k -= p.catch_up;
+        j = p.catch_up * light + v + k * G;
+    }
+    return j < p.tiles_m * p.tiles_n ? p.lead_tiles + j : -1;
+}
+
+__device__ __forceinline__ TileOut tile_out(const TcParams& p, bool lead) {
+    return lead ? TileOut{p.lead_M, p.lead_N, p.lead_C, p.lead_ldc, nullptr} : TileOut{p.M, p.N, p.C, p.ldc, p.bias};
+}
+
 template <int BN, int PASSES, int EPI, bool TRACE = false>
 __global__ void __launch_bounds__(kThreads, 1) gemm_tc_kernel(const __grid_constant__ TcParams p) {
     using Cfg = TcCfg<BN, PASSES>;
@@ -390,7 +440,6 @@
     uint64_t* turn_bar = empty_bar + Cfg::kStages;
 
     const int wg = threadIdx.x >> 7;
-    const int n_tiles = p.tiles_m * p.tiles_n;
 
     if (threadIdx.x == 0) {
         init_ring<PASSES>(p, full_bar, empty_bar, Cfg::kStages, 1);
@@ -405,13 +454,12 @@
         if (threadIdx.x == 0) {
             int stage = 0;
             uint32_t phase = 0;
-            for (int t = blockIdx.x; t < n_tiles; t += gridDim.x) {
-                const int m0 = (t % p.tiles_m) * BM;
-                const int n0 = (t / p.tiles_m) * BN;
-                for (int s = 0; s < p.nseg; ++s) {
+            for (int it = 0, t; (t = tile_of(p, blockIdx.x, it)) >= 0; ++it) {
+                const TileAt at = tile_at<BN>(p, t);
+                for (int s = at.s0; s < at.s1; ++s) {
                     for (int kb = 0; kb < p.kblocks[s]; ++kb) {
                         ptx::mbar_wait(&empty_bar[stage], phase ^ 1);
-                        fill_stage<Cfg>(p, smem + stage * Cfg::kStageBytes, &full_bar[stage], s, kb, m0, n0);
+                        fill_stage<Cfg>(p, smem + stage * Cfg::kStageBytes, &full_bar[stage], s, kb, at.m0, at.n0);
                         if (++stage == Cfg::kStages) { stage = 0; phase ^= 1; }
                     }
                 }
@@ -421,21 +469,23 @@
         ptx::setmaxnreg_inc<232>();
         const int cw = wg - 1;
         const int tid = threadIdx.x & 127;
-        int kb_tile = 0;
-        for (int s = 0; s < p.nseg; ++s) kb_tile += p.kblocks[s];
         int mine = 0;
-        for (int it = cw, t = blockIdx.x + cw * gridDim.x; t < n_tiles; it += 2, t += 2 * gridDim.x, ++mine) {
-            const int m0 = (t % p.tiles_m) * BM;
-            const int n0 = (t / p.tiles_m) * BN;
+        long g0 = 0;
+        for (int it = 0, t; (t = tile_of(p, blockIdx.x, it)) >= 0; ++it) {
+            const TileAt at = tile_at<BN>(p, t);
+            int kb_tile = 0;
+            for (int s = at.s0; s < at.s1; ++s) kb_tile += p.kblocks[s];
+            if ((it & 1) != cw) { g0 += kb_tile; continue; }
+            const int m0 = at.m0, n0 = at.n0;
             if (it > 0) ptx::mbar_wait(&turn_bar[cw], (cw == 1 ? mine : mine - 1) & 1);
             if (TRACE && it == 1 && tid == 0) CAPB_TRACE(4);
-            const long g0 = (long)it * kb_tile;
             int stage = (int)(g0 % Cfg::kStages);
             uint32_t phase = (uint32_t)(g0 / Cfg::kStages) & 1;
+            g0 += kb_tile;
             float acc0[BN / 2], acc1[BN / 2];
 #pragma unroll
             for (int i = 0; i < BN / 2; ++i) { acc0[i] = 0.0f; acc1[i] = 0.0f; }
-            for (int s = 0; s < p.nseg; ++s) {
+            for (int s = at.s0; s < at.s1; ++s) {
                 for (int kb = 0; kb < p.kblocks[s]; ++kb) {
                     ptx::mbar_wait(&full_bar[stage], phase);
                     if (TRACE && it == 0 && s == 0 && kb == 0 && tid == 0) CAPB_TRACE(1);
@@ -448,8 +498,9 @@
             }
             if (tid == 0) ptx::mbar_arrive(&turn_bar[cw ^ 1]);
             if (TRACE && it < 2 && tid == 0) CAPB_TRACE(2 + it);
-            epilogue_rows128<BN, EPI, TRACE>(p, acc0, acc1, m0, n0, tid, (TRACE && it < 2 && tid == 0) ? 9 + 3 * it : -1);
+            epilogue_rows128<BN, EPI, TRACE>(p, tile_out(p, at.lead), acc0, acc1, m0, n0, tid, (TRACE && it < 2 && tid == 0) ? 9 + 3 * it : -1);
             if (TRACE && it < 2 && tid == 0) CAPB_TRACE(6 + it);
+            ++mine;
         }
     }
     __syncthreads();
@@ -517,7 +568,7 @@
                 }
             }
             if (TRACE && it == 0 && tid == 0) CAPB_TRACE(2 + cw);
-            epilogue_rows128<BN, EPI, TRACE>(p, acc0, acc1, m0, n0, tid, (TRACE && it == 0 && tid == 0) ? 9 + 3 * cw : -1);
+            epilogue_rows128<BN, EPI, TRACE>(p, tile_out(p, false), acc0, acc1, m0, n0, tid, (TRACE && it == 0 && tid == 0) ? 9 + 3 * cw : -1);
             if (TRACE && it == 0 && tid == 0) CAPB_TRACE(6 + cw);
         }
     }
@@ -569,7 +620,11 @@
     TcParams prm2 = prm;
     prm2.tiles_n = cdiv(prm.N, BN);
     prm2.tiles_m = cdiv(prm.M, TM);
-    const int n_tiles = prm2.tiles_n * prm2.tiles_m;
+    if (prm.lead_nseg > 0) {
+        prm2.lead_tiles_m = cdiv(prm.lead_M, BM);
+        prm2.lead_tiles = prm2.lead_tiles_m * cdiv(prm.lead_N, BN);
+    }
+    const int n_tiles = prm2.lead_tiles + prm2.tiles_n * prm2.tiles_m;
     const int sms = sm_count();
     kernel<<<n_tiles < sms ? n_tiles : sms, kThreads, Cfg::kSmemBytes, stream>>>(prm2);
     CAPB_CHECK_CUDA(cudaGetLastError());
@@ -650,6 +705,23 @@
     return cdiv(M, 2 * BM) * tiles_n <= sms && cdiv(M, BM) * tiles_n > sms ? 2 * BM : BM;
 }
 
+static bool encode_segs(TcParams& t, const GemmProblem& p, int first, int bn, int passes, std::string* err) {
+    for (int i = 0; i < p.nseg; ++i) {
+        const GemmSeg& g = p.seg[i];
+        const int s = first + i;
+        t.kblocks[s] = cdiv(g.K, BK);
+        bool ok = encode_plane(&t.a_hi[s], g.A_hi, p.M, g.K, g.lda_h, BM, err) &&
+                  encode_plane(&t.w_hi[s], g.W_hi, p.N, g.K, g.ldw_h, bn, err);
+        if (ok && passes == 3) {
+            if (g.A_lo == nullptr || g.W_lo == nullptr) { *err = "lo planes missing for 3-pass mode"; ok = false; }
+            ok = ok && encode_plane(&t.a_lo[s], g.A_lo, p.M, g.K, g.lda_h, BM, err) &&
+                 encode_plane(&t.w_lo[s], g.W_lo, p.N, g.K, g.ldw_h, bn, err);
+        }
+        if (!ok) return false;
+    }
+    return true;
+}
+
 GemmTcPlan* gemm_tc_plan_create(const GemmProblem& p, int passes) {
     std::string why;
     if (!gemm_tc_supported(p, &why)) { set_error("gemm_tc: unsupported problem: " + why); return nullptr; }
@@ -663,17 +735,35 @@
     t.M = p.M;
     t.N = p.N;
     std::string err;
-    for (int s = 0; s < p.nseg; ++s) {
-        const GemmSeg& g = p.seg[s];
-        t.kblocks[s] = cdiv(g.K, BK);
-        bool ok = encode_plane(&t.a_hi[s], g.A_hi, p.M, g.K, g.lda_h, BM, &err) &&
-                  encode_plane(&t.w_hi[s], g.W_hi, p.N, g.K, g.ldw_h, plan->bn, &err);
-        if (ok && passes == 3) {
-            if (g.A_lo == nullptr || g.W_lo == nullptr) { err = "lo planes missing for 3-pass mode"; ok = false; }
-            ok = ok && encode_plane(&t.a_lo[s], g.A_lo, p.M, g.K, g.lda_h, BM, &err) &&
-                 encode_plane(&t.w_lo[s], g.W_lo, p.N, g.K, g.ldw_h, plan->bn, &err);
-        }
-        if (!ok) { set_error("gemm_tc: " + err); delete plan; return nullptr; }
+    if (!encode_segs(t, p, 0, plan->bn, passes, &err)) { set_error("gemm_tc: " + err); delete plan; return nullptr; }
+    fill_epilogue(t, p.epi);
+    return plan;
+}
+
+GemmTcPlan* gemm_tc_group_plan_create(const GemmProblem& lead, const GemmProblem& p, int passes) {
+    std::string why;
+    if (!gemm_tc_supported(lead, &why) || !gemm_tc_supported(p, &why)) { set_error("gemm_tc: unsupported problem: " + why); return nullptr; }
+    if (lead.nseg + p.nseg > kMaxSeg) { set_error("gemm_tc: a grouped launch holds 3 K-segments in all"); return nullptr; }
+    if (lead.M != p.M) { set_error("gemm_tc: the problems of a grouped launch share their rows"); return nullptr; }
+    if (passes != 1 && passes != 3) { set_error("gemm_tc: passes must be 1 or 3"); return nullptr; }
+    GemmTcPlan* plan = new GemmTcPlan();
+    memset(&plan->prm, 0, sizeof(TcParams));
+    plan->passes = passes;
+    plan->bn = 160;
+    TcParams& t = plan->prm;
+    t.nseg = lead.nseg + p.nseg;
+    t.M = p.M;
+    t.N = p.N;
+    t.lead_nseg = lead.nseg;
+    t.lead_M = lead.M;
+    t.lead_N = lead.N;
+    t.lead_C = lead.epi.C;
+    t.lead_ldc = lead.epi.ldc;
+    std::string err;
+    if (!encode_segs(t, lead, 0, plan->bn, passes, &err) || !encode_segs(t, p, lead.nseg, plan->bn, passes, &err)) {
+        set_error("gemm_tc: " + err);
+        delete plan;
+        return nullptr;
     }
     fill_epilogue(t, p.epi);
     return plan;
@@ -694,6 +784,17 @@
     if (prm.M <= 0 || prm.N <= 0) return 0;
     const int kind = prm.lstm ? kEpiLstm : prm.C_hi != nullptr ? kEpiPlanes : kEpiStore;
     if (prm.trace != nullptr && plan->passes != 3) { set_error("gemm_tc: the traced kernel is the 3-pass one"); return 1; }
+    if (prm.lead_nseg > 0) {
+        if (kind != kEpiStore || prm.row_bias != nullptr || prm.gather_bias != nullptr || prm.residual != nullptr || prm.relu || prm.trace != nullptr) {
+            set_error("gemm_tc: a grouped launch stores fp32 with a column bias only");
+            return 1;
+        }
+        prm.lead_M = M;
+        int kb_lead = 0, kb_main = 0;
+        for (int s = 0; s < prm.nseg; ++s) (s < prm.lead_nseg ? kb_lead : kb_main) += prm.kblocks[s];
+        prm.catch_up = (kb_lead + kb_main / 2) / kb_main;
+        return launch_width<kEpiStore, BM>(plan->bn, plan->passes, prm, stream);
+    }
     const int bm = gemm_tc_tile_m(prm.M, prm.N, plan->bn);
     if (kind == kEpiLstm) return launch_kind<kEpiLstm>(bm, plan->bn, plan->passes, prm, stream);
     if (kind == kEpiPlanes) return launch_kind<kEpiPlanes>(bm, plan->bn, plan->passes, prm, stream);
diff --git a/imagecaptioning.pytorch_b200/csrc/kernels.cuh b/imagecaptioning.pytorch_b200/csrc/kernels.cuh
--- a/imagecaptioning.pytorch_b200/csrc/kernels.cuh
+++ b/imagecaptioning.pytorch_b200/csrc/kernels.cuh
@@ -119,9 +119,51 @@
 };
 int beam_step_launch(const BeamState& s, int t, int live, const float* top_val, const int* top_idx, int penalty_kind, float penalty_alpha,
                      cudaStream_t stream);
+struct NextCell {
+    const float* q = nullptr;
+    long ld_q = 0;
+    const float* row_bias = nullptr;
+    long ld_rb = 0;
+    const float* gather_bias = nullptr;
+    long ld_gb = 0;
+    float* c[2] = {nullptr, nullptr};
+    long ld_c = 0;
+    ActView h_out;
+};
+struct CellOperands {
+    float4 g, rb, gb;
+    float cp;
+};
+__device__ __forceinline__ CellOperands next_cell_load(const NextCell& nc, int img, int p, int w, int u, const float* c_prev) {
+    CellOperands o;
+    o.g = __ldg(reinterpret_cast<const float4*>(nc.q + (long)p * nc.ld_q + 4 * u));
+    o.rb = __ldg(reinterpret_cast<const float4*>(nc.row_bias + (long)img * nc.ld_rb + 4 * u));
+    o.gb = __ldg(reinterpret_cast<const float4*>(nc.gather_bias + (long)w * nc.ld_gb + 4 * u));
+    o.cp = __ldg(c_prev + (long)p * nc.ld_c + u);
+    return o;
+}
+__device__ __forceinline__ void next_cell_store(const NextCell& nc, long r, int u, CellOperands o, float* c_out) {
+    float4 g = o.g;
+    g.x += o.rb.x; g.y += o.rb.y; g.z += o.rb.z; g.w += o.rb.w;
+    g.x += o.gb.x; g.y += o.gb.y; g.z += o.gb.z; g.w += o.gb.w;
+    float c, h;
+    lstm_cell_unit(g.x, g.y, g.z, g.w, o.cp, c, h);
+    c_out[r * nc.ld_c + u] = c;
+    const long i = r * nc.h_out.ld + u;
+    nc.h_out.f[i] = h;
+    split_f32(h, nc.h_out.hi[i], nc.h_out.lo[i]);
+}
+__device__ __forceinline__ void next_cell_unit(const NextCell& nc, long r, int img, int p, int w, int u, const float* c_prev, float* c_out) {
+    next_cell_store(nc, r, u, next_cell_load(nc, img, p, w, u, c_prev), c_out);
+}
+bool next_cell_applies(const NextCell& c);
+int state_gather_cell_launch(int rows, int rpi, const int* tokens, const int* src_row, int H, StateCopy s1, const NextCell& cell, const float* c_prev,
+                             float* c_out, cudaStream_t stream);
+
 struct NextStateGather {
     StateCopy s0, s1;
     int H = 0;
+    NextCell cell;
 };
 bool beam_search_step_applies(const VocabStepArgs& a, const NextStateGather& next);
 int beam_search_step_launch(const BeamState& s, const VocabStepArgs& a, int t, int live, int penalty_kind, float penalty_alpha,
diff --git a/imagecaptioning.pytorch_b200/csrc/pointwise.cu b/imagecaptioning.pytorch_b200/csrc/pointwise.cu
--- a/imagecaptioning.pytorch_b200/csrc/pointwise.cu
+++ b/imagecaptioning.pytorch_b200/csrc/pointwise.cu
@@ -20,6 +20,19 @@
         o.hi[row * o.ld + col] = h;
         o.lo[row * o.ld + col] = l;
     }
+}
+
+__global__ void state_gather_cell_kernel(int rows, int rpi, const int* __restrict__ tokens, const int* __restrict__ src_row, int H, StateCopy sc1,
+                                         NextCell cell, const float* __restrict__ c_prev, float* __restrict__ c_out) {
+    const int r = blockIdx.x;
+    if (r >= rows) return;
+    const int src = src_row[r], w = tokens[r];
+    if ((H & 3) == 0 && (sc1.ld_src & 3) == 0 && (sc1.dst.ld & 3) == 0) {
+        for (int c4 = threadIdx.x; c4 < (H >> 2); c4 += blockDim.x) copy_states4(r, src, c4, 1, sc1, sc1);
+    } else {
+        for (int c = threadIdx.x; c < H; c += blockDim.x) store_act(sc1.dst, r, c, sc1.src[(long)src * sc1.ld_src + c]);
+    }
+    for (int u = threadIdx.x; u < H; u += blockDim.x) next_cell_unit(cell, r, r / rpi, src, w, u, c_prev, c_out);
 }
 
 __global__ void state_gather_embed_kernel(int rows, const int* __restrict__ tokens, const int* __restrict__ src_row,
@@ -294,6 +307,14 @@
     return 0;
 }
 
+int state_gather_cell_launch(int rows, int rpi, const int* tokens, const int* src_row, int H, StateCopy s1, const NextCell& cell, const float* c_prev,
+                             float* c_out, cudaStream_t stream) {
+    if (rows <= 0) return 0;
+    CAPB_REQUIRE(rpi >= 1 && next_cell_applies(cell), "the attention-LSTM cell needs its operands with 16-byte aligned gate rows");
+    state_gather_cell_kernel<<<rows, 256, 0, stream>>>(rows, rpi, tokens, src_row, H, s1, cell, c_prev, c_out);
+    CAPB_CHECK_CUDA(cudaGetLastError());
+    return 0;
+}
 
 int lstm_pointwise_launch(int rows, int H, const float* gates, long ld_g, const int* src_row, const float* c_prev, long ld_cp,
                           float* c_out, long ld_co, ActView h_out, const float* gather_bias, long ld_gb, const int* gather_idx,
diff --git a/imagecaptioning.pytorch_b200/models.py b/imagecaptioning.pytorch_b200/models.py
--- a/imagecaptioning.pytorch_b200/models.py
+++ b/imagecaptioning.pytorch_b200/models.py
@@ -333,15 +333,16 @@
     def launch_count(self) -> int:
         return 0 if self._engine is None else int(getattr(_lib.load(), 'capb200_%s_launch_count' % self._abi)(self._engine))
 
-    GEMM_IDS = ('fc_embed', 'att_embed', 'ctx2att', 'fc_gate_bias', 'att_lstm', 'h2att', 'lang_lstm', 'logit', 'newfc_core')
+    GEMM_IDS = ('fc_embed', 'att_embed', 'ctx2att', 'fc_gate_bias', 'att_lstm', 'h2att', 'lang_lstm', 'logit', 'newfc_core', 'logit_att_lstm')
 
     def set_profiling(self, enable: bool):
         _lib.check(_lib.load().capb200_engine_set_profiling(self._engine, int(enable)), 'set_profiling')
 
     def read_profile(self, reset=True):
         import numpy as np
-        ms, fl, calls = np.zeros(9), np.zeros(9), np.zeros(9, dtype=np.int64)
-        _lib.check(_lib.load().capb200_engine_read_profile(self._engine, int(reset), ms.ctypes.data, fl.ctypes.data, calls.ctypes.data, 9), 'read_profile')
+        n = len(self.GEMM_IDS)
+        ms, fl, calls = np.zeros(n), np.zeros(n), np.zeros(n, dtype=np.int64)
+        _lib.check(_lib.load().capb200_engine_read_profile(self._engine, int(reset), ms.ctypes.data, fl.ctypes.data, calls.ctypes.data, n), 'read_profile')
         return {n: (float(ms[i]), float(fl[i]), int(calls[i])) for i, n in enumerate(self.GEMM_IDS)}
 
     def forward(self, *args, **kwargs):
```

New measurement: 25630 (median of 6 runs). +2.2%, better.
